# chrished/DEMC.jl

Measured on AMD Instinct MI355X. Metric: chain-updates/sec (N x gens/s) + gens-to-Rhat<1.05, MvNormal d=5 N=1024, higher is better.
Workload: dtype f64

## Files before the change

demc.jl_amd/_lib.py:

```python
from __future__ import annotations

import ctypes as C
import os
import subprocess
from pathlib import Path

import numpy as np

PKG_DIR = Path(__file__).resolve().parent
REPO_ROOT = PKG_DIR.parent
LIB_PATH = Path(os.environ["DEMCZ_LIB"]) if os.environ.get("DEMCZ_LIB") else PKG_DIR / "libdemcz_hip.so"
ABI_VERSION = 1
LAYOUT_SPLIT = 100
LAYOUT_SPLIT_WAVE = 164
LAYOUT_PROGRAM_WAVE = 264

TARGET_MVNORMAL, TARGET_ISO_QUAD, TARGET_LINREG_SSE, TARGET_HOST_CALLBACK, TARGET_PROGRAM = 0, 1, 2, 3, 4
OK, ERR_INVALID_ARGUMENT, ERR_HIP, ERR_CAPACITY, ERR_STATE, ERR_NO_DEVICE, ERR_COMM = range(7)

_dp = C.POINTER(C.c_double)
_ip = C.POINTER(C.c_int32)
_lp = C.POINTER(C.c_int64)
_up = C.POINTER(C.c_uint64)

SYMBOLS = [
    "demcz_abi_version", "demcz_create", "demcz_destroy", "demcz_last_error", "demcz_set_state",
    "demcz_get_state", "demcz_set_history_origin", "demcz_run", "demcz_synchronize",
    "demcz_get_history", "demcz_get_changed", "demcz_rhat", "demcz_accept_ratio", "demcz_mean_cov",
    "demcz_propose", "demcz_accept_commit", "demcz_end_generation", "demcz_comm_unique_id",
    "demcz_comm_init", "demcz_export_current_device", "demcz_append_rows_device",
    "demcz_set_external_append", "demcz_get_info", "demcz_selftest_draws", "demcz_append_rows",
    "demcz_rhat_partial", "demcz_set_rng_offset", "demcz_rhat_array", "demcz_accept_ratio_array",
    "demcz_mean_cov_array", "demcz_set_append_lag", "demcz_run_checked", "demcz_set_kernel_timing",
    "demcz_get_kernel_time", "demcz_set_live_spin_limit", "demcz_get_live_status",
    "demcz_debug_append_slab", "demcz_get_changed_total", "demcz_debug_set_live_fault",
    "demcz_set_comm_timeout", "demcz_debug_stall_exchange", "demcz_get_kernel_time_series",
    "demcz_history_stream", "demcz_get_history_view", "demcz_detach_history", "demcz_release_host_buffer", "demcz_get_archive_pinned",
    "demcz_debug_kernel_counts", "demcz_pool_trim", "demcz_debug_kernel_name", "demcz_peer_group", "demcz_get_peer_status", "demcz_peer_export", "demcz_peer_attach",
    "demcz_peer_detach", "demcz_get_peer_ping", "demcz_set_live_rearms", "demcz_get_live_rearms",
    "demcz_closure_buffers", "demcz_program_check", "demcz_set_program",
    "demcz_program_check_layout",
    "demcz_autocov_sums", "demcz_autocov_sums_array", "demcz_ess_from_sums", "demcz_ess", "demcz_ess_array",
    "demcz_quantile_plan", "demcz_select_counts", "demcz_select_step", "demcz_quantile_finish", "demcz_quantiles",
    "demcz_quantiles_array", "demcz_best", "demcz_best_array",
    "demcz_derive_check", "demcz_derive", "demcz_derive_array",
    "demcz_rank_to_z", "demcz_rank_normalize", "demcz_rank_normalize_array", "demcz_indicator_le", "demcz_rank_diagnostics",
    "demcz_rank_diagnostics_array",
    "demcz_set_snooker", "demcz_get_snooker",
    "demcz_pointwise_check", "demcz_pointwise", "demcz_pointwise_array", "demcz_psis_tail_length", "demcz_gpd_fit",
    "demcz_loo_columns", "demcz_loo_columns_array", "demcz_loo", "demcz_loo_array",
    "demcz_bridge_check", "demcz_bridge_posterior", "demcz_bridge_posterior_array", "demcz_bridge_proposal",
    "demcz_bridge_proposal_program", "demcz_bridge_iterate", "demcz_bridge", "demcz_bridge_array",
    "demcz_histogram_edges", "demcz_histogram", "demcz_histogram_array", "demcz_histogram2d", "demcz_histogram2d_array",
    "demcz_hdi_steps", "demcz_hdi", "demcz_hdi_array",
]


class DemczError(RuntimeError):
    def __init__(self, code: int, msg: str):
        super().__init__(f"libdemcz_hip status {code}: {msg}")
        self.code = code


class Config(C.Structure):
    _fields_ = [
        ("N", C.c_int64), ("chain_id0", C.c_int64), ("d", C.c_int32), ("K", C.c_int32),
        ("Mcap", C.c_int64), ("Gcap", C.c_int64), ("Nblocks", C.c_int32),
        ("block_offsets", _ip), ("block_indices", _ip), ("eps_scale", _dp),
        ("seed", C.c_uint64), ("device_id", C.c_int32), ("target_kind", C.c_int32),
        ("mu", _dp), ("W", _dp), ("c0", C.c_double), ("design", _dp), ("yobs", _dp),
        ("nobs", C.c_int64), ("stream", C.c_void_p), ("lanes_per_chain", C.c_int32),
        ("reserved0", C.c_int32),
    ]


HIPCC_FLAGS = ["-O3", "--offload-arch=gfx950", "-ffp-contract=off", "-fPIC", "-Werror", "-Wno-pass-failed"]


def sources() -> list:
    csrc = PKG_DIR / "csrc"
    return ([csrc / "demcz_capi.hip"] + sorted(csrc.glob("demcz_pw_inst_*.hip")) + sorted(csrc.glob("demcz_mlr_inst_*.hip"))
            + [csrc / "demcz_snooker_inst.hip", csrc / "demcz_bridge_inst.hip", csrc / "demcz_program.hip"])


def build_command(out: Path = LIB_PATH) -> list:
    return ["hipcc"] + HIPCC_FLAGS + ["-shared", "-o", str(out)] + [str(p) for p in sources()] + ["-lrccl", "-lhiprtc"]


def build_lib(out: Path = LIB_PATH, extra: list = (), jobs: int = 0) -> Path:
    from concurrent.futures import ThreadPoolExecutor
    objdir = REPO_ROOT / "build" / "obj" / Path(out).stem
    objdir.mkdir(parents=True, exist_ok=True)
    srcs = sources()
    jobs = jobs or max(1, min(len(srcs), len(os.sched_getaffinity(0))))

    def compile_one(src):
        obj = objdir / (src.stem + ".o")
        r = subprocess.run(["hipcc"] + list(extra) + HIPCC_FLAGS + ["-c", "-o", str(obj), str(src)], capture_output=True, text=True)
        if r.returncode != 0:
            raise RuntimeError(f"hipcc failed on {src.name}:\n{r.stderr[-4000:]}")
        return obj

    with ThreadPoolExecutor(max_workers=jobs) as ex:
        objs = list(ex.map(compile_one, srcs))
    subprocess.run(["hipcc", "--offload-arch=gfx950", "-shared", "-fPIC", "-o", str(out)] + [str(o) for o in objs] + ["-lrccl", "-lhiprtc"], check=True)
    return Path(out)


def build(force: bool = False) -> Path:
    srcs = list((PKG_DIR / "csrc").glob("*")) + [REPO_ROOT / "include" / "demcz.h"]
    if not force and LIB_PATH.exists():
        newest = max(p.stat().st_mtime for p in srcs)
        if LIB_PATH.stat().st_mtime >= newest:
            return LIB_PATH
    return build_lib(LIB_PATH)


_LIB = None


def load():
    global _LIB
    if _LIB is not None:
        return _LIB
    if not LIB_PATH.exists():
        raise FileNotFoundError(
            f"{LIB_PATH} is missing: build it with `python -c 'import __graft_entry__ as g; g.build()'` "
            "(hipcc --offload-arch=gfx950).  There is no CPU fallback.")
    L = C.CDLL(str(LIB_PATH))
    L.demcz_abi_version.restype = C.c_int32
    if L.demcz_abi_version() != ABI_VERSION:
        raise RuntimeError("libdemcz_hip.so ABI version mismatch: rebuild")
    L.demcz_last_error.restype = C.c_char_p
    L.demcz_last_error.argtypes = [C.c_void_p]
    L.demcz_create.argtypes = [C.POINTER(C.c_void_p), C.POINTER(Config)]
    L.demcz_destroy.argtypes = [C.c_void_p]
    L.demcz_set_state.argtypes = [C.c_void_p, _dp, _dp, _dp, C.c_int64, C.c_int64]
    L.demcz_get_state.argtypes = [C.c_void_p, _dp, _dp, _dp, C.c_int64, _lp]
    L.demcz_set_history_origin.argtypes = [C.c_void_p, C.c_int64]
    L.demcz_run.argtypes = [C.c_void_p, C.c_int64, C.c_int64, C.c_double, _dp]
    L.demcz_synchronize.argtypes = [C.c_void_p]
    L.demcz_get_history.argtypes = [C.c_void_p, C.c_int64, C.c_int64, _dp, _dp]
    L.demcz_get_changed.argtypes = [C.c_void_p, C.c_int64, C.c_int64, _lp]
    L.demcz_get_changed_total.argtypes = [C.c_void_p, C.c_int64, C.c_int64, _lp, _ip]
    L.demcz_rhat.argtypes = [C.c_void_p, C.c_int64, C.c_int64, _dp]
    L.demcz_accept_ratio.argtypes = [C.c_void_p, C.c_int64, C.c_int64, _dp]
    L.demcz_mean_cov.argtypes = [C.c_void_p, C.c_int64, C.c_int64, _dp, _dp]
    L.demcz_propose.argtypes = [C.c_void_p, C.c_int64, C.c_int32, C.c_double, _dp]
    L.demcz_accept_commit.argtypes = [C.c_void_p, _dp, _dp]
    L.demcz_end_generation.argtypes = [C.c_void_p, C.c_int64]
    L.demcz_closure_buffers.argtypes = [C.c_void_p, C.POINTER(C.c_void_p), C.POINTER(C.c_void_p)]
    L.demcz_comm_unique_id.argtypes = [C.c_void_p]
    L.demcz_comm_init.argtypes = [C.c_void_p, C.c_void_p, C.c_int32, C.c_int32]
    L.demcz_export_current_device.argtypes = [C.c_void_p, C.c_void_p]
    L.demcz_append_rows_device.argtypes = [C.c_void_p, C.c_void_p, C.c_int64, C.c_int64]
    L.demcz_append_rows.argtypes = [C.c_void_p, _dp, C.c_int64, C.c_int64]
    L.demcz_rhat_partial.argtypes = [C.c_void_p, C.c_int64, C.c_int64, C.c_int32, _dp, _dp]
    L.demcz_set_rng_offset.argtypes = [C.c_void_p, C.c_int64]
    L.demcz_set_snooker.argtypes = [C.c_void_p, C.c_int32, C.c_double, C.c_double]
    L.demcz_get_snooker.argtypes = [C.c_void_p, _ip, _dp, _dp, _lp]
    L.demcz_set_append_lag.argtypes = [C.c_void_p, C.c_int32]
    L.demcz_rhat_array.argtypes = [C.c_int32, _dp, C.c_int64, C.c_int32, C.c_int64, _dp]
    L.demcz_autocov_sums.argtypes = [C.c_void_p, C.c_int64, C.c_int64, C.c_int64, C.c_int64, _dp]
    L.demcz_autocov_sums_array.argtypes = [C.c_int32, _dp, C.c_int64, C.c_int32, C.c_int64, C.c_int64, C.c_int64, _dp]
    L.demcz_ess_from_sums.argtypes = [C.c_int32, C.c_int64, C.c_int64, C.c_int64, _dp, _dp, _dp, _dp, _dp, _lp, _ip]
    L.demcz_ess.argtypes = [C.c_void_p, C.c_int64, C.c_int64, C.c_int64, _dp, _dp, _dp, _lp, _ip]
    L.demcz_ess_array.argtypes = [C.c_int32, _dp, C.c_int64, C.c_int32, C.c_int64, C.c_int64, _dp, _dp, _dp, _lp, _ip]
    L.demcz_quantile_plan.argtypes = [C.c_int64, C.c_int32, _dp, _lp, _lp, _dp]
    L.demcz_select_counts.argtypes = [C.c_void_p, C.c_int64, C.c_int64, C.c_int32, C.c_int32, _up, _lp, _lp]
    L.demcz_select_step.argtypes = [C.c_int32, C.c_int32, _lp, _up, _lp]
    L.demcz_quantile_finish.argtypes = [C.c_int32, C.c_int32, _up, _up, _dp, _lp, _dp, _dp, _dp]
    L.demcz_quantiles.argtypes = [C.c_void_p, C.c_int64, C.c_int64, C.c_int32, _dp, _dp, _dp, _dp]
    L.demcz_quantiles_array.argtypes = [C.c_int32, _dp, C.c_int64, C.c_int32, C.c_int64, C.c_int32, _dp, _dp, _dp, _dp]
    L.demcz_best.argtypes = [C.c_void_p, C.c_int64, C.c_int64, _dp, _lp, _lp, _dp]
    L.demcz_best_array.argtypes = [C.c_int32, _dp, C.c_int64, C.c_int64, _dp, _lp, _lp]
    L.demcz_accept_ratio_array.argtypes = [C.c_int32, _dp, C.c_int64, C.c_int64, _dp]
    L.demcz_mean_cov_array.argtypes = [C.c_int32, _dp, C.c_int64, C.c_int32, C.c_int64, _dp, _dp]
    L.demcz_set_external_append.argtypes = [C.c_void_p, C.c_int32]
    L.demcz_get_info.argtypes = [C.c_void_p, _lp, _lp, _ip]
    L.demcz_selftest_draws.argtypes = [C.c_int32, C.c_uint64, C.c_uint64, C.c_uint64, C.c_int32,
                                       C.POINTER(C.c_uint64), _dp, _dp]
    L.demcz_set_live_spin_limit.argtypes = [C.c_void_p, C.c_int32]
    L.demcz_get_live_status.argtypes = [C.c_void_p, _ip, _ip]
    L.demcz_debug_kernel_counts.argtypes = [C.c_void_p, _lp]
    L.demcz_history_stream.argtypes = [C.c_void_p, C.c_int32]
    L.demcz_get_history_view.argtypes = [C.c_void_p, C.c_int64, C.c_int64, C.POINTER(C.c_void_p), C.POINTER(C.c_void_p)]
    L.demcz_detach_history.argtypes = [C.c_void_p, C.POINTER(C.c_void_p), C.POINTER(C.c_void_p)]
    L.demcz_release_host_buffer.argtypes = [C.c_void_p]
    L.demcz_pool_trim.argtypes = [_lp, _lp]
    L.demcz_peer_group.argtypes = [C.POINTER(C.c_void_p), C.c_int32]
    L.demcz_get_peer_status.argtypes = [C.c_void_p, _ip, _ip]
    L.demcz_peer_export.argtypes = [C.c_void_p, C.c_int32, C.c_int32, C.c_void_p]
    L.demcz_peer_attach.argtypes = [C.c_void_p, C.c_void_p]
    L.demcz_peer_detach.argtypes = [C.c_void_p]
    L.demcz_get_peer_ping.argtypes = [C.c_void_p, _ip, _dp]
    L.demcz_set_live_rearms.argtypes = [C.c_void_p, C.c_int32]
    L.demcz_get_live_rearms.argtypes = [C.c_void_p, _ip, _ip]
    L.demcz_debug_kernel_name.argtypes = [C.c_void_p, C.c_char_p, C.c_int32]
    L.demcz_program_check.argtypes = [C.c_int32, C.c_char_p, C.c_char_p]
    L.demcz_program_check_layout.argtypes = [C.c_int32, C.c_char_p, C.c_char_p, C.c_int32]
    L.demcz_set_program.argtypes = [C.c_void_p, C.c_char_p, C.c_char_p, _dp, C.c_int64]
    L.demcz_derive_check.argtypes = [C.c_int32, C.c_int32, C.c_char_p, C.c_char_p]
    L.demcz_derive.argtypes = [C.c_void_p, C.c_int64, C.c_int64, C.c_int32, C.c_char_p, C.c_char_p, _dp, C.c_int64, C.POINTER(C.c_void_p)]
    L.demcz_derive_array.argtypes = [C.c_int32, _dp, _dp, C.c_int64, C.c_int32, C.c_int64, C.c_int32, C.c_char_p, C.c_char_p, _dp,
                                     C.c_int64, C.POINTER(C.c_void_p)]
    L.demcz_rank_to_z.argtypes = [C.c_int64, _dp, C.c_int64, _dp]
    L.demcz_rank_normalize.argtypes = [C.c_void_p, C.c_int64, C.c_int64, C.c_int32, _dp, C.POINTER(C.c_void_p)]
    L.demcz_rank_normalize_array.argtypes = [C.c_int32, _dp, C.c_int64, C.c_int32, C.c_int64, C.c_int32, _dp, C.POINTER(C.c_void_p)]
    L.demcz_indicator_le.argtypes = [C.c_void_p, C.c_int64, C.c_int64, C.c_int32, _dp, C.POINTER(C.c_void_p)]
    L.demcz_rank_diagnostics.argtypes = [C.c_void_p, C.c_int64, C.c_int64, _dp, _dp, _dp]
    L.demcz_rank_diagnostics_array.argtypes = [C.c_int32, _dp, C.c_int64, C.c_int32, C.c_int64, _dp, _dp, _dp]
    L.demcz_histogram_edges.argtypes = [C.c_int32, C.c_double, C.c_double, _dp]
    L.demcz_histogram.argtypes = [C.c_void_p, C.c_int64, C.c_int64, C.c_int32, _dp, _dp, _dp, _lp, _lp, _lp, _lp]
    L.demcz_histogram_array.argtypes = [C.c_int32, _dp, C.c_int64, C.c_int32, C.c_int64, C.c_int32, _dp, _dp, _dp, _lp, _lp, _lp, _lp]
    L.demcz_histogram2d.argtypes = [C.c_void_p, C.c_int64, C.c_int64, C.c_int32, _ip, C.c_int32, C.c_int32, _dp, _dp, _dp, _dp, _lp, _lp]
    L.demcz_histogram2d_array.argtypes = [C.c_int32, _dp, C.c_int64, C.c_int32, C.c_int64, C.c_int32, _ip, C.c_int32, C.c_int32, _dp, _dp,
                                          _dp, _dp, _lp, _lp]
    L.demcz_hdi_steps.argtypes = [C.c_int64, C.c_int32, _dp, _lp]
    L.demcz_hdi.argtypes = [C.c_void_p, C.c_int64, C.c_int64, C.c_int32, _dp, _dp]
    L.demcz_hdi_array.argtypes = [C.c_int32, _dp, C.c_int64, C.c_int32, C.c_int64, C.c_int32, _dp, _dp]
    _vpp = C.POINTER(C.c_void_p)
    L.demcz_pointwise_check.argtypes = [C.c_int32, C.c_char_p, C.c_char_p]
    L.demcz_pointwise.argtypes = [C.c_void_p, C.c_int64, C.c_int64, C.c_int64, C.c_int32, C.c_char_p, C.c_char_p, _dp, C.c_int64, _vpp]
    L.demcz_pointwise_array.argtypes = [C.c_int32, _dp, C.c_int64, C.c_int32, C.c_int64, C.c_int64, C.c_int32, C.c_char_p, C.c_char_p,
                                        _dp, C.c_int64, _vpp]
    L.demcz_psis_tail_length.argtypes = [C.c_int64, C.c_double, _lp]
    L.demcz_gpd_fit.argtypes = [C.c_int64, _dp, _dp, _dp, _dp]
    L.demcz_loo_columns.argtypes = [C.c_void_p, C.c_int64, C.c_int64, _dp, _dp, _dp, _lp, _dp, _dp]
    L.demcz_loo_columns_array.argtypes = [C.c_int32, _dp, C.c_int64, C.c_int32, C.c_int64, _dp, _dp, _dp, _lp, _dp, _dp]
    L.demcz_loo.argtypes = [C.c_void_p, C.c_int64, C.c_int64, C.c_int64, C.c_char_p, C.c_char_p, _dp, C.c_int64, _dp, _dp, _dp, _lp,
                            _dp, _dp]
    L.demcz_loo_array.argtypes = [C.c_int32, _dp, C.c_int64, C.c_int32, C.c_int64, C.c_int64, C.c_char_p, C.c_char_p, _dp, C.c_int64,
                                  _dp, _dp, _dp, _lp, _dp, _dp]
    _bridge_out = [_dp, _dp, _lp, _ip, _lp, _lp, _dp, _lp, _dp, _dp, _dp]
    L.demcz_bridge_check.argtypes = [C.c_int32, C.c_char_p, C.c_char_p]
    L.demcz_bridge_posterior.argtypes = [C.c_void_p, C.c_int64, C.c_int64, _dp, _dp, _vpp]
    L.demcz_bridge_posterior_array.argtypes = [C.c_int32, _dp, _dp, C.c_int64, C.c_int32, C.c_int64, _dp, _dp, _vpp]
    L.demcz_bridge_proposal.argtypes = [C.c_void_p, C.c_int64, C.c_int64, C.c_uint64, _dp, _dp, _vpp, _vpp]
    L.demcz_bridge_proposal_program.argtypes = [C.c_int32, C.c_int32, C.c_int64, C.c_int64, C.c_uint64, _dp, _dp, C.c_char_p, C.c_char_p,
                                                _dp, C.c_int64, _vpp, _vpp]
    L.demcz_bridge_iterate.argtypes = [C.c_void_p, C.c_int64, C.c_int64, C.c_void_p, C.c_int64, C.c_int64, C.c_double, C.c_double,
                                       C.c_int64, _dp, _lp, _ip, _dp, _lp, _vpp]
    L.demcz_bridge.argtypes = [C.c_void_p, C.c_int64, C.c_int64, C.c_uint64, C.c_double, C.c_double, C.c_int64] + _bridge_out
    L.demcz_bridge_array.argtypes = [C.c_int32, _dp, _dp, C.c_int64, C.c_int32, C.c_int64, C.c_char_p, C.c_char_p, _dp, C.c_int64,
                                     C.c_uint64, C.c_double, C.c_double, C.c_int64] + _bridge_out
    L.demcz_get_archive_pinned.argtypes =[C.c_void_p, C.POINTER(C.c_void_p), _lp]
    L.demcz_get_kernel_time_series.argtypes = [C.c_void_p, C.c_int32, _dp, _dp, _ip]
    L.demcz_set_comm_timeout.argtypes = [C.c_void_p, C.c_int64]
    L.demcz_debug_stall_exchange.argtypes = [C.c_void_p, C.c_int32]
    L.demcz_debug_set_live_fault.argtypes = [C.c_void_p, C.c_int32, C.c_int64]
    L.demcz_debug_append_slab.argtypes = [C.c_void_p, _dp, C.c_int32, C.c_int32, C.c_int32]
    for name in SYMBOLS:
        fn = getattr(L, name)
        if name != "demcz_last_error":
            fn.restype = C.c_int32
    _LIB = L
    return L


def derive_launch_constants() -> tuple:
    import re
    text = (PKG_DIR / "csrc" / "demcz_kernels_derive.h").read_text()
    return tuple(int(re.search(rf"constexpr int {name} = (\d+);", text).group(1)) for name in ("DERIVE_THREADS", "DERIVE_MAX_WG"))


def f64(a, order="C"):
    return np.require(a, dtype=np.float64, requirements=["F" if order == "F" else "C", "A"])


def ptr(a, t=_dp):
    return a.ctypes.data_as(t) if a is not None else None
```

demc.jl_amd/csrc/demcz_capi.hip:

```cpp
#include "../../include/demcz.h"
#include "demcz_kernels.h"
#include "demcz_kernels_acf.h"
#include "demcz_kernels_sel.h"
#include "demcz_select_host.h"
#include "demcz_kernels_rank.h"
#include "demcz_kernels_density.h"
#include "demcz_kernels_loo.h"
#include "demcz_kernels_bridge.h"
#include "demcz_slab_plan.h"
#include "demcz_run_plan.h"
#include "demcz_kernels_ml.h"
#include "demcz_kernels_pc.h"
#include "demcz_kernels_lr.h"
#include "demcz_kernels_ps.h"
#include "demcz_kernels_ps2.h"
#include "demcz_kernels_ps2d.h"
#include "demcz_kernels_snooker.h"
#include "demcz_pw_dispatch.h"
#include "demcz_mlr_dispatch.h"
#include "demcz_program.h"

#include <rccl/rccl.h>

#include <algorithm>
#include <chrono>
#include <thread>
#include <cstdlib>
#include <deque>
#include <map>
#include <mutex>
#include <cfloat>
#include <cmath>
#include <cstdio>
#include <cstring>
#include <string>
#include <unordered_map>
#include <vector>

using namespace demcz;

static thread_local std::string g_create_error;

namespace {
struct BufPool {
    struct Entry { void* p; size_t bytes; int device; };
    std::mutex mu;
    std::vector<Entry> free_list;
    size_t cached = 0;
    const size_t cap;
    const bool host;
    BufPool(size_t cap_, bool host_) : cap(cap_), host(host_) {}
    hipError_t acquire(void** out, size_t bytes, int device)
    {
        {
            std::lock_guard<std::mutex> lk(mu);
            int best = -1;
            for (int i = 0; i < (int)free_list.size(); ++i) {
                const Entry& e = free_list[i];
                if (e.device == device && e.bytes >= bytes && e.bytes <= bytes + bytes / 4 + (1u << 20) && (best < 0 || e.bytes < free_list[best].bytes)) best = i;
            }
            if (best >= 0) {
                *out = free_list[best].p;
                cached -= free_list[best].bytes;
                sizes[*out] = free_list[best].bytes;
                free_list.erase(free_list.begin() + best);
                return hipSuccess;
            }
        }
        hipError_t e = host ? hipHostMalloc(out, bytes, hipHostMallocDefault) : hipMalloc(out, bytes);
        if (e != hipSuccess) {
            (void)hipGetLastError();
            if (trim() > 0) e = host ? hipHostMalloc(out, bytes, hipHostMallocDefault) : hipMalloc(out, bytes);
        }
        if (e == hipSuccess) { std::lock_guard<std::mutex> lk(mu); sizes[*out] = bytes; }
        return e;
    }
    size_t trim()
    {
        std::vector<Entry> drop;
        size_t n = 0;
        {
            std::lock_guard<std::mutex> lk(mu);
            drop.swap(free_list);
            n = cached;
            cached = 0;
        }
        for (const Entry& e : drop) { if (host) (void)hipHostFree(e.p); else (void)hipFree(e.p); }
        return n;
    }
    void discard(void* p)
    {
        if (!p) return;
        { std::lock_guard<std::mutex> lk(mu); sizes.erase(p); }
        if (host) (void)hipHostFree(p); else (void)hipFree(p);
    }
    void release(void* p, int device)
    {
        if (!p) return;
        size_t bytes = 0;
        {
            std::lock_guard<std::mutex> lk(mu);
            auto it = sizes.find(p);
            if (it != sizes.end()) { bytes = it->second; sizes.erase(it); }
            if (bytes && cached + bytes <= cap && !getenv("DEMCZ_NO_POOL")) {
                free_list.push_back({p, bytes, device});
                cached += bytes;
                return;
            }
        }
        if (host) (void)hipHostFree(p); else (void)hipFree(p);
    }
    std::unordered_map<void*, size_t> sizes;
};
BufPool g_dev_pool(6ull << 30, false);
BufPool g_host_pool(3ull << 30, true);
}
static std::mutex g_stream_mu;
static std::vector<std::pair<int, hipStream_t>> g_stream_pool;
static hipError_t stream_acquire(int device, hipStream_t* out)
{
    {
        std::lock_guard<std::mutex> lk(g_stream_mu);
        for (size_t i = 0; i < g_stream_pool.size(); ++i)
            if (g_stream_pool[i].first == device) { *out = g_stream_pool[i].second; g_stream_pool.erase(g_stream_pool.begin() + (long)i); return hipSuccess; }
    }
    return hipStreamCreateWithFlags(out, hipStreamNonBlocking);
}
static void stream_release(int device, hipStream_t s, bool drained)
{
    if (!s) return;
    if (drained && !getenv("DEMCZ_NO_POOL")) {
        std::lock_guard<std::mutex> lk(g_stream_mu);
        if (g_stream_pool.size() < 32) { g_stream_pool.emplace_back(device, s); return; }
    }
    (void)hipStreamDestroy(s);
}
static hipError_t dev_malloc(int device, void** out, size_t bytes) { return g_dev_pool.acquire(out, std::max<size_t>(bytes, 16), device); }
static hipError_t dev_free(int device, void* p) { g_dev_pool.release(p, device); return hipSuccess; }
static hipError_t host_malloc(void** out, size_t bytes) { return g_host_pool.acquire(out, std::max<size_t>(bytes, 16), -1); }
static hipError_t host_free(void* p) { g_host_pool.release(p, -1); return hipSuccess; }

struct demcz_handle;
enum SplitKind {
    SPLIT_NONE = 0,
    SPLIT_PC8,
    SPLIT_ML,
    SPLIT_MLB,
    SPLIT_WAVE,
};

enum KernelArm { ARM_ONE_LANE, ARM_ML, ARM_ML_COOP, ARM_MLB, ARM_LR16, ARM_PC8, ARM_ML_REC, ARM_MLB_REC, ARM_LR16_REC, ARM_LR8S,
                 ARM_PS, ARM_PS2, ARM_PS2D, ARM_PW, ARM_PROGRAM_WAVE, ARM_SNOOKER };
struct WindowKernel {
    const void* fn = nullptr;
    hipFunction_t mod = nullptr;
    int threads = 0;
    size_t dyn_lds = 0;
    bool big_lds = false;
    int waves = 0;
    bool steady = false;
    KernelArm arm = ARM_ONE_LANE;
    bool live = false, temper = false;
    int pw_form = 0;
};

struct LaunchFacts {
    bool live = false;
    bool temper = false;
    bool ps2 = false;
    bool dual = false;
    bool pw_reg = false;
    bool pw_matrix = false;
    bool coop = false;
    bool lr16 = false;
    bool snooker = false;
};

struct PeerGroup {
    std::vector<demcz_handle*> members;
    bool failed = false;
    int32_t rearms_left = 3;
    bool lockstep_only = false;
    bool busy = false;
    bool dead = false;
};

struct demcz_handle {
    demcz_config cfg{};
    int lanes = 1;
    hipStream_t stream = nullptr;
    bool own_stream = false;
    std::string err;
    std::vector<int32_t> block_offsets, block_indices, slot_of;
    std::vector<double> eps;
    int64_t S = 0;
    int64_t ZS = 0;
    bool full_block = false;
    int ngrp = 1;
    uint64_t gstart = 1ull;
    int mlb_qb = 0;
    double* dZ = nullptr;
    double* dX = nullptr;
    double* dlp = nullptr;
    double* dchain = nullptr;
    double* dchain_alloc = nullptr;
    double* dlogobj = nullptr;
    double* dlp_origin = nullptr;
    bool origin_valid = false;
    double* dtemp = nullptr;
    int64_t temp_cap = 0;
    int32_t* d_block_offsets = nullptr;
    int32_t* d_slot_of = nullptr;
    double* d_eps = nullptr;
    double* d_mu = nullptr;
    double* d_Wp = nullptr;
    double* d_design = nullptr;
    double* d_y = nullptr;
    double* d_scratch = nullptr;
    int64_t scratch_cap = 0;
    double* d_stage = nullptr;
    int64_t stage_cap = 0;
    int64_t M = 0;
    int64_t g_done = 0;
    int64_t g0 = 0;
    int64_t rng_offset = 0;
    bool has_state = false;
    int64_t launches = 0;
    mutable int64_t kernel_counts[1] = {0};
    WindowKernel last_kernel;
    bool external_append = false;
    double* dXprop = nullptr;
    double* dlogu = nullptr;
    bool proposal_pending = false;
    bool gen_open = false;
    double* hc_X = nullptr;
    double* hc_lp = nullptr;
    volatile unsigned int* hc_flag = nullptr;
    unsigned int* hc_count = nullptr;
    unsigned int hc_seq = 0;
    hipStream_t diag_stream = nullptr;
    hipEvent_t diag_ev = nullptr;
    hipEvent_t rhat_side_ev = nullptr;
    bool rhat_side_pending = false;
    double* d_spec_X = nullptr;
    double* d_spec_lp = nullptr;
    hipEvent_t spec_ev = nullptr;
    double* pinned_rhat = nullptr;
    unsigned int* pinned_err = nullptr;
    int64_t pinned_err_launches = -1;
    int64_t pinned_cap = 0;
    bool timing = false;
    std::vector<std::pair<hipEvent_t, hipEvent_t>> timed;
    std::vector<int32_t> timed_slabs;
    std::vector<double> series_start_ms, series_dur_ms;
    int64_t timed_launches = 0;
    int64_t live_wg_cap = -1;
    SplitKind split_kind = SPLIT_NONE;
    int split_lanes = 0;
    int split_per_wg = 1;
    int32_t* d_slot_role = nullptr;
    double* d_rec[2] = {nullptr, nullptr};
    unsigned int* d_live_err = nullptr;
#ifdef DEMCZ_STAMPS
    unsigned long long* d_stamps = nullptr;
#endif
    bool arena = false, rec_in_arena = false, hist_joint = false;
    int64_t arena_gens = 0;
    int64_t arena_span = 0;
    double* arena_rec[2] = {nullptr, nullptr};
    double* arena_temp = nullptr;
    int64_t rec_cap = 0;
    int rec_cur = 0;
    bool host_paced = false;
    int wpw = 1;
    bool ps_dual = false;
    bool dual_now = false;
    bool lr_spec = false;
    bool no_live = false;
    bool live_claimed = false;
    unsigned int live_spin_limit = 0;
    int32_t live_fault_polls = 0;
    int64_t live_fault_g = 0;
    bool in_checked = false;
    struct RunCall { int64_t g_from, g_to; double gamma; bool tempered; std::vector<double> temperature; };
    std::vector<RunCall> live_log;
    double* d_safe_X = nullptr;
    double* d_safe_lp = nullptr;
    bool snap_pending = false;
    int64_t safe_M = 0, safe_M_app = 0, safe_g_done = 0;
    bool replaying = false;
    int32_t live_redos = 0;
    int32_t live_rearms_left = 3;
    int32_t live_rearms = 0;
    int64_t rearm_from = -1;
    uint32_t fail_row_hint = 0xffffffffu;
    RecDesc rec_desc[2];
    hipStream_t prod_stream = nullptr;
    hipEvent_t prod_done[2] = {nullptr, nullptr};
    hipEvent_t prod_gate = nullptr;
    bool prod_pending[2] = {false, false};
    hipEvent_t after_launch_ev = nullptr;
    unsigned int* d_acc = nullptr;
    int64_t acc_waves = 0;
    int32_t acc_slots = 0, acc_next = 0;
    struct LaunchRec { int64_t g_first, g_last; int32_t slot; };
    std::deque<LaunchRec> acc_log;
    ncclComm_t comm = nullptr;
    ncclComm_t comm_side = nullptr;
    int nranks = 1, rank = 0;
    double* d_gather = nullptr;
    int lag = 0;
    int64_t M_app = 0;
    struct PendingRows { int64_t visible_from; int64_t M_after; hipEvent_t ev; int64_t xseq = 0; };
    std::deque<PendingRows> pending;
    int64_t batch_J = -1;
    hipStream_t comm_stream = nullptr;
    double* d_send[2] = {nullptr, nullptr};
    double* d_recv[2] = {nullptr, nullptr};
    hipEvent_t buf_done[2] = {nullptr, nullptr};
    int64_t xseq = 0, xseq_waited = 0, buf_xseq[2] = {0, 0};
    int batch_buf = 0, batch_cnt = 0;
    int64_t batch_base = 0;
    bool hs_on = false;
    double* hs_chain = nullptr;
    double* hs_logobj = nullptr;
    hipStream_t hs_stream = nullptr;
    bool pooled_dev = false;
    volatile long long* xdone = nullptr;
    int peer_mode = 0;
    int n_peers = 0;
    double* peer_Z[DEMCZ_MAX_PEERS] = {nullptr};
    void* ipc_mapped[DEMCZ_MAX_PEERS] = {nullptr};
    struct PeerGroup* group = nullptr;
    bool err_clean = false;
    bool peer_fence = false;
    unsigned int* d_err_all = nullptr;
    bool archive_fine = false;
    size_t dZ_bytes = 0;
    size_t mailbox_off = 0;
    bool peers_closed = false;
    int32_t ping_ok = -1;
    double ping_wait_us = 0.0;
    int64_t live_share = 0;
    int64_t comm_timeout_ms = 60000;
    bool comm_dead = false;
    int* stall_flag = nullptr;
    int32_t stall_next_ms = 0;
    bool prog_ready = false;
    demcz_prog::Module prog;
    std::string prog_source, prog_options;
    bool prog_wave = false;
    bool derived = false;
    int64_t snooker_every = 0;
    double snooker_lo = 1.2, snooker_hi = 2.2;
    int64_t snooker_steps = 0;
    bool snooker_now = false;
};

#define HIPCHK(h, expr)                                                                          \
    do {                                                                                         \
        hipError_t e_ = (expr);                                                                  \
        if (e_ != hipSuccess) {                                                                  \
            (h)->err = std::string(#expr) + ": " + hipGetErrorString(e_);                        \
            return DEMCZ_ERR_HIP;                                                                \
        }                                                                                        \
    } while (0)

#define NCCLCHK(h, expr)                                                                         \
    do {                                                                                         \
        ncclResult_t r_ = (expr);                                                                \
        if (r_ != ncclSuccess) {                                                                 \
            (h)->err = std::string(#expr) + ": " + ncclGetErrorString(r_);                       \
            return DEMCZ_ERR_COMM;                                                               \
        }                                                                                        \
    } while (0)


#define DEADCHK(h)                                                                               \
    do {                                                                                         \
        if ((h)->comm_dead) return DEMCZ_ERR_COMM;                                               \
    } while (0)

static int32_t fail(demcz_handle* h, int32_t code, const std::string& msg)
{
    if (h) h->err = msg; else g_create_error = msg;
    return code;
}

static int32_t refuse_derived(const demcz_handle* h, const char* who)
{
    if (!h || !h->derived) return DEMCZ_OK;
    return fail(const_cast<demcz_handle*>(h), DEMCZ_ERR_STATE,
                std::string(who) + ": the handle is a derived history (demcz_derive): it takes the statistics over its values, demcz_get_history "
                                   "without log_obj, demcz_derive, demcz_pointwise, demcz_loo, demcz_bridge_iterate, demcz_synchronize and demcz_destroy, and nothing else");
}
#define NOT_DERIVED(h)                                                                           \
    do {                                                                                         \
        int32_t rd_ = refuse_derived((h), __func__);                                             \
        if (rd_) return rd_;                                                                     \
    } while (0)
// ... 104 lines not shown
}

static int32_t sync_event(demcz_handle* h, hipEvent_t ev, const char* what)
{
    if (h->comm_dead) return DEMCZ_ERR_COMM;
    if (!h->comm) {
        const hipError_t e = hipEventSynchronize(ev);
        if (e != hipSuccess) { h->err = std::string(what) + ": hipEventSynchronize: " + hipGetErrorString(e); return DEMCZ_ERR_HIP; }
        return DEMCZ_OK;
    }
    return wait_deadline(h, [ev]() { return hipEventQuery(ev); }, what);
}

#define SYNCCHK_AS(h, s, who)                                                                    \
    do {                                                                                         \
        int32_t rcs_ = sync_stream((h), (s), (who));                                             \
        if (rcs_) return rcs_;                                                                   \
    } while (0)
#define SYNCCHK(h, s) SYNCCHK_AS(h, s, __func__)

static int32_t quiesce_all(demcz_handle* h)
{
    if (h->comm_dead) return DEMCZ_ERR_COMM;
    if (!h->comm) return DEMCZ_OK;
    for (hipStream_t st : {h->stream, h->comm_stream, h->prod_stream, h->diag_stream, h->hs_stream})
        if (st) { int32_t rc = sync_stream(h, st, "quiesce"); if (rc) return rc; }
    return DEMCZ_OK;
}

static int32_t maybe_stall(demcz_handle* h, hipStream_t s)
{
    if (h->stall_next_ms <= 0) return DEMCZ_OK;
    if (getenv("DEMCZ_DEBUG_COMM")) fprintf(stderr, "[demcz] stall kernel of %d ms enqueued\n", h->stall_next_ms);
    if (!h->stall_flag) HIPCHK(h, dev_malloc(h->cfg.device_id, (void**)&h->stall_flag, sizeof(int)));
    HIPCHK(h, hipMemsetAsync(h->stall_flag, 0, sizeof(int), s));
    hipLaunchKernelGGL(stall_kernel, dim3(1), dim3(1), 0, s, h->stall_flag, (unsigned long long)h->stall_next_ms * 100000ull);
    HIPCHK(h, hipGetLastError());
    h->stall_next_ms = 0;
    return DEMCZ_OK;
}

static int64_t blockstep_nblk(int b)
{
    const int nn = (b == 1) ? 1 : b;
    return 1 + (nn + 1) / 2 + 1;
}

constexpr size_t ML_MAX_DYNAMIC_LDS = 160 * 1024;
constexpr size_t PEER_MAILBOX_BYTES = 4096;
constexpr size_t REC_PAD = 64;
constexpr int PC_CONSUMER_CHAINS = 8;
static int ml_lanes_available(int target_kind, int d, bool full_block, int64_t nobs, int max_blocklen, int nblocks);
static bool pc_available(int target_kind, int d, bool full_block);
static bool mlb32_wanted(int64_t N);
static bool split_ml_available(int target_kind, int d, bool full_block, int64_t nobs);
static bool ps_available(int target_kind, int d);
static int64_t live_wg_capacity(demcz_handle* h);
static WindowKernel window_kernel_of(const demcz_handle* h, const LaunchFacts& f);
static LaunchFacts launch_facts(const demcz_handle* h, const WindowParams* P, bool live);
constexpr int MAX_LIVE_KERNELS = 6;
static int live_kernels(const demcz_handle* h, WindowKernel out[MAX_LIVE_KERNELS]);
static void rec_invalidate(demcz_handle* h)
{
    if (h->prod_stream) (void)hipStreamSynchronize(h->prod_stream);
    h->prod_pending[0] = h->prod_pending[1] = false;
    h->rec_desc[0].valid = h->rec_desc[1].valid = false;
}
static int32_t rec_scrub(demcz_handle* h)
{
    rec_invalidate(h);
    if (h->lanes != DEMCZ_LAYOUT_SPLIT || h->rec_cap <= 0 || getenv("DEMCZ_NO_SCRUB")) return DEMCZ_OK;
    for (int b = 0; b < 2; ++b) {
        if (!h->d_rec[b]) continue;
        const size_t per = h->rec_in_arena ? (size_t)(h->cfg.d + 2) : (size_t)((h->split_kind == SPLIT_MLB) ? 2 * h->S : (int64_t)h->cfg.d + 2);
        const size_t nd = (size_t)h->rec_cap * per * (size_t)h->cfg.N + REC_PAD;
        HIPCHK(h, hipMemsetAsync(h->d_rec[b], 0, nd * sizeof(double), h->stream));
    }
    return DEMCZ_OK;
}
static int32_t flush_exchanges(demcz_handle* h);
static void peer_detach(demcz_handle* h);
static void peer_no_dual(demcz_handle* h);
static int32_t peer_setup_ipc(demcz_handle* h);
static bool peer_capable(const demcz_handle* h);
static int32_t check_live_err(demcz_handle* h);
static int32_t live_verify(demcz_handle* h);
static int32_t group_verify(demcz_handle* h);
static int32_t live_failed(demcz_handle* h, bool& failed);
static void live_release(demcz_handle* h);
static int64_t live_span(demcz_handle* h);
static int64_t rec_target_bytes(bool dual);
static int32_t rec_reserve(demcz_handle* h, int64_t gens);
static int32_t check_hist_range(demcz_handle* h, int64_t g_from, int64_t g_to, const char* who);
static bool ps2_applicable(const demcz_handle* h, const WindowParams& P);

extern "C" int32_t demcz_abi_version(void) { return DEMCZ_ABI_VERSION; }

extern "C" const char* demcz_last_error(const demcz_handle* h)
{
    return h ? h->err.c_str() : g_create_error.c_str();
}

template <class T>
static hipError_t dev_alloc_copy(T** dst, const T* src, size_t n, hipStream_t s, int device)
{
    hipError_t e = dev_malloc(device, (void**)dst, std::max<size_t>(n, 1) * sizeof(T));
    if (e != hipSuccess) return e;
    if (n) e = hipMemcpyAsync(*dst, src, n * sizeof(T), hipMemcpyHostToDevice, s);
    return e;
}

static void free_all(demcz_handle* h)
{
    bool drained = !h->comm_dead;
    for (hipStream_t st : {h->stream, h->prod_stream, h->diag_stream, h->comm_stream, h->hs_stream})
        if (st && hipStreamQuery(st) != hipSuccess) drained = false;
    if (h->d_acc) (void)dev_free(h->cfg.device_id, h->d_acc);
    if (h->d_err_all) (void)dev_free(h->cfg.device_id, h->d_err_all);
    if (h->archive_fine) { if (h->dZ) (void)hipFree(h->dZ); h->dZ = nullptr; }
    if (h->pooled_dev) {
        if (h->archive_fine) {
        } else if (drained) {
            g_dev_pool.release(h->dZ, h->cfg.device_id);
        } else {
            g_dev_pool.discard(h->dZ);
        }
        if (h->hist_joint) { if (drained) g_dev_pool.release(h->dchain_alloc, h->cfg.device_id); else g_dev_pool.discard(h->dchain_alloc); }
        h->dZ = nullptr;
        if (h->hist_joint) { h->dchain = nullptr; h->dchain_alloc = nullptr; }
    }
    if (h->hs_stream) stream_release(h->cfg.device_id, h->hs_stream, drained);
    if (drained) { g_host_pool.release(h->hs_chain, -1); g_host_pool.release(h->hs_logobj, -1); }
    else { g_host_pool.discard(h->hs_chain); g_host_pool.discard(h->hs_logobj); }
    void* bufs[] = {h->dZ, h->dX, h->dlp, h->dchain, h->hist_joint ? nullptr : h->dlogobj, h->dlp_origin, h->dtemp, h->d_block_offsets,
                    h->d_slot_of, h->d_slot_role, h->d_eps, h->d_mu, h->d_Wp, h->d_design, h->d_y, h->d_scratch, h->dXprop,
                    h->dlogu, h->d_gather};
    for (void* b : bufs)
        if (b) (void)dev_free(h->cfg.device_id, b);
    for (auto& pe : h->pending) if (pe.ev) (void)hipEventDestroy(pe.ev);
    h->pending.clear();
    for (int b = 0; b < 2; ++b) {
        if (h->d_rec[b] && !h->rec_in_arena) (void)dev_free(h->cfg.device_id, h->d_rec[b]);
        if (b == 0 && h->d_live_err) (void)dev_free(h->cfg.device_id, h->d_live_err);
        if (h->d_send[b]) (void)dev_free(h->cfg.device_id, h->d_send[b]);
        if (h->d_recv[b]) (void)dev_free(h->cfg.device_id, h->d_recv[b]);
        if (h->buf_done[b]) (void)hipEventDestroy(h->buf_done[b]);
    }
    if (h->comm_stream) stream_release(h->cfg.device_id, h->comm_stream, !h->comm_dead && hipStreamQuery(h->comm_stream) == hipSuccess);
    if (h->prod_stream) { if (!h->comm_dead) (void)hipStreamSynchronize(h->prod_stream); stream_release(h->cfg.device_id, h->prod_stream, !h->comm_dead); }
    for (int b = 0; b < 2; ++b) if (h->prod_done[b]) (void)hipEventDestroy(h->prod_done[b]);
    if (h->prod_gate) (void)hipEventDestroy(h->prod_gate);
    if (h->d_stage) (void)host_free(h->d_stage);
    for (auto& pr : h->timed) { (void)hipEventDestroy(pr.first); (void)hipEventDestroy(pr.second); }
    if (h->pinned_rhat) (void)host_free(h->pinned_rhat);
    if (h->pinned_err) (void)host_free(h->pinned_err);
    if (h->d_safe_X) (void)dev_free(h->cfg.device_id, h->d_safe_X);
    if (h->d_safe_lp) (void)dev_free(h->cfg.device_id, h->d_safe_lp);
    if (h->d_spec_X) (void)dev_free(h->cfg.device_id, h->d_spec_X);
    if (h->d_spec_lp) (void)dev_free(h->cfg.device_id, h->d_spec_lp);
    if (h->spec_ev) (void)hipEventDestroy(h->spec_ev);
    if (h->diag_ev) (void)hipEventDestroy(h->diag_ev);
    if (h->rhat_side_ev) (void)hipEventDestroy(h->rhat_side_ev);
    if (h->diag_stream) stream_release(h->cfg.device_id, h->diag_stream, !h->comm_dead && hipStreamQuery(h->diag_stream) == hipSuccess);
    if (h->stall_flag) (void)dev_free(h->cfg.device_id, h->stall_flag);
    if (h->hc_X) (void)hipHostFree(h->hc_X);
    if (h->hc_lp) (void)hipHostFree(h->hc_lp);
    if (h->hc_flag) (void)hipHostFree(const_cast<unsigned int*>(h->hc_flag));
    if (h->hc_count) (void)dev_free(h->cfg.device_id, h->hc_count);
    if (h->xdone) (void)host_free(const_cast<long long*>(h->xdone));
    if (!h->comm_dead) {
        if (h->comm_side) (void)ncclCommDestroy(h->comm_side);
        if (h->comm) (void)ncclCommDestroy(h->comm);
    }
    if (h->own_stream && h->stream) stream_release(h->cfg.device_id, h->stream, !h->comm_dead && hipStreamQuery(h->stream) == hipSuccess);
}

extern "C" int32_t demcz_create(demcz_handle** out, const demcz_config* cfg)
{
    if (!out || !cfg) return fail(nullptr, DEMCZ_ERR_INVALID_ARGUMENT, "demcz_create: null argument");
    *out = nullptr;
    if (cfg->N < 1 || cfg->d < 1 || cfg->d > MAX_D || cfg->K < 1 || cfg->Mcap < 2 || cfg->Gcap < 0 ||
        cfg->Nblocks < 1 || !cfg->block_offsets || !cfg->block_indices || !cfg->eps_scale || cfg->chain_id0 < 0)
        return fail(nullptr, DEMCZ_ERR_INVALID_ARGUMENT,
                    "demcz_create: need N>=1, 1<=d<=64, K>=1, Mcap>=2, Gcap>=0, Nblocks>=1 and block/eps tables");
    if (cfg->lanes_per_chain != 0 && cfg->lanes_per_chain != 1 && cfg->lanes_per_chain != 8 && cfg->lanes_per_chain != 16 &&
        cfg->lanes_per_chain != DEMCZ_LAYOUT_SPLIT && cfg->lanes_per_chain != DEMCZ_LAYOUT_SPLIT_WAVE &&
        cfg->lanes_per_chain != DEMCZ_LAYOUT_PROGRAM_WAVE)
        return fail(nullptr, DEMCZ_ERR_INVALID_ARGUMENT,
                    "demcz_create: lanes_per_chain must be 0 (auto), 1, 8, 16, DEMCZ_LAYOUT_SPLIT, DEMCZ_LAYOUT_SPLIT_WAVE or (program targets) "
                    "DEMCZ_LAYOUT_PROGRAM_WAVE");
    if (cfg->lanes_per_chain == DEMCZ_LAYOUT_PROGRAM_WAVE && cfg->target_kind != DEMCZ_TARGET_PROGRAM)
        return fail(nullptr, DEMCZ_ERR_INVALID_ARGUMENT, "demcz_create: DEMCZ_LAYOUT_PROGRAM_WAVE is the wave-per-chain layout of program targets: "
                                                         "target_kind must be DEMCZ_TARGET_PROGRAM (built-in targets: DEMCZ_LAYOUT_SPLIT_WAVE)");
    const int d = cfg->d;
    if (cfg->block_offsets[0] != 0) return fail(nullptr, DEMCZ_ERR_INVALID_ARGUMENT, "block_offsets[0] must be 0");
    for (int ib = 0; ib < cfg->Nblocks; ++ib) {
        const int a = cfg->block_offsets[ib], b = cfg->block_offsets[ib + 1];
        if (b <= a || b - a > d) return fail(nullptr, DEMCZ_ERR_INVALID_ARGUMENT, "empty or oversized block");
        for (int t = a; t < b; ++t) {
            if (cfg->block_indices[t] < 0 || cfg->block_indices[t] >= d)
                return fail(nullptr, DEMCZ_ERR_INVALID_ARGUMENT, "block index out of range");
            for (int u = a; u < t; ++u)
                if (cfg->block_indices[u] == cfg->block_indices[t])
                    return fail(nullptr, DEMCZ_ERR_INVALID_ARGUMENT, "duplicate index inside a block");
        }
    }
    switch (cfg->target_kind) {
    case DEMCZ_TARGET_MVNORMAL:
        if (!cfg->mu || !cfg->W) return fail(nullptr, DEMCZ_ERR_INVALID_ARGUMENT, "MVNORMAL needs mu and W");
        break;
    case DEMCZ_TARGET_ISO_QUAD:
        if (!cfg->mu) return fail(nullptr, DEMCZ_ERR_INVALID_ARGUMENT, "ISO_QUAD needs mu");
        break;
    case DEMCZ_TARGET_LINREG_SSE:
        if (!cfg->design || !cfg->yobs || cfg->nobs < 1)
            return fail(nullptr, DEMCZ_ERR_INVALID_ARGUMENT, "LINREG_SSE needs design, yobs, nobs>=1");
        break;
    case DEMCZ_TARGET_HOST_CALLBACK: break;
    case DEMCZ_TARGET_PROGRAM:
        if (cfg->lanes_per_chain != 0 && cfg->lanes_per_chain != 1 && cfg->lanes_per_chain != DEMCZ_LAYOUT_PROGRAM_WAVE)
            return fail(nullptr, DEMCZ_ERR_INVALID_ARGUMENT, "demcz_create: a program target runs one lane per chain: lanes_per_chain must be 0 or 1 "
                                                             "(or DEMCZ_LAYOUT_PROGRAM_WAVE: one wavefront per chain)");
        if (cfg->d > demcz_prog::MAX_PROGRAM_D)
            return fail(nullptr, DEMCZ_ERR_INVALID_ARGUMENT, "demcz_create: a program target needs 1 <= d <= 32");
        if (cfg->lanes_per_chain == DEMCZ_LAYOUT_PROGRAM_WAVE) {
            bool one_block = cfg->Nblocks == 1 && cfg->block_offsets[1] == d;
            for (int p = 0; one_block && p < d; ++p) one_block = cfg->block_indices[p] == p;
            if (!one_block)
                return fail(nullptr, DEMCZ_ERR_INVALID_ARGUMENT, "demcz_create: DEMCZ_LAYOUT_PROGRAM_WAVE needs one block 0..d-1 in order (block updates run one lane per chain)");
            if (d < demcz_prog::WAVE_MIN_D)
                return fail(nullptr, DEMCZ_ERR_INVALID_ARGUMENT, "demcz_create: DEMCZ_LAYOUT_PROGRAM_WAVE needs 2 <= d <= 32");
            if (cfg->N > PS_MAX_N)
                return fail(nullptr, DEMCZ_ERR_INVALID_ARGUMENT, "demcz_create: DEMCZ_LAYOUT_PROGRAM_WAVE needs N <= " + std::to_string(PS_MAX_N) +
                                                                 " (one wavefront per chain: PS_MAX_N)");
            if (!(cfg->Mcap <= 0xffffffffll && (double)cfg->Mcap * 8.0 * (((d + 7) / 8) * 8) < 4294967296.0))
                return fail(nullptr, DEMCZ_ERR_INVALID_ARGUMENT, "demcz_create: DEMCZ_LAYOUT_PROGRAM_WAVE needs an archive reachable by 32-bit offsets: "
                                                                 "Mcap * 8 * (d rounded up to a multiple of 8) < 2^32");
        }
        break;
    default: return fail(nullptr, DEMCZ_ERR_INVALID_ARGUMENT, "unknown target_kind");
    }
    int ndev = 0;
    if (hipGetDeviceCount(&ndev) != hipSuccess || ndev < 1)
        return fail(nullptr, DEMCZ_ERR_NO_DEVICE, "demcz_create: no HIP device visible (there is no CPU fallback)");
    if (cfg->device_id < 0 || cfg->device_id >= ndev)
        return fail(nullptr, DEMCZ_ERR_INVALID_ARGUMENT, "demcz_create: device_id out of range");

    demcz_handle* h = new demcz_handle();
    h->cfg = *cfg;
    h->lanes = 1;
    if (const char* re = getenv("DEMCZ_LIVE_REARMS")) h->live_rearms_left = std::max(0, atoi(re));
    auto bail = [&](int32_t code) {
        g_create_error = h->err;
        free_all(h);
        delete h;
        return code;
    };
#define CRCHK(expr)                                                                              \
    do {                                                                                         \
        hipError_t e_ = (expr);                                                                  \
        if (e_ != hipSuccess) {                                                                  \
            h->err = std::string(#expr) + ": " + hipGetErrorString(e_);                          \
            return bail(DEMCZ_ERR_HIP);                                                          \
        }                                                                                        \
    } while (0)
    CRCHK(hipSetDevice(cfg->device_id));
    if (cfg->stream) {
        h->stream = (hipStream_t)cfg->stream;
    } else {
        CRCHK(stream_acquire(cfg->device_id, &h->stream));
        h->own_stream = true;
    }
    h->block_offsets.assign(cfg->block_offsets, cfg->block_offsets + cfg->Nblocks + 1);
    h->block_indices.assign(cfg->block_indices, cfg->block_indices + h->block_offsets.back());
    h->eps.assign(cfg->eps_scale, cfg->eps_scale + d);
    h->slot_of.assign((size_t)cfg->Nblocks * d, -1);
    h->S = 0;
    for (int ib = 0; ib < cfg->Nblocks; ++ib) {
        const int a = h->block_offsets[ib], b = h->block_offsets[ib + 1];
        for (int t = a; t < b; ++t) h->slot_of[(size_t)ib * d + h->block_indices[t]] = t - a;
        h->S += blockstep_nblk(b - a);
    }
    h->full_block = (cfg->Nblocks == 1 && h->block_offsets[1] == d);
    if (h->full_block)
        for (int p = 0; p < d; ++p) h->full_block = h->full_block && (h->block_indices[p] == p);
    if (cfg->target_kind == DEMCZ_TARGET_MVNORMAL && cfg->Nblocks >= 2 && h->block_offsets.back() == d) {
        bool ok = true;
        uint64_t starts = 0;
        for (int ib = 0; ib < cfg->Nblocks && ok; ++ib) {
            const int lo = h->block_offsets[ib], hi = h->block_offsets[ib + 1];
            uint64_t seen = 0;
            for (int t = lo; t < hi; ++t) {
                const int j = h->block_indices[t];
                if (j < lo || j >= hi || ((seen >> (j - lo)) & 1ull)) { ok = false; break; }
                seen |= 1ull << (j - lo);
            }
            starts |= 1ull << lo;
        }
        if (ok) {
            h->ngrp = cfg->Nblocks;
            h->gstart = starts;
            bool equal = true;
            for (int ib = 0; ib < cfg->Nblocks; ++ib) equal = equal && (h->block_offsets[ib + 1] - h->block_offsets[ib] == h->block_offsets[1]);
            if (equal && d == 20 && h->block_offsets[1] == 5 && !getenv("DEMCZ_NO_MLB_INCREMENTAL")) h->mlb_qb = 5;
        }
    }
    {
// ... 1782 lines not shown
extern "C" int32_t demcz_run(demcz_handle* h, int64_t g_from, int64_t g_to, double gamma, const double* temperature)
{
    NOT_DERIVED(h);
    return run_call(h, g_from, g_to, gamma, temperature, RunHints{});
}

extern "C" int32_t demcz_synchronize(demcz_handle* h)
{
    if (!h) return DEMCZ_ERR_INVALID_ARGUMENT;
    DEADCHK(h);
    HIPCHK(h, hipSetDevice(h->cfg.device_id));
    SYNCCHK(h, h->stream);
    if (h->comm_stream) SYNCCHK(h, h->comm_stream);
    if (h->prod_stream) SYNCCHK(h, h->prod_stream);
    return live_verify(h);
}

static int32_t check_hist_range(demcz_handle* h, int64_t g_from, int64_t g_to, const char* who)
{
    if (h->cfg.Gcap <= 0) return fail(h, DEMCZ_ERR_STATE, std::string(who) + ": handle keeps no history (Gcap = 0)");
    if (g_from < 1 || g_to < g_from || g_from - h->g0 - 1 < 0 || g_to - h->g0 > h->cfg.Gcap)
        return fail(h, DEMCZ_ERR_INVALID_ARGUMENT, std::string(who) + ": generations outside the history window");
    return DEMCZ_OK;
}

extern "C" int32_t demcz_get_history(demcz_handle* h, int64_t g_from, int64_t g_to, double* chain, double* log_obj)
{
    if (!h) return DEMCZ_ERR_INVALID_ARGUMENT;
    DEADCHK(h);
    if (log_obj) NOT_DERIVED(h);
    int32_t rc = check_hist_range(h, g_from, g_to, "demcz_get_history");
    if (rc) return rc;
    HIPCHK(h, hipSetDevice(h->cfg.device_id));
    rc = live_verify(h);
    if (rc) return rc;
    const int64_t N = h->cfg.N, G = g_to - g_from + 1, s0 = g_from - h->g0 - 1;
    const int d = h->cfg.d;
    if (chain)
        HIPCHK(h, hipMemcpyAsync(chain, h->dchain + (size_t)N * d * s0, (size_t)N * d * G * sizeof(double),
                                 hipMemcpyDeviceToHost, h->stream));
    if (log_obj)
        HIPCHK(h, hipMemcpyAsync(log_obj, h->dlogobj + (size_t)N * s0, (size_t)N * G * sizeof(double),
                                 hipMemcpyDeviceToHost, h->stream));
    SYNCCHK(h, h->stream);
    return DEMCZ_OK;
}

extern "C" int32_t demcz_get_changed(demcz_handle* h, int64_t g_from, int64_t g_to, int64_t* changed)
{
    NOT_DERIVED(h);
    if (!h || !changed) return DEMCZ_ERR_INVALID_ARGUMENT;
    int32_t rc = check_hist_range(h, g_from, g_to, "demcz_get_changed");
    if (rc) return rc;
    const int64_t G = g_to - g_from + 1, s0 = g_from - h->g0 - 1;
    if (s0 == 0 && !h->origin_valid)
        return fail(h, DEMCZ_ERR_STATE, "demcz_get_changed: the log_obj before the first history slot is not known "
                                        "(set the history origin when exactly g0 generations have been run)");
    HIPCHK(h, hipSetDevice(h->cfg.device_id));
    rc = live_verify(h);
    if (rc) return rc;
    rc = ensure_scratch(h, G);
    if (rc) return rc;
    static_assert(sizeof(long long) == sizeof(double), "scratch reuse");
    hipLaunchKernelGGL(changed_from_history_kernel, dim3((unsigned)G), dim3(256), 0, h->stream, (const double*)h->dlogobj,
                       (const double*)h->dlp_origin, h->cfg.N, s0, (long long*)h->d_scratch);
    HIPCHK(h, hipGetLastError());
    static_assert(sizeof(int64_t) == sizeof(long long), "int64 layout");
    HIPCHK(h, hipMemcpyAsync(changed, h->d_scratch, (size_t)G * sizeof(int64_t), hipMemcpyDeviceToHost, h->stream));
    SYNCCHK(h, h->stream);
    return DEMCZ_OK;
}

namespace demcz {
__global__ void __launch_bounds__(256) sum_counts_kernel(const unsigned int* acc, int64_t waves, int slot0, int nslots, int ring,
                                                         int skip_first, long long* out)
{
    __shared__ long long red[256];
    long long a = 0;
    for (int64_t i = threadIdx.x; i < (int64_t)nslots * waves; i += 256) {
        const int sl = (int)(i / waves);
        const int64_t w = i % waves;
        const unsigned int* e = acc + ((size_t)((slot0 + sl) % ring) * (size_t)waves + (size_t)w) * 2;
        a += (long long)e[0];
        if (skip_first && sl == 0) a -= (long long)e[1];
    }
    red[threadIdx.x] = a;
    __syncthreads();
    for (int st = 128; st > 0; st >>= 1) {
        if ((int)threadIdx.x < st) red[threadIdx.x] += red[threadIdx.x + st];
        __syncthreads();
    }
    if (threadIdx.x == 0) *out = red[0];
}
}

extern "C" int32_t demcz_get_changed_total(demcz_handle* h, int64_t g_from, int64_t g_to, int64_t* total, int32_t* from_ballots)
{
    NOT_DERIVED(h);
    if (!h || !total || g_from < 1 || g_to < g_from) return DEMCZ_ERR_INVALID_ARGUMENT;
    HIPCHK(h, hipSetDevice(h->cfg.device_id));
    int32_t rc = live_verify(h);
    if (rc) return rc;
    int first = -1, last = -1, skip = 0;
    for (int i = 0; i < (int)h->acc_log.size(); ++i) {
        const auto& r = h->acc_log[i];
        if (first < 0 && (r.g_first == g_from || r.g_first == g_from - 1) && r.g_last >= g_from) { first = i; skip = (r.g_first == g_from - 1); }
        if (first >= 0 && r.g_last == g_to) { last = i; break; }
    }
    bool ok = first >= 0 && last >= first;
    for (int i = first; ok && i < last; ++i)
        ok = h->acc_log[i].g_last + 1 == h->acc_log[i + 1].g_first && (h->acc_log[i].slot + 1) % h->acc_slots == h->acc_log[i + 1].slot;
    if (ok && h->d_acc) {
        rc = ensure_scratch(h, 1);
        if (rc) return rc;
        static_assert(sizeof(long long) == sizeof(double), "scratch reuse");
        hipLaunchKernelGGL(sum_counts_kernel, dim3(1), dim3(256), 0, h->stream, (const unsigned int*)h->d_acc, h->acc_waves,
                           (int)h->acc_log[first].slot, last - first + 1, (int)h->acc_slots, skip, (long long*)h->d_scratch);
        HIPCHK(h, hipGetLastError());
        long long v = 0;
        HIPCHK(h, hipMemcpyAsync(&v, h->d_scratch, sizeof(v), hipMemcpyDeviceToHost, h->stream));
        SYNCCHK(h, h->stream);
        *total = (int64_t)v;
        if (from_ballots) *from_ballots = 1;
        return DEMCZ_OK;
    }
    std::vector<int64_t> ch((size_t)(g_to - g_from + 1));
    rc = demcz_get_changed(h, g_from, g_to, ch.data());
    if (rc) return rc;
    int64_t t = 0;
    for (int64_t v : ch) t += v;
    *total = t;
    if (from_ballots) *from_ballots = 0;
    return DEMCZ_OK;
}

struct RhatPlan { int64_t N, w, s0, n, nd, need; int d, nchunk; double *S1, *S2, *mean_j, *s2_j, *sums; int slabs = 1; double* out = nullptr; };

static int rhat_chunks(int64_t n) { return (int)std::min<int64_t>(std::max<int64_t>(1, n / 32), 32); }
static int64_t rhat_need(int64_t nd, int d, int nchunk) { return 2 * (2 * nchunk * nd) + 2 * (2 * nd) + 4 * d; }

static int32_t rhat_plan(demcz_handle* h, int64_t g_from, int64_t g_to, RhatPlan& r, const char* who = "demcz_rhat")
{
    int32_t rc = check_hist_range(h, g_from, g_to, who);
    if (rc) return rc;
    r.N = h->cfg.N; r.w = g_to - g_from + 1; r.s0 = g_from - h->g0 - 1; r.d = h->cfg.d;
    r.n = r.w / 2;
    if (r.n < 2) return fail(h, DEMCZ_ERR_INVALID_ARGUMENT, std::string(who) + ": window needs at least 4 generations");
    r.nchunk = rhat_chunks(r.n);
    r.nd = r.N * r.d;
    r.need = rhat_need(r.nd, r.d, r.nchunk);
    return DEMCZ_OK;
}

static int32_t rhat_scratch(demcz_handle* h, RhatPlan& r, int64_t extra, bool compute, hipStream_t qs = nullptr)
{
    HIPCHK(h, hipSetDevice(h->cfg.device_id));
    int32_t rc = ensure_scratch(h, r.need * r.slabs + (r.slabs > 1 ? (int64_t)r.slabs * r.d : 0) + extra);
    if (rc) return rc;
    r.S1 = h->d_scratch;
    r.S2 = r.S1 + 2 * r.nchunk * r.nd;
    r.mean_j = r.S2 + 2 * r.nchunk * r.nd;
    r.s2_j = r.mean_j + 2 * r.nd;
    r.sums = r.s2_j + 2 * r.nd;
    r.out = r.slabs > 1 ? h->d_scratch + r.need * r.slabs : r.sums + 3 * r.d;
    if (compute) {
        const int bs = 256;
        const unsigned gx = (unsigned)((r.nd + bs - 1) / bs);
        if (!qs) qs = h->stream;
        hipLaunchKernelGGL(rhat_moments_kernel, dim3(gx, 2 * r.nchunk, r.slabs), dim3(bs), 0, qs, h->dchain, r.N, r.d, r.s0, r.n, r.nchunk, r.S1, r.S2,
                           r.w, r.need);
        hipLaunchKernelGGL(rhat_chainstats_kernel, dim3(gx, 2, r.slabs), dim3(bs), 0, qs, h->dchain, r.N, r.d, r.s0, r.n, r.nchunk, r.S1, r.S2, r.mean_j,
                           r.s2_j, r.w, r.need);
        HIPCHK(h, hipGetLastError());
    }
    return DEMCZ_OK;
}

static int32_t rhat_prepare(demcz_handle* h, int64_t g_from, int64_t g_to, RhatPlan& r, bool compute, hipStream_t qs = nullptr, int slabs = 1)
{
    int32_t rc = rhat_plan(h, g_from, g_to, r);
    if (rc) return rc;
    if (slabs > 1) {
        rc = check_hist_range(h, g_from, g_from + r.w * slabs - 1, "demcz_run_checked");
        if (rc) return rc;
        r.slabs = slabs;
    }
    return rhat_scratch(h, r, 0, compute, qs);
}

extern "C" int32_t demcz_rhat_partial(demcz_handle* h, int64_t g_from, int64_t g_to, int32_t stage, const double* grand, double* out)
{
    if (!h || !out || (stage != 0 && stage != 1) || (stage == 1 && !grand)) return DEMCZ_ERR_INVALID_ARGUMENT;
    RhatPlan r;
    int32_t rc = live_verify(h);
    if (rc) return rc;
    rc = rhat_prepare(h, g_from, g_to, r, true);
    if (rc) return rc;
    const int d = r.d;
    if (stage == 0) {
        hipLaunchKernelGGL(rhat_reduce_kernel, dim3(d), dim3(256), 0, h->stream, r.mean_j, r.s2_j, r.N, d, 0, (const double*)nullptr, 1.0, r.sums);
        HIPCHK(h, hipGetLastError());
        HIPCHK(h, hipMemcpyAsync(out, r.sums, (size_t)d * sizeof(double), hipMemcpyDeviceToHost, h->stream));
    } else {
        HIPCHK(h, hipMemcpyAsync(r.sums, grand, (size_t)d * sizeof(double), hipMemcpyHostToDevice, h->stream));
        hipLaunchKernelGGL(rhat_reduce_kernel, dim3(d), dim3(256), 0, h->stream, r.mean_j, r.s2_j, r.N, d, 1, (const double*)r.sums, 1.0, r.sums + d);
        HIPCHK(h, hipGetLastError());
        HIPCHK(h, hipMemcpyAsync(out, r.sums + d, (size_t)2 * d * sizeof(double), hipMemcpyDeviceToHost, h->stream));
    }
    SYNCCHK(h, h->stream);
    return DEMCZ_OK;
}

static int32_t rhat_enqueue(demcz_handle* h, int64_t g_from, int64_t g_to, double* out, bool side = false, int slabs = 1)
{
    RhatPlan r;
    hipStream_t qs = h->stream;
    static const bool own_env = getenv("DEMCZ_RHAT_OWN_STREAM") != nullptr;
    if (side && !h->comm && !own_env && h->prod_stream) {
        if (!h->diag_ev) HIPCHK(h, hipEventCreateWithFlags(&h->diag_ev, hipEventDisableTiming));
        if (h->after_launch_ev) {
            HIPCHK(h, hipStreamWaitEvent(h->prod_stream, h->after_launch_ev, 0));
        } else {
            HIPCHK(h, hipEventRecord(h->diag_ev, h->stream));
            HIPCHK(h, hipStreamWaitEvent(h->prod_stream, h->diag_ev, 0));
            h->after_launch_ev = h->diag_ev;
        }
        qs = h->prod_stream;
    } else if (side && h->comm && h->peer_mode == 2 && !h->no_live && h->comm_side && h->comm_stream && h->lag == 0) {
        if (!h->diag_ev) HIPCHK(h, hipEventCreateWithFlags(&h->diag_ev, hipEventDisableTiming));
        if (h->after_launch_ev) {
            HIPCHK(h, hipStreamWaitEvent(h->comm_stream, h->after_launch_ev, 0));
        } else {
            HIPCHK(h, hipEventRecord(h->diag_ev, h->stream));
            HIPCHK(h, hipStreamWaitEvent(h->comm_stream, h->diag_ev, 0));
            h->after_launch_ev = h->diag_ev;
        }
        qs = h->comm_stream;
    } else if (side && !h->comm) {
        if (!h->diag_stream) HIPCHK(h, stream_acquire(h->cfg.device_id, &h->diag_stream));
        if (!h->diag_ev) HIPCHK(h, hipEventCreateWithFlags(&h->diag_ev, hipEventDisableTiming));
        if (h->after_launch_ev) {
            HIPCHK(h, hipStreamWaitEvent(h->diag_stream, h->after_launch_ev, 0));
        } else {
            HIPCHK(h, hipEventRecord(h->diag_ev, h->stream));
            HIPCHK(h, hipStreamWaitEvent(h->diag_stream, h->diag_ev, 0));
            h->after_launch_ev = h->diag_ev;
        }
        qs = h->diag_stream;
    }
    if (qs == h->stream && h->rhat_side_pending) {
        HIPCHK(h, hipStreamWaitEvent(h->stream, h->rhat_side_ev, 0));
        h->rhat_side_pending = false;
    }
    struct SideMark {
        demcz_handle* h; hipStream_t qs;
        ~SideMark() {
            if (qs == h->stream) return;
            if (!h->rhat_side_ev && hipEventCreateWithFlags(&h->rhat_side_ev, hipEventDisableTiming) != hipSuccess) { h->rhat_side_ev = nullptr; return; }
            if (hipEventRecord(h->rhat_side_ev, qs) == hipSuccess) h->rhat_side_pending = true;
        }
    } side_mark{h, qs};
    if (slabs > 1 && h->comm) return fail(h, DEMCZ_ERR_STATE, "demcz_run_checked: batched checks are for unsharded runs");
    int32_t rc = rhat_prepare(h, g_from, g_to, r, true, qs, slabs);
    if (rc) return rc;
    const int d = r.d;
    const int64_t n = r.n;
    const int64_t m = 2 * r.N * h->nranks;
    const bool sharded = (h->comm != nullptr);
    double* sums = r.sums;
    if (!sharded) {
        hipLaunchKernelGGL(rhat_tail_kernel, dim3(d, r.slabs), dim3(256), 0, qs, r.mean_j, r.s2_j, r.N, d, (double)n, (double)m, r.out, r.need);
        HIPCHK(h, hipGetLastError());
        HIPCHK(h, hipMemcpyAsync(out, r.out, (size_t)r.slabs * d * sizeof(double), hipMemcpyDeviceToHost, qs));
        return DEMCZ_OK;
    }
    const ncclComm_t cq = (qs == h->comm_stream && qs != h->stream) ? h->comm_side : h->comm;
    hipLaunchKernelGGL(rhat_reduce_kernel, dim3(d), dim3(256), 0, qs, r.mean_j, r.s2_j, r.N, d, 0, (const double*)nullptr, 1.0, sums);
    HIPCHK(h, hipGetLastError());
    NCCLCHK(h, ncclAllReduce(sums, sums, (size_t)d, ncclDouble, ncclSum, cq, qs));
    hipLaunchKernelGGL(rhat_reduce_kernel, dim3(d), dim3(256), 0, qs, r.mean_j, r.s2_j, r.N, d, 1, (const double*)sums, (double)m, sums + d);
    HIPCHK(h, hipGetLastError());
    NCCLCHK(h, ncclAllReduce(sums + d, sums + d, (size_t)2 * d, ncclDouble, ncclSum, cq, qs));
    hipLaunchKernelGGL(rhat_final_kernel, dim3((unsigned)((d + 63) / 64)), dim3(64), 0, qs, (const double*)(sums + d), d, (double)n, (double)m, sums + 3 * d);
    HIPCHK(h, hipGetLastError());
    HIPCHK(h, hipMemcpyAsync(out, sums + 3 * d, (size_t)d * sizeof(double), hipMemcpyDeviceToHost, qs));
    return DEMCZ_OK;
}

extern "C" int32_t demcz_rhat(demcz_handle* h, int64_t g_from, int64_t g_to, double* rhat)
{
    if (!h || !rhat) return DEMCZ_ERR_INVALID_ARGUMENT;
    int32_t rc = live_verify(h);
    if (rc) return rc;
    rc = rhat_enqueue(h, g_from, g_to, rhat);
    if (rc) return rc;
    SYNCCHK(h, h->stream);
    return DEMCZ_OK;
}

struct AcfPlan { RhatPlan r; int nchunk, tiles; int64_t per; double *part, *out; };

static void acf_chunks(int64_t N, int d, int64_t n, int& nchunk, int64_t& per)
{
    const int64_t waves = (N * d + ACF_BS - 1) / ACF_BS;
    const int64_t want = (4096 + 8 * waves - 1) / (8 * waves);
    const int64_t k = std::max<int64_t>(1, std::min<int64_t>(std::min<int64_t>(n / (2 * ACF_TL), want), 64));
    per = ((n + k - 1) / k + ACF_TL - 1) / ACF_TL * ACF_TL;
    nchunk = (int)((n + per - 1) / per);
}

static int32_t acf_prepare(demcz_handle* h, int64_t g_from, int64_t g_to, AcfPlan& a, const char* who)
{
    int32_t rc = live_verify(h);
    if (rc) return rc;
    rc = rhat_plan(h, g_from, g_to, a.r, who);
    if (rc) return rc;
    RhatPlan& r = a.r;
    acf_chunks(r.N, r.d, r.n, a.nchunk, a.per);
    const int64_t tile = (int64_t)2 * a.nchunk * ACF_TL * r.nd;
    a.tiles = (int)std::max<int64_t>(1, std::min<int64_t>(4, ((int64_t)1 << 24) / tile));
    rc = rhat_scratch(h, r, a.tiles * tile + (int64_t)a.tiles * ACF_TL * r.d, false);
    if (rc) return rc;
    if (h->rhat_side_pending) {
        HIPCHK(h, hipStreamWaitEvent(h->stream, h->rhat_side_ev, 0));
        h->rhat_side_pending = false;
    }
    a.part = h->d_scratch + r.need;
    a.out = a.part + a.tiles * tile;
    return DEMCZ_OK;
}

static int32_t acf_enqueue(demcz_handle* h, const AcfPlan& a, int64_t lag_from, int64_t lag_to, double* sums)
{
    const RhatPlan& r = a.r;
    const unsigned gx = (unsigned)((r.nd + ACF_BS - 1) / ACF_BS);
    for (int64_t t = lag_from; t <= lag_to; t += (int64_t)a.tiles * ACF_TL) {
        const int64_t nl = std::min<int64_t>((int64_t)a.tiles * ACF_TL, lag_to - t + 1);
        const unsigned nz = (unsigned)((nl + ACF_TL - 1) / ACF_TL);
        hipLaunchKernelGGL(acf_products_kernel, dim3(gx, 2 * a.nchunk, nz), dim3(ACF_BS), 0, h->stream, (const double*)h->dchain,
                           (const double*)r.mean_j, r.N, r.d, r.s0, r.n, a.nchunk, a.per, t, a.part);
        hipLaunchKernelGGL(acf_reduce_kernel, dim3(r.d, (unsigned)nl), dim3(256), 0, h->stream, (const double*)a.part, r.N, r.d, a.nchunk,
                           a.out, (int64_t)0);
        HIPCHK(h, hipGetLastError());
        HIPCHK(h, hipMemcpyAsync(sums + (size_t)r.d * (t - lag_from), a.out, (size_t)r.d * nl * sizeof(double), hipMemcpyDeviceToHost, h->stream));
    }
    return DEMCZ_OK;
}

extern "C" int32_t demcz_autocov_sums(demcz_handle* h, int64_t g_from, int64_t g_to, int64_t lag_from, int64_t lag_to, double* sums)
{
    if (!h || !sums) return DEMCZ_ERR_INVALID_ARGUMENT;
    AcfPlan a;
    int32_t rc = acf_prepare(h, g_from, g_to, a, "demcz_autocov_sums");
    if (rc) return rc;
    if (lag_from < 0 || lag_to < lag_from || lag_to > a.r.n - 1)
        return fail(h, DEMCZ_ERR_INVALID_ARGUMENT, "demcz_autocov_sums: 0 <= lag_from <= lag_to <= n - 1, n = half the window");
    rc = rhat_scratch(h, a.r, 0, true);
    if (rc) return rc;
    rc = acf_enqueue(h, a, lag_from, lag_to, sums);
    if (rc) return rc;
    SYNCCHK(h, h->stream);
    return DEMCZ_OK;
}

extern "C" int32_t demcz_ess_from_sums(int32_t d, int64_t m, int64_t n, int64_t nlags, const double* sums, const double* between,
                                       double* ess, double* tau, double* varplus, int64_t* pairs, int32_t* converged)
{
    if (d <= 0 || m < 1 || n < 2 || nlags < 1 || !sums || !between || !ess) return DEMCZ_ERR_INVALID_ARGUMENT;
    const double dn = (double)n, dm = (double)m, S = dm * dn;
    const double cap = S * std::log10(S), floor_tau = 1.0 / std::log10(S);
    const int64_t L = nlags - 1;
    for (int p = 0; p < d; ++p) {
        const double A0 = sums[p] / S;
        const double W = A0 * dn / (dn - 1.0);
        const double vp = A0 + between[p] / (dm - 1.0);
        double sum = 0.0, prev = 0.0;
        int64_t k = 0;
        int32_t conv = 0;
        for (; 2 * k + 1 <= L; ++k) {
            const double r0 = k ? 1.0 - (W - sums[p + (size_t)d * (2 * k)] / S) / vp : 1.0;
            const double r1 = 1.0 - (W - sums[p + (size_t)d * (2 * k + 1)] / S) / vp;
            double P = r0 + r1;
            if (!(P > 0.0)) {
                conv = 1;
                if (P != P) sum = P;
                break;
            }
            if (k && prev < P) P = prev;
            sum += P;
            prev = P;
        }
        const double t = -1.0 + 2.0 * sum;
        ess[p] = (t < floor_tau) ? cap : S / t;
        if (tau) tau[p] = t;
        if (varplus) varplus[p] = vp;
        if (pairs) pairs[p] = k;
        if (converged) converged[p] = conv;
    }
    return DEMCZ_OK;
}

extern "C" int32_t demcz_ess(demcz_handle* h, int64_t g_from, int64_t g_to, int64_t max_lag,
                             double* ess, double* tau, double* varplus, int64_t* pairs, int32_t* converged)
{
    if (!h || !ess) return DEMCZ_ERR_INVALID_ARGUMENT;
    if (h->comm && h->nranks > 1)
        return fail(h, DEMCZ_ERR_INVALID_ARGUMENT, "demcz_ess: on a sharded handle add demcz_autocov_sums and demcz_rhat_partial over the ranks "
                                                   "on the host and finish with demcz_ess_from_sums");
    AcfPlan a;
    int32_t rc = acf_prepare(h, g_from, g_to, a, "demcz_ess");
    if (rc) return rc;
    rc = rhat_scratch(h, a.r, 0, true);
    if (rc) return rc;
    const RhatPlan& r = a.r;
    const int d = r.d;
    const int64_t n = r.n, m = 2 * r.N;
    const int64_t L = (max_lag <= 0) ? n - 1 : std::min<int64_t>(n - 1, max_lag);
    hipLaunchKernelGGL(rhat_reduce_kernel, dim3(d), dim3(256), 0, h->stream, r.mean_j, r.s2_j, r.N, d, 0, (const double*)nullptr, 1.0, r.sums);
    hipLaunchKernelGGL(rhat_reduce_kernel, dim3(d), dim3(256), 0, h->stream, r.mean_j, r.s2_j, r.N, d, 1, (const double*)r.sums, (double)m, r.sums + d);
    HIPCHK(h, hipGetLastError());
    std::vector<double> between((size_t)d), sums;
    std::vector<int32_t> conv((size_t)d);
    HIPCHK(h, hipMemcpyAsync(between.data(), r.sums + d, (size_t)d * sizeof(double), hipMemcpyDeviceToHost, h->stream));
    const int64_t batch = (int64_t)a.tiles * ACF_TL;
    int64_t have = 0;
    for (;;) {
        const int64_t to = std::min<int64_t>(L, have + batch - 1);
        sums.resize((size_t)d * (to + 1));
        rc = acf_enqueue(h, a, have, to, sums.data() + (size_t)d * have);
        if (rc) { (void)hipStreamSynchronize(h->stream); return rc; }
        SYNCCHK(h, h->stream);
        have = to + 1;
        rc = demcz_ess_from_sums(d, m, n, have, sums.data(), between.data(), ess, tau, varplus, pairs, conv.data());
        if (rc) return fail(h, rc, "demcz_ess: finisher");
        if (have > L || std::all_of(conv.begin(), conv.end(), [](int32_t c) { return c == 1; })) break;
    }
    if (converged) std::copy(conv.begin(), conv.end(), converged);
    return DEMCZ_OK;
}
// ... 2298 lines not shown
}

extern "C" int32_t demcz_bridge_posterior_array(int32_t device_id, const double* chain, const double* log_obj, int64_t N, int32_t d,
                                                int64_t G, const double* mean, const double* L, demcz_handle** derived)
{
    if (derived) *derived = nullptr;
    if (!chain || !log_obj || !derived || !mean || !L) return DEMCZ_ERR_INVALID_ARGUMENT;
    return with_arrays(device_id, N, d, G, chain, log_obj, [&](demcz_handle* h) { return bridge_posterior_from(h, 1, G, mean, L, derived); });
}

extern "C" int32_t demcz_bridge_proposal(demcz_handle* h, int64_t Np, int64_t wp, uint64_t seed, const double* mean, const double* L,
                                         demcz_handle** logratio, demcz_handle** draws)
{
    if (logratio) *logratio = nullptr;
    if (draws) *draws = nullptr;
    NOT_DERIVED(h);
    if (!h || !logratio || !mean || !L) return DEMCZ_ERR_INVALID_ARGUMENT;
    DEADCHK(h);
    BridgeTarget t;
    int32_t rc = bridge_target_of(h, "demcz_bridge_proposal", t);
    if (rc) return rc;
    return bridge_proposal_from(h, h->cfg.d, t, Np, wp, seed, mean, L, logratio, draws);
}

extern "C" int32_t demcz_bridge_proposal_program(int32_t device_id, int32_t d, int64_t Np, int64_t wp, uint64_t seed, const double* mean,
                                                 const double* L, const char* source, const char* options, const double* data,
                                                 int64_t ndata, demcz_handle** logratio, demcz_handle** draws)
{
    if (logratio) *logratio = nullptr;
    if (draws) *draws = nullptr;
    if (!logratio || !mean || !L) return DEMCZ_ERR_INVALID_ARGUMENT;
    int32_t rc = demcz_bridge_check(d, source, options);
    if (rc) return rc;
    return with_arrays(device_id, 1, d, 1, nullptr, nullptr, [&](demcz_handle* h) {
        BridgeTarget t;
        int32_t r2 = bridge_target_program(h, d, source, options, data, ndata, "demcz_bridge_proposal_program", t);
        return r2 ? r2 : bridge_proposal_from(h, d, t, Np, wp, seed, mean, L, logratio, draws);
    });
}

extern "C" int32_t demcz_bridge_iterate(demcz_handle* post, int64_t g_from, int64_t g_to, demcz_handle* prop, int64_t gp_from,
                                        int64_t gp_to, double neff, double tol, int64_t max_iter, double* logml, int64_t* iterations,
                                        int32_t* converged, double* moments, int64_t* n_nan, demcz_handle** f2)
{
    if (f2) *f2 = nullptr;
    if (!post || !prop) return DEMCZ_ERR_INVALID_ARGUMENT;
    DEADCHK(post);
    DEADCHK(prop);
    BridgeResult res;
    int32_t rc = bridge_iterate_from(post, g_from, g_to, prop, gp_from, gp_to, neff, tol, max_iter, res, f2);
    if (rc) return rc;
    if (logml) *logml = res.logml;
    if (iterations) *iterations = res.iterations;
    if (converged) *converged = res.converged;
    if (moments) std::copy(res.moments, res.moments + 4, moments);
    if (n_nan) *n_nan = res.n_nan;
    return DEMCZ_OK;
}

extern "C" int32_t demcz_bridge(demcz_handle* h, int64_t g_from, int64_t g_to, uint64_t seed, double neff, double tol, int64_t max_iter,
                                double* logml, double* se_logml, int64_t* iterations, int32_t* converged, int64_t* n_post,
                                int64_t* n_prop, double* neff_used, int64_t* n_nan, double* ess_f2, double* mean_out, double* L_out)
{
    NOT_DERIVED(h);
    if (!h) return DEMCZ_ERR_INVALID_ARGUMENT;
    DEADCHK(h);
    int32_t rc = rank_refuse_sharded(h, "demcz_bridge");
    if (rc) return rc;
    BridgeTarget t;
    rc = bridge_target_of(h, "demcz_bridge", t);
    if (rc) return rc;
    const BridgeOut o{logml, se_logml, iterations, converged, n_post, n_prop, neff_used, n_nan, ess_f2, mean_out, L_out};
    return bridge_from(h, t, g_from, g_to, seed, neff, tol, max_iter, o);
}

extern "C" int32_t demcz_bridge_array(int32_t device_id, const double* chain, const double* log_obj, int64_t N, int32_t d, int64_t G,
                                      const char* source, const char* options, const double* data, int64_t ndata, uint64_t seed,
                                      double neff, double tol, int64_t max_iter, double* logml, double* se_logml, int64_t* iterations,
                                      int32_t* converged, int64_t* n_post, int64_t* n_prop, double* neff_used, int64_t* n_nan,
                                      double* ess_f2, double* mean_out, double* L_out)
{
    if (!chain || !log_obj) return DEMCZ_ERR_INVALID_ARGUMENT;
    int32_t rc = demcz_bridge_check(d, source, options);
    if (rc) return rc;
    const BridgeOut o{logml, se_logml, iterations, converged, n_post, n_prop, neff_used, n_nan, ess_f2, mean_out, L_out};
    return with_arrays(device_id, N, d, G, chain, log_obj, [&](demcz_handle* h) {
        BridgeTarget t;
        int32_t r2 = bridge_target_program(h, d, source, options, data, ndata, "demcz_bridge_array", t);
        return r2 ? r2 : bridge_from(h, t, 1, G, seed, neff, tol, max_iter, o);
    });
}

extern "C" int32_t demcz_get_info(const demcz_handle* h, int64_t* M, int64_t* launches_window, int32_t* lanes_per_chain)
{
    NOT_DERIVED(h);
    if (!h) return DEMCZ_ERR_INVALID_ARGUMENT;
    if (M) *M = h->M_app;
    if (launches_window) *launches_window = h->launches;
    if (lanes_per_chain) *lanes_per_chain = h->prog_wave ? DEMCZ_LAYOUT_PROGRAM_WAVE : (h->split_kind == SPLIT_WAVE) ? DEMCZ_LAYOUT_SPLIT_WAVE : h->lanes;
    return DEMCZ_OK;
}

extern "C" int32_t demcz_selftest_draws(int32_t device_id, uint64_t seed, uint64_t chain, uint64_t blk0, int32_t n,
                                        uint64_t* words, double* normals, double* logu)
{
    if (n < 1 || !words || !normals || !logu) return DEMCZ_ERR_INVALID_ARGUMENT;
    int ndev = 0;
    if (hipGetDeviceCount(&ndev) != hipSuccess || ndev < 1)
        return fail(nullptr, DEMCZ_ERR_NO_DEVICE, "demcz_selftest_draws: no HIP device visible");
    if (hipSetDevice(device_id) != hipSuccess) return fail(nullptr, DEMCZ_ERR_HIP, "hipSetDevice failed");
    uint64_t* dw = nullptr; double* dn = nullptr; double* dl = nullptr;
    int32_t rc = DEMCZ_OK;
    if (hipMalloc((void**)&dw, (size_t)n * 16) != hipSuccess || hipMalloc((void**)&dn, (size_t)n * 16) != hipSuccess ||
        hipMalloc((void**)&dl, (size_t)n * 8) != hipSuccess) {
        rc = fail(nullptr, DEMCZ_ERR_HIP, "demcz_selftest_draws: hipMalloc failed");
    } else {
        hipLaunchKernelGGL(selftest_draws_kernel, dim3((unsigned)((n + 63) / 64)), dim3(64), 0, 0, seed, chain, blk0, (int)n, dw, dn, dl);
        if (hipMemcpy(words, dw, (size_t)n * 16, hipMemcpyDeviceToHost) != hipSuccess ||
            hipMemcpy(normals, dn, (size_t)n * 16, hipMemcpyDeviceToHost) != hipSuccess ||
            hipMemcpy(logu, dl, (size_t)n * 8, hipMemcpyDeviceToHost) != hipSuccess)
            rc = fail(nullptr, DEMCZ_ERR_HIP, "demcz_selftest_draws: kernel or copy failed");
    }
    if (dw) (void)hipFree(dw);
    if (dn) (void)hipFree(dn);
    if (dl) (void)hipFree(dl);
    return rc;
}

#ifdef DEMCZ_STAMPS
extern "C" int32_t demcz_debug_read_stamps(demcz_handle* h, unsigned long long* out, int64_t n_wg)
{
    NOT_DERIVED(h);
    if (!h || !out || n_wg < 0 || n_wg > DEMCZ_STAMP_WGS || !h->d_stamps) return DEMCZ_ERR_INVALID_ARGUMENT;
    SYNCCHK(h, h->stream);
    HIPCHK(h, hipMemcpy(out, h->d_stamps, (size_t)n_wg * 16 * sizeof(unsigned long long), hipMemcpyDeviceToHost));
    return DEMCZ_OK;
}
#endif

static int32_t run_checked_body(demcz_handle* h, int64_t g_from, int64_t g_to, double gamma, const double* temperature,
                                int64_t every, double threshold, int64_t* g_stop, int32_t* n_checks,
                                double* rhat_max, int32_t n_max, double* rhat_last)
{
    const int d = h->cfg.d;
    int32_t checks = 0;
    int64_t g = g_from;
    if (g_stop) *g_stop = g_to;
    const bool monitor = !(threshold > 0.0);
    const int64_t max_checks = (g_to - g_from + 1) / every + 2;
    HIPCHK(h, hipSetDevice(h->cfg.device_id));
    if (max_checks * d > h->pinned_cap) {
        { int32_t rcq = quiesce_all(h); if (rcq) return rcq; }
        SYNCCHK(h, h->stream);
        if (h->pinned_rhat) (void)host_free(h->pinned_rhat);
        h->pinned_rhat = nullptr; h->pinned_cap = 0;
        const int64_t cap = std::max<int64_t>(max_checks, 1024) * d;
        HIPCHK(h, host_malloc((void**)&h->pinned_rhat, (size_t)cap * sizeof(double)));
        h->pinned_cap = cap;
    }
    double* pinned = h->pinned_rhat;
    auto max_of = [d](const double* r) {
        double mx = r[0];
        for (int p = 1; p < d; ++p) mx = (r[p] > mx || r[p] != r[p]) ? r[p] : mx;
        return mx;
    };
    int32_t rc = DEMCZ_OK;
    const bool speculate = !monitor && !h->comm && h->lag == 0 && !h->external_append && !temperature;
    const int64_t N = h->cfg.N;
    if (speculate) {
        if (!h->d_spec_X) HIPCHK(h, dev_malloc(h->cfg.device_id, (void**)&h->d_spec_X, (size_t)N * d * sizeof(double)));
        if (!h->d_spec_lp) HIPCHK(h, dev_malloc(h->cfg.device_id, (void**)&h->d_spec_lp, (size_t)N * sizeof(double)));
        if (!h->spec_ev) HIPCHK(h, hipEventCreateWithFlags(&h->spec_ev, hipEventDisableTiming));
    }
    bool ahead = false;
    const bool grouped = monitor && !h->comm && h->lag == 0 && !h->external_append;
    int64_t max_slabs = 1;
    if (grouped && h->cfg.Gcap > 0) {
        const int64_t need1 = rhat_need(N * d, d, rhat_chunks(every / 2));
        const int64_t ls0 = live_span(h);
        max_slabs = std::max<int64_t>(1, std::min<int64_t>(std::min<int64_t>(SLAB_GROUP_MAX, ((int64_t)1 << 25) / need1), (ls0 > 0 ? ls0 : h->cfg.Gcap) / every + 1));
        rc = ensure_scratch(h, max_slabs * (need1 + d));
    }
    auto cut_now = [h]() {
        int64_t cut = 0;
        if (h->live_fault_polls != 0) cut = h->live_fault_g;
        if (h->no_live && h->rearm_from >= 0 && (cut == 0 || h->rearm_from + 1 < cut)) cut = h->rearm_from + 1;
        return cut;
    };
    while (g <= g_to && rc == DEMCZ_OK) {
        int64_t nxt = std::min(g_to, slab_end_at_or_after(g, every));
        RunHints hints;
        if (grouped) {
            const int64_t ls = live_span(h);
            const int64_t span = ls > 0 ? ls : INT64_MAX;
            nxt = slab_group_end(g, g_to, every, span, cut_now(), max_slabs);
            hints.bracket_slabs = (int32_t)(slab_ends_in(g, nxt, every) + (nxt % every != 0 ? 1 : 0));
            hints.next_ngen = nxt < g_to ? std::min<int64_t>(span, slab_group_end(nxt + 1, g_to, every, span, cut_now(), max_slabs) - nxt) : 0;
        }
        if (!ahead) rc = run_call(h, g, nxt, gamma, temperature ? temperature + (g - g_from) : nullptr, hints);
        ahead = false;
        if (rc) break;
        int64_t c0 = slab_end_at_or_after(g, every);
        while (c0 <= nxt && c0 - every < h->g0) c0 += every;
        const int64_t nck = c0 <= nxt ? (nxt - c0) / every + 1 : 0;
        if (nck > 0) {
            double* slot = pinned + (size_t)checks * d;
            rc = rhat_enqueue(h, c0 - every + 1, c0, slot, monitor && nxt < g_to, (int)nck);
            if (rc) break;
            checks += (int32_t)nck;
            if (!monitor) {
                int64_t M_before = 0;
                if (speculate && nxt < g_to) {
                    if (hipEventRecord(h->spec_ev, h->stream) != hipSuccess) { rc = fail(h, DEMCZ_ERR_HIP, "demcz_run_checked: event failed"); break; }
                    if (hipMemcpyAsync(h->d_spec_X, h->dX, (size_t)N * d * sizeof(double), hipMemcpyDeviceToDevice, h->stream) != hipSuccess ||
                        hipMemcpyAsync(h->d_spec_lp, h->dlp, (size_t)N * sizeof(double), hipMemcpyDeviceToDevice, h->stream) != hipSuccess) {
                        rc = fail(h, DEMCZ_ERR_HIP, "demcz_run_checked: snapshot failed");
                        break;
                    }
                    M_before = h->M_app;
                    const int64_t nn = std::min(g_to, slab_end_at_or_after(nxt + 1, every));
                    rc = demcz_run(h, nxt + 1, nn, gamma, nullptr);
                    if (rc) break;
                    ahead = true;
                    if ((rc = sync_event(h, h->spec_ev, "demcz_run_checked")) != DEMCZ_OK) break;
                } else if ((rc = sync_stream(h, h->stream, "demcz_run_checked")) != DEMCZ_OK) {
                    break;
                }
                if (max_of(slot) < threshold) {
                    if (g_stop) *g_stop = nxt;
                    if (ahead) {
                        if ((rc = sync_stream(h, h->stream, "demcz_run_checked")) != DEMCZ_OK) break;
                        rc = check_live_err(h);
                        if (rc) break;
                        if (hipMemcpyAsync(h->dX, h->d_spec_X, (size_t)N * d * sizeof(double), hipMemcpyDeviceToDevice, h->stream) != hipSuccess ||
                            hipMemcpyAsync(h->dlp, h->d_spec_lp, (size_t)N * sizeof(double), hipMemcpyDeviceToDevice, h->stream) != hipSuccess) {
                            rc = fail(h, DEMCZ_ERR_HIP, "demcz_run_checked: restore failed");
                            break;
                        }
                        const size_t rest = (size_t)(h->M_app - M_before) * (size_t)h->ZS;
                        if (rest > 0) {
                            hipLaunchKernelGGL(fill_u64_kernel, dim3((unsigned)((rest + 255) / 256)), dim3(256), 0, h->stream,
                                               reinterpret_cast<unsigned long long*>(h->dZ + (size_t)M_before * h->ZS), rest, LIVE_SENTINEL);
                            if (hipGetLastError() != hipSuccess) { rc = fail(h, DEMCZ_ERR_HIP, "demcz_run_checked: restore failed"); break; }
                        }
                        const int64_t s_lo = nxt - h->g0, s_hi = std::min<int64_t>(h->g_done - h->g0, h->cfg.Gcap);
                        if (s_hi > s_lo &&
                            (hipMemsetAsync(h->dchain + (size_t)N * d * s_lo, 0, (size_t)N * d * (s_hi - s_lo) * sizeof(double), h->stream) != hipSuccess ||
                             hipMemsetAsync(h->dlogobj + (size_t)N * s_lo, 0, (size_t)N * (s_hi - s_lo) * sizeof(double), h->stream) != hipSuccess)) {
                            rc = fail(h, DEMCZ_ERR_HIP, "demcz_run_checked: restore failed");
                            break;
                        }
                        if (h->hs_on) { h->after_launch_ev = nullptr; rc = stream_history(h, nxt + 1, h->g_done); if (rc) break; }
                        h->M_app = M_before;
                        h->M = M_before;
                        h->g_done = nxt;
                        if ((rc = rec_scrub(h)) != DEMCZ_OK) break;
                        if (!h->live_log.empty() && h->live_log.back().g_from == nxt + 1) h->live_log.pop_back();
                        while (!h->acc_log.empty() && h->acc_log.back().g_last > nxt) h->acc_log.pop_back();
                    }
                    break;
                }
            }
        }
        g = nxt + 1;
    }
    h->pinned_err_launches = -1;
    if (rc == DEMCZ_OK && !h->live_log.empty() && h->peer_mode != 2) {
        if (!h->pinned_err && host_malloc((void**)&h->pinned_err, 4 * sizeof(unsigned int)) != hipSuccess) { h->pinned_err = nullptr; (void)hipGetLastError(); }
        if (h->pinned_err && hipMemcpyAsync(h->pinned_err, h->d_live_err, 4 * sizeof(unsigned int), hipMemcpyDeviceToHost, h->stream) == hipSuccess)
            h->pinned_err_launches = h->launches;
    }
    if (rc == DEMCZ_OK) rc = sync_stream(h, h->stream, "demcz_run_checked");
    if (rc == DEMCZ_OK && h->diag_stream) rc = sync_stream(h, h->diag_stream, "demcz_run_checked");
    if (rc == DEMCZ_OK && h->prod_stream) rc = sync_stream(h, h->prod_stream, "demcz_run_checked");
    if (rc == DEMCZ_OK && h->comm_stream) rc = sync_stream(h, h->comm_stream, "demcz_run_checked");
    if (rc == DEMCZ_OK) {
        for (int32_t i = 0; i < checks; ++i)
            if (rhat_max && i < n_max) rhat_max[i] = max_of(pinned + (size_t)i * d);
        if (rhat_last && checks > 0) std::copy(pinned + (size_t)(checks - 1) * d, pinned + (size_t)checks * d, rhat_last);
        if (n_checks) *n_checks = checks;
    }
    return rc;
}

extern "C" int32_t demcz_run_checked(demcz_handle* h, int64_t g_from, int64_t g_to, double gamma, const double* temperature,
                                     int64_t every, double threshold, int64_t* g_stop, int32_t* n_checks,
                                     double* rhat_max, int32_t n_max, double* rhat_last)
{
    NOT_DERIVED(h);
    if (!h) return DEMCZ_ERR_INVALID_ARGUMENT;
    DEADCHK(h);
    if (every < 4 || g_from < 1 || g_to < g_from) return fail(h, DEMCZ_ERR_INVALID_ARGUMENT, "demcz_run_checked: need every >= 4 and 1 <= g_from <= g_to");
    if (!h->has_state) return fail(h, DEMCZ_ERR_STATE, "demcz_run_checked: call demcz_set_state first");
    if (h->peer_mode == 1 || h->peer_mode == 3) return fail(h, DEMCZ_ERR_STATE, "demcz_run_checked: replica groups and host-mediated peers are driven call by call (demcz_run, demcz_rhat_partial)");
    HIPCHK(h, hipSetDevice(h->cfg.device_id));
    int32_t rc = live_verify(h);
    if (rc) return rc;
    if (h->no_live && h->rearm_from >= g_from) h->rearm_from = g_from - 1;
    const bool pacing = (getenv("DEMCZ_NO_HOST_PACING") == nullptr);
    for (;;) {
        h->host_paced = pacing;
        h->in_checked = true;
        rc = run_checked_body(h, g_from, g_to, gamma, temperature, every, threshold, g_stop, n_checks, rhat_max, n_max, rhat_last);
        h->host_paced = false;
        h->in_checked = false;
        if (h->live_log.empty()) break;
        if (rc != DEMCZ_OK && h->peer_mode == 2) break;
        bool failed = false;
        { int32_t rcf = live_failed(h, failed); if (rcf) { rc = rcf; break; } }
        if (!failed) { h->live_log.clear(); break; }
        std::vector<demcz_handle::RunCall> dropped;
        rc = live_rollback(h, dropped);
        if (rc) break;
        h->replaying = true;
    }
    h->replaying = false;
    return rc;
}

extern "C" int32_t demcz_set_live_spin_limit(demcz_handle* h, int32_t polls)
{
    NOT_DERIVED(h);
    if (!h || polls < 0) return DEMCZ_ERR_INVALID_ARGUMENT;
    h->live_spin_limit = (unsigned int)polls;
    return DEMCZ_OK;
}

extern "C" int32_t demcz_set_live_rearms(demcz_handle* h, int32_t n)
{
    NOT_DERIVED(h);
    if (!h || n < 0) return DEMCZ_ERR_INVALID_ARGUMENT;
    h->live_rearms_left = n;
    if (h->peer_mode == 1 && h->group) {
        h->group->rearms_left = n;
        for (demcz_handle* m : h->group->members) m->live_rearms_left = n;
    }
    if (n == 0) h->rearm_from = -1;
    return DEMCZ_OK;
}

extern "C" int32_t demcz_get_live_rearms(const demcz_handle* h, int32_t* rearms, int32_t* left)
{
    NOT_DERIVED(h);
    if (!h) return DEMCZ_ERR_INVALID_ARGUMENT;
    if (rearms) *rearms = h->live_rearms;
    if (left) *left = h->live_rearms_left;
    return DEMCZ_OK;
}

extern "C" int32_t demcz_debug_set_live_fault(demcz_handle* h, int32_t polls, int64_t g_from)
{
    NOT_DERIVED(h);
    if (!h || polls < -1 || g_from < 0) return DEMCZ_ERR_INVALID_ARGUMENT;
    h->live_fault_polls = polls;
    h->live_fault_g = g_from;
    return DEMCZ_OK;
}

extern "C" int32_t demcz_debug_kernel_counts(const demcz_handle* h, int64_t* counts)
{
    NOT_DERIVED(h);
    if (!h || !counts) return DEMCZ_ERR_INVALID_ARGUMENT;
    const bool wave = h->lanes == DEMCZ_LAYOUT_SPLIT && h->split_kind == SPLIT_WAVE;
    counts[0] = h->kernel_counts[0];
    counts[1] = wave ? h->launches - h->kernel_counts[0] : 0;
    counts[2] = wave ? 0 : h->launches;
    return DEMCZ_OK;
}

extern "C" int32_t demcz_debug_kernel_name(const demcz_handle* h, char* buf, int32_t cap)
{
    NOT_DERIVED(h);
    if (!h || !buf || cap < 1) return DEMCZ_ERR_INVALID_ARGUMENT;
    const int d = h->cfg.d;
    const char* tg = h->cfg.target_kind == DEMCZ_TARGET_MVNORMAL ? "MVNORMAL" : h->cfg.target_kind == DEMCZ_TARGET_ISO_QUAD ? "ISO_QUAD"
                     : h->cfg.target_kind == DEMCZ_TARGET_LINREG_SSE ? "LINREG_SSE" : h->cfg.target_kind == DEMCZ_TARGET_PROGRAM ? "PROGRAM" : "HOST";
    const WindowKernel k = h->last_kernel.threads ? h->last_kernel : window_kernel_of(h, launch_facts(h, nullptr, false));
    const char* lv = k.live ? "true" : "false";
    const char* tm = k.temper ? "true" : "false";
    char tmp[160];
    switch (k.arm) {
    case ARM_LR8S: snprintf(tmp, sizeof tmp, "window_kernel_lr8s<%d, %s>", d, lv); break;
    case ARM_PROGRAM_WAVE: snprintf(tmp, sizeof tmp, "%s<%d, %d, %s, %s> (program)", d <= 5 ? "window_kernel_ps" : "window_kernel_pw", (int)TARGET_PROGRAM, d, lv, tm); break;
    case ARM_PS: snprintf(tmp, sizeof tmp, "window_kernel_ps<%s, %d, %s, %s>", tg, d, lv, tm); break;
    case ARM_PS2: snprintf(tmp, sizeof tmp, "window_kernel_ps2<%s, %d, %s, %s>", tg, d, lv, tm); break;
    case ARM_PS2D: snprintf(tmp, sizeof tmp, "window_kernel_ps2d<%s, %d, %s, %s>", tg, d, lv, tm); break;
    case ARM_PW:
        snprintf(tmp, sizeof tmp, "window_kernel_pw<%s, %d, %s, %s%s>", tg, d, lv, tm,
                 k.pw_form == PW_FORM_MATRIX ? ", true" : k.pw_form == PW_FORM_REGULAR ? ", false, true" : "");
        break;
    case ARM_MLB_REC:
        if (h->mlb_qb > 0 && h->split_lanes == 16) snprintf(tmp, sizeof tmp, "window_kernel_mlb<%s, %d, %d, true, %s, %d>", tg, d, h->split_lanes, lv, h->mlb_qb);
        else snprintf(tmp, sizeof tmp, "window_kernel_mlb<%s, %d, %d, true, %s>", tg, d, h->split_lanes, lv);
        break;
    case ARM_LR16_REC: snprintf(tmp, sizeof tmp, "window_kernel_lr16<%d, true, %s>", d, lv); break;
    case ARM_ML_REC: snprintf(tmp, sizeof tmp, "window_kernel_ml<%s, %d, 16, true, %s>", tg, d, lv); break;
    case ARM_PC8: snprintf(tmp, sizeof tmp, "window_kernel_pc8<%s, %d, %s, %s>", tg, d, lv, tm); break;
    case ARM_MLB: snprintf(tmp, sizeof tmp, "window_kernel_mlb<%s, %d, %d>", tg, d, h->lanes); break;
    case ARM_LR16: snprintf(tmp, sizeof tmp, "window_kernel_lr16<%d, false, false>", d); break;
    case ARM_ML_COOP: snprintf(tmp, sizeof tmp, "window_kernel_ml<%s, %d, %d, false, false, true>", tg, d, h->lanes); break;
    case ARM_ML: snprintf(tmp, sizeof tmp, "window_kernel_ml<%s, %d, %d>", tg, d, h->lanes); break;
    case ARM_SNOOKER:
        if (h->cfg.target_kind == DEMCZ_TARGET_PROGRAM) snprintf(tmp, sizeof tmp, "snooker_kernel<%d, %d> (program)", (int)TARGET_PROGRAM, d);
        else if (k.dyn_lds) snprintf(tmp, sizeof tmp, "snooker_kernel_generic<%s>", tg);
        else snprintf(tmp, sizeof tmp, "snooker_kernel<%s, %d>", tg, d);
        break;
    case ARM_ONE_LANE:
        if (h->cfg.target_kind == DEMCZ_TARGET_PROGRAM) snprintf(tmp, sizeof tmp, "window_kernel<%d, %d, %s> (program)", (int)TARGET_PROGRAM, d, h->full_block ? "true" : "false");
        else snprintf(tmp, sizeof tmp, "window_kernel<%s, %d, %s>", tg, d, h->full_block ? "true" : "false");
        break;
    }
    snprintf(buf, (size_t)cap, "demcz::%s", tmp);
    return DEMCZ_OK;
}

extern "C" int32_t demcz_get_live_status(const demcz_handle* h, int32_t* live_enabled, int32_t* redos)
{
    NOT_DERIVED(h);
    if (!h) return DEMCZ_ERR_INVALID_ARGUMENT;
    if (live_enabled) *live_enabled = (h->lanes == DEMCZ_LAYOUT_SPLIT && !h->no_live && h->live_claimed) ? 1 : 0;
    if (redos) *redos = h->live_redos;
    return DEMCZ_OK;
}

extern "C" int32_t demcz_debug_append_slab(demcz_handle* h, const double* slab, int32_t R, int32_t cnt, int32_t batched)
{
    NOT_DERIVED(h);
    if (!h || !slab || R < 1 || cnt < 1 || (!batched && cnt != 1)) return DEMCZ_ERR_INVALID_ARGUMENT;
    if (!h->has_state) return fail(h, DEMCZ_ERR_STATE, "demcz_debug_append_slab: no state");
    if (h->lag != 0 || !h->pending.empty()) return fail(h, DEMCZ_ERR_STATE, "demcz_debug_append_slab: rows are pending");
    const int64_t N = h->cfg.N, rows = N * R * cnt;
    const int d = h->cfg.d;
    if (h->M_app + rows > h->cfg.Mcap) return fail(h, DEMCZ_ERR_CAPACITY, "demcz_debug_append_slab: Z capacity exceeded");
    HIPCHK(h, hipSetDevice(h->cfg.device_id));
    int32_t rc = ensure_scratch(h, rows * d);
    if (rc) return rc;
    HIPCHK(h, hipMemcpyAsync(h->d_scratch, slab, (size_t)rows * d * sizeof(double), hipMemcpyHostToDevice, h->stream));
    const int64_t tot = rows * d;
    if (batched)
        hipLaunchKernelGGL(append_batch_kernel, dim3((unsigned)((tot + 255) / 256)), dim3(256), 0, h->stream, h->dZ, h->ZS,
                           h->M_app, (const double*)h->d_scratch, N, (int)R, (int)cnt, d);
    else
        hipLaunchKernelGGL(append_gathered_kernel, dim3((unsigned)((tot + 255) / 256)), dim3(256), 0, h->stream, h->dZ, h->ZS,
                           h->M_app, (const double*)h->d_scratch, N, (int)R, d);
    HIPCHK(h, hipGetLastError());
    SYNCCHK(h, h->stream);
    h->M_app += rows;
    h->M = h->M_app;
    rec_invalidate(h);
    return DEMCZ_OK;
}

extern "C" int32_t demcz_set_kernel_timing(demcz_handle* h, int32_t enabled)
{
    NOT_DERIVED(h);
    if (!h) return DEMCZ_ERR_INVALID_ARGUMENT;
    h->timing = enabled != 0;
    return DEMCZ_OK;
}

extern "C" int32_t demcz_get_kernel_time(demcz_handle* h, int64_t* launches, double* milliseconds)
{
    NOT_DERIVED(h);
    if (!h) return DEMCZ_ERR_INVALID_ARGUMENT;
    HIPCHK(h, hipSetDevice(h->cfg.device_id));
    SYNCCHK(h, h->stream);
    double total = 0.0;
    h->after_launch_ev = nullptr;
    h->series_start_ms.clear(); h->series_dur_ms.clear();
    for (auto& pr : h->timed) {
        float ms = 0.0f, st = 0.0f;
        HIPCHK(h, hipEventElapsedTime(&ms, pr.first, pr.second));
        if (&pr != &h->timed.front()) HIPCHK(h, hipEventElapsedTime(&st, h->timed.front().first, pr.first));
        const int32_t k = h->timed_slabs[(size_t)(&pr - &h->timed.front())];
        for (int32_t i = 0; i < k; ++i) { h->series_start_ms.push_back((double)st + i * ((double)ms / k)); h->series_dur_ms.push_back((double)ms / k); }
        total += ms;
    }
    for (auto& pr : h->timed) {
        (void)hipEventDestroy(pr.first);
        (void)hipEventDestroy(pr.second);
    }
    if (launches) *launches = h->timed_launches;
    if (milliseconds) *milliseconds = total;
    h->timed.clear();
    h->timed_slabs.clear();
    h->timed_launches = 0;
    return DEMCZ_OK;
}

extern "C" int32_t demcz_get_kernel_time_series(demcz_handle* h, int32_t cap, double* start_ms, double* duration_ms, int32_t* n)
{
    NOT_DERIVED(h);
    if (!h || cap < 0 || !n) return DEMCZ_ERR_INVALID_ARGUMENT;
    const int32_t m = (int32_t)std::min<size_t>(h->series_start_ms.size(), (size_t)cap);
    for (int32_t i = 0; i < m; ++i) {
        if (start_ms) start_ms[i] = h->series_start_ms[i];
        if (duration_ms) duration_ms[i] = h->series_dur_ms[i];
    }
    *n = (int32_t)h->series_start_ms.size();
    return DEMCZ_OK;
}
```

demc.jl_amd/csrc/demcz_kernels.h:

```cpp
#pragma once

#include "demcz_device.h"

#pragma clang fp contract(off)

#ifdef DEMCZ_STAMPS
#define DEMCZ_STAMP(P, i) do { if ((P).stamps && threadIdx.x == 0 && blockIdx.x < 65536u) (P).stamps[(size_t)blockIdx.x * 16 + (i)] = __builtin_readcyclecounter(); } while (0)
#else
#define DEMCZ_STAMP(P, i) do { } while (0)
#endif

namespace demcz {

enum { TARGET_MVNORMAL = 0, TARGET_ISO_QUAD = 1, TARGET_LINREG_SSE = 2, TARGET_HOST_CALLBACK = 3, TARGET_PROGRAM = 4 };

constexpr int MAX_D = 64;
constexpr int LINREG_PARTIALS = 16;
constexpr int WINDOW_BS = 64;

struct TargetParams {
    const double* mu;
    const double* Wp;
    double c0;
    const double* design;
// ... 376 lines not shown
            if (P.snap) {
#pragma unroll
                for (int p = 0; p < D; ++p) P.snap[nb * P.N * D + c + P.N * p] = x[p];
            }
            ++nb;
        }
    }
#pragma unroll
    for (int p = 0; p < D; ++p) P.Xcur[c + P.N * p] = x[p];
    P.lpcur[c] = lp;
    wave_store_counts(P, blockIdx.x, cnt_total, cnt_first);
}

template <int TARGET>
__global__ void __launch_bounds__(WINDOW_BS) window_kernel_generic(const WindowParams P)
{
    extern __shared__ double lds[];
    const int d = P.d;
    double* xs = lds;
    double* xps = lds + d * WINDOW_BS;
    double* zs = lds + 2 * d * WINDOW_BS;
    const int64_t c = (int64_t)blockIdx.x * WINDOW_BS + threadIdx.x;
    if (c >= P.N) return;
    const int tid = threadIdx.x;

    for (int p = 0; p < d; ++p) xs[p * WINDOW_BS + tid] = P.Xcur[c + P.N * p];
    double lp = P.lpcur[c];
    rng_state st;
    rng_seek(st, P.seed, (uint64_t)(P.chain_id0 + c), (uint64_t)(P.g_first - 1) * (uint64_t)P.S);
    int to_b = P.to_boundary;
    int64_t nb = 0;
    unsigned int cnt_total = 0, cnt_first = 0;
    const unsigned long long speak64 = __builtin_amdgcn_ballot_w64(true);

    for (int gi = 0; gi < P.ngen; ++gi) {
        const double lp_gen0 = lp;
        for (int ib = 0; ib < P.Nblocks; ++ib) {
            uint64_t r1, r2, i1, i2;
            rng_next(st, r1, r2);
            draw_rows(r1, r2, (uint64_t)P.M, i1, i2);
            const int b = P.block_offsets[ib + 1] - P.block_offsets[ib];
            const int nn = (b == 1) ? 1 : b;
            const int npairs = (nn + 1) / 2;
            for (int pr = 0; pr < npairs; ++pr) {
                rng_next(st, r1, r2);
                double z0, z1;
                normal_pair(r1, r2, z0, z1);
                zs[(2 * pr) * WINDOW_BS + tid] = z0;
                zs[(2 * pr + 1) * WINDOW_BS + tid] = z1;
            }
            const double scale = (b == 1) ? P.gamma : P.gamma / sqrt((double)(2 * b));
            const int32_t* so = P.slot_of + ib * d;
            const double* za = P.Z + (int64_t)i1 * P.ZS;
            const double* zb = P.Z + (int64_t)i2 * P.ZS;
            for (int p = 0; p < d; ++p) {
                const int t = so[p];
                double xv = xs[p * WINDOW_BS + tid];
                if (t >= 0) {
                    double diff = za[p] - zb[p];
                    double zt = zs[((b == 1) ? 0 : t) * WINDOW_BS + tid];
                    double t1 = scale * diff;
                    double t2 = P.eps[p] * zt;
                    double delta = t1 + t2;
                    xv = xv + delta;
                }
                xps[p * WINDOW_BS + tid] = xv;
            }
            rng_next(st, r1, r2);
            const double logu = dm_log(u_open(r1));
            const double lpp = target_logp<TARGET, 0>(P.tp, d, [&](int j) { return xps[j * WINDOW_BS + tid]; });
            double dlt = lpp - lp;
            if (P.temperature) dlt = dlt / P.temperature[gi];
            if (logu < dlt) {
                for (int p = 0; p < d; ++p) xs[p * WINDOW_BS + tid] = xps[p * WINDOW_BS + tid];
                lp = lpp;
            }
        }
        {
            const unsigned int k = wave_count_changed(lp, lp_gen0, speak64);
            cnt_total += k;
            cnt_first = (gi == 0) ? k : cnt_first;
        }
        const int64_t slot = P.slot_first + gi;
        if (P.chain) {
            for (int p = 0; p < d; ++p) P.chain[c + P.N * (p + (int64_t)d * slot)] = xs[p * WINDOW_BS + tid];
            P.logobj[c + P.N * slot] = lp;
        }
        if (--to_b == 0) {
            to_b = P.K;
            for (int p = 0; p < d; ++p) {
                const double xv = xs[p * WINDOW_BS + tid];
                if (P.do_append) P.Zw[(P.M_append + nb * P.N + c) * P.ZS + p] = xv;
                if (P.snap) P.snap[nb * P.N * d + c + P.N * p] = xv;
            }
            ++nb;
        }
    }
    for (int p = 0; p < d; ++p) P.Xcur[c + P.N * p] = xs[p * WINDOW_BS + tid];
    P.lpcur[c] = lp;
    wave_store_counts(P, blockIdx.x, cnt_total, cnt_first);
}

template <int TARGET>
__global__ void logp_kernel(TargetParams tp, int d, const double* X, int64_t ldX, int64_t n, double* out)
{
    const int64_t c = (int64_t)blockIdx.x * blockDim.x + threadIdx.x;
    if (c >= n) return;
    out[c] = target_logp<TARGET, 0>(tp, d, [&](int j) { return X[c + ldX * j]; });
}

#ifndef DEMCZ_NO_AUX_KERNELS
__global__ void fill_u64_kernel(unsigned long long* p, size_t n, unsigned long long v)
{
    const size_t i = (size_t)blockIdx.x * blockDim.x + threadIdx.x;
    if (i < n) p[i] = v;
}

__global__ void append_rows_kernel(double* Z, int64_t ZS, int64_t M, const double* rows, int64_t nrows,
                                   int64_t ldrows, int d)
{
    const int64_t i = (int64_t)blockIdx.x * blockDim.x + threadIdx.x;
    if (i >= nrows * d) return;
    const int64_t r = i % nrows, p = i / nrows;
    Z[(M + r) * ZS + p] = rows[r + ldrows * p];
}

__global__ void export_rows_kernel(const double* Z, int64_t ZS, int64_t r0, double* out, int64_t nrows, int64_t ldout, int d)
{
    const int64_t i = (int64_t)blockIdx.x * blockDim.x + threadIdx.x;
    if (i >= nrows * d) return;
    const int64_t r = i % nrows, p = i / nrows;
    out[r + ldout * p] = Z[(r0 + r) * ZS + p];
}

__global__ void append_gathered_kernel(double* Z, int64_t ZS, int64_t M, const double* slab, int64_t n_loc,
                                       int R, int d)
{
    const int64_t i = (int64_t)blockIdx.x * blockDim.x + threadIdx.x;
    const int64_t per = n_loc * d;
    if (i >= per * R) return;
    const int64_t r = i / per, rem = i % per, p = rem / n_loc, j = rem % n_loc;
    Z[(M + r * n_loc + j) * ZS + p] = slab[i];
}

__global__ void append_batch_kernel(double* Z, int64_t ZS, int64_t base, const double* slab, int64_t n_loc, int R, int cnt, int d)
{
    const int64_t i = (int64_t)blockIdx.x * blockDim.x + threadIdx.x;
    const int64_t per = n_loc * d;
    if (i >= per * cnt * R) return;
    const int64_t r = i / (per * cnt), rem = i % (per * cnt), sidx = rem / per, rem2 = rem % per, p = rem2 / n_loc, j = rem2 % n_loc;
    Z[(base + (sidx * R + r) * n_loc + j) * ZS + p] = slab[i];
}

__global__ void rhat_moments_kernel(const double* chain, int64_t N, int d, int64_t s0, int64_t n, int nchunk,
                                    double* S1, double* S2, int64_t w, int64_t slice)
{
    const int64_t i = (int64_t)blockIdx.x * blockDim.x + threadIdx.x;
    if (i >= N * d) return;
    s0 += (int64_t)blockIdx.z * w;
    S1 += (int64_t)blockIdx.z * slice;
    S2 += (int64_t)blockIdx.z * slice;
    const int h = blockIdx.y / nchunk, ck = blockIdx.y % nchunk;
    const int64_t per = (n + nchunk - 1) / nchunk;
    const int64_t t0 = ck * per, t1 = (t0 + per < n) ? t0 + per : n;
    const int64_t stride = N * d;
    const double* base = chain + i + stride * (s0 + h * n);
    const double x0 = base[0];
    double a = 0.0, b = 0.0;
    int64_t t = t0;
    for (; t + 8 <= t1; t += 8) {
        double v[8];
#pragma unroll
        for (int u = 0; u < 8; ++u) v[u] = base[stride * (t + u)];
#pragma unroll
        for (int u = 0; u < 8; ++u) {
            const double w = v[u] - x0;
            a += w;
            b = fma(w, w, b);
        }
    }
    for (; t < t1; ++t) {
        double v = base[stride * t] - x0;
        a += v;
        b = fma(v, v, b);
    }
    const int64_t o = i + stride * blockIdx.y;
    S1[o] = a;
    S2[o] = b;
}

__global__ void rhat_chainstats_kernel(const double* chain, int64_t N, int d, int64_t s0, int64_t n, int nchunk,
                                       const double* S1, const double* S2, double* mean_j, double* s2_j, int64_t w, int64_t slice)
{
    const int64_t i = (int64_t)blockIdx.x * blockDim.x + threadIdx.x;
    if (i >= N * d) return;
    s0 += (int64_t)blockIdx.z * w;
    S1 += (int64_t)blockIdx.z * slice;
    S2 += (int64_t)blockIdx.z * slice;
    mean_j += (int64_t)blockIdx.z * slice;
    s2_j += (int64_t)blockIdx.z * slice;
    const int h = blockIdx.y;
    const int64_t stride = N * d;
    const double x0 = chain[i + stride * (s0 + h * n)];
    double a = 0.0, b = 0.0;
    for (int ck = 0; ck < nchunk; ++ck) {
        a += S1[i + stride * (h * nchunk + ck)];
        b += S2[i + stride * (h * nchunk + ck)];
    }
    const double nn = (double)n;
    mean_j[i + stride * h] = x0 + a / nn;
    s2_j[i + stride * h] = (b - a * a / nn) / (nn - 1.0);
}

__global__ void __launch_bounds__(256) rhat_reduce_kernel(const double* mean_j, const double* s2_j, int64_t N, int d,
                                                          int stage, const double* grand, double grand_div, double* out)
{
    __shared__ double ra[256], rb[256];
    const int p = blockIdx.x;
    const int64_t stride = N * d;
    double a = 0.0, b = 0.0;
    const double gm = stage ? grand[p] / grand_div : 0.0;
    int64_t h = 0, c = threadIdx.x;
    while (c >= N) { c -= N; ++h; }
    for (int64_t k = threadIdx.x; k < 2 * N; k += 256) {
        const int64_t at = c + N * p + stride * h;
        const double mj = mean_j[at];
        if (stage == 0) {
            a += mj;
        } else {
            const double dv = mj - gm;
            a = fma(dv, dv, a);
            b += s2_j[at];
        }
        c += 256;
        while (c >= N) { c -= N; ++h; }
    }
    ra[threadIdx.x] = a;
    rb[threadIdx.x] = b;
    __syncthreads();
    for (int s = 128; s > 0; s >>= 1) {
        if ((int)threadIdx.x < s) {
            ra[threadIdx.x] += ra[threadIdx.x + s];
            rb[threadIdx.x] += rb[threadIdx.x + s];
        }
        __syncthreads();
    }
    if (threadIdx.x == 0) {
        out[p] = ra[0];
        if (stage) out[d + p] = rb[0];
    }
}

__global__ void __launch_bounds__(256) rhat_tail_kernel(const double* mean_j, const double* s2_j, int64_t N, int d,
                                                        double n, double m, double* rhat, int64_t slice)
{
    __shared__ double ra[256], rb[256];
    const int p = blockIdx.x;
    mean_j += (int64_t)blockIdx.y * slice;
    s2_j += (int64_t)blockIdx.y * slice;
    rhat += (int64_t)blockIdx.y * d;
    const int64_t stride = N * d;
    double a = 0.0, b = 0.0;
    int64_t h0 = 0, c0 = threadIdx.x;
    while (c0 >= N) { c0 -= N; ++h0; }
    {
        int64_t h = h0, c = c0;
        for (int64_t k = threadIdx.x; k < 2 * N; k += 256) {
            a += mean_j[c + N * p + stride * h];
            c += 256;
            while (c >= N) { c -= N; ++h; }
        }
    }
    ra[threadIdx.x] = a;
    __syncthreads();
    for (int s = 128; s > 0; s >>= 1) {
        if ((int)threadIdx.x < s) ra[threadIdx.x] += ra[threadIdx.x + s];
        __syncthreads();
    }
    const double gm = ra[0] / m;
    __syncthreads();
    a = 0.0;
    {
        int64_t h = h0, c = c0;
        for (int64_t k = threadIdx.x; k < 2 * N; k += 256) {
            const int64_t at = c + N * p + stride * h;
            const double dv = mean_j[at] - gm;
            a = fma(dv, dv, a);
            b += s2_j[at];
            c += 256;
            while (c >= N) { c -= N; ++h; }
        }
    }
    ra[threadIdx.x] = a;
    rb[threadIdx.x] = b;
    __syncthreads();
    for (int s = 128; s > 0; s >>= 1) {
        if ((int)threadIdx.x < s) {
            ra[threadIdx.x] += ra[threadIdx.x + s];
            rb[threadIdx.x] += rb[threadIdx.x + s];
        }
        __syncthreads();
    }
    if (threadIdx.x == 0) {
        const double B = n / (m - 1.0) * ra[0];
        const double W = rb[0] / m;
        const double varhat = (n - 1.0) / n * W + B / n;
        rhat[p] = sqrt(varhat / W);
    }
}

__global__ void rhat_final_kernel(const double* in, int d, double n, double m, double* rhat)
{
    const int p = blockIdx.x * blockDim.x + threadIdx.x;
    if (p >= d) return;
    const double B = n / (m - 1.0) * in[p];
    const double W = in[d + p] / m;
    const double varhat = (n - 1.0) / n * W + B / n;
    rhat[p] = sqrt(varhat / W);
}

__global__ void __launch_bounds__(256) changed_from_history_kernel(const double* logobj, const double* lp_origin, int64_t N,
                                                                   int64_t s_from, long long* out)
{
    __shared__ int cnt[256];
    const int64_t s = s_from + blockIdx.x;
    const double* cur = logobj + N * s;
    const double* prev = (s == 0) ? lp_origin : logobj + N * (s - 1);
    int k = 0;
    for (int64_t c = threadIdx.x; c < N; c += 256) k += ((cur[c] - prev[c]) != 0.0) ? 1 : 0;
    cnt[threadIdx.x] = k;
    __syncthreads();
    for (int st = 128; st > 0; st >>= 1) {
        if ((int)threadIdx.x < st) cnt[threadIdx.x] += cnt[threadIdx.x + st];
        __syncthreads();
    }
    if (threadIdx.x == 0) out[blockIdx.x] = cnt[0];
}

__global__ void __launch_bounds__(64) changed_per_chain_kernel(const double* logobj, int64_t N, int64_t s0, int64_t w, int nchunk,
                                                               unsigned int* cnt)
{
    const int64_t c = (int64_t)blockIdx.x * 64 + threadIdx.x;
    if (c >= N) return;
    const int64_t per = (w - 1 + nchunk - 1) / nchunk;
    const int64_t t0 = 1 + (int64_t)blockIdx.y * per, t1 = (t0 + per < w) ? t0 + per : w;
    if (t0 >= t1) return;
    unsigned int k = 0;
    double prev = logobj[c + N * (s0 + t0 - 1)];
    for (int64_t t = t0; t < t1; ++t) {
        const double cur = logobj[c + N * (s0 + t)];
        k += ((cur - prev) != 0.0) ? 1u : 0u;
        prev = cur;
    }
    atomicAdd(&cnt[c], k);
}

__global__ void changed_ratio_kernel(const unsigned int* cnt, int64_t N, int64_t w, double* ratio)
{
    const int64_t c = (int64_t)blockIdx.x * blockDim.x + threadIdx.x;
    if (c < N) ratio[c] = (double)cnt[c] / (double)(w - 1);
}

constexpr int MC_TS = 8;
constexpr int MC_VALS = MC_TS * MC_TS + MC_TS;

__global__ void __launch_bounds__(256) meancov_partial_kernel(const double* chain, int64_t N, int d, int64_t s0, int64_t w, int nchunk,
                                                              double* partial)
{
    __shared__ double red[4][MC_VALS];
    const int T = (d + MC_TS - 1) / MC_TS;
    int I = 0, J = (int)blockIdx.z;
    while (J >= T - I) { J -= T - I; ++I; }
    J += I;
    const int64_t c = (int64_t)blockIdx.x * 256 + threadIdx.x;
    const int64_t per = (w + nchunk - 1) / nchunk;
    const int64_t t0 = (int64_t)blockIdx.y * per, t1 = (t0 + per < w) ? t0 + per : w;
    const int64_t stride = N * d;
    double acc[MC_TS][MC_TS], sm[MC_TS];
#pragma unroll
    for (int a = 0; a < MC_TS; ++a) {
        sm[a] = 0.0;
#pragma unroll
        for (int b = 0; b < MC_TS; ++b) acc[a][b] = 0.0;
    }
    if (c < N) {
        double ri[MC_TS], rj[MC_TS];
#pragma unroll
        for (int a = 0; a < MC_TS; ++a) {
            ri[a] = (I * MC_TS + a < d) ? chain[N * (I * MC_TS + a) + stride * s0] : 0.0;
            rj[a] = (J * MC_TS + a < d) ? chain[N * (J * MC_TS + a) + stride * s0] : 0.0;
        }
        for (int64_t t = t0; t < t1; ++t) {
            const double* base = chain + c + stride * (s0 + t);
            double xi[MC_TS], xj[MC_TS];
#pragma unroll
            for (int a = 0; a < MC_TS; ++a) {
                xi[a] = (I * MC_TS + a < d) ? base[N * (I * MC_TS + a)] - ri[a] : 0.0;
                xj[a] = (J * MC_TS + a < d) ? base[N * (J * MC_TS + a)] - rj[a] : 0.0;
            }
#pragma unroll
            for (int a = 0; a < MC_TS; ++a) {
                sm[a] += xi[a];
#pragma unroll
                for (int b = 0; b < MC_TS; ++b) acc[a][b] = fma(xi[a], xj[b], acc[a][b]);
            }
        }
    }
    const int lane = threadIdx.x & 63, wv = threadIdx.x >> 6;
#pragma unroll
    for (int a = 0; a < MC_TS; ++a) {
#pragma unroll
        for (int b = 0; b <= MC_TS; ++b) {
            double v = (b < MC_TS) ? acc[a][b] : sm[a];
#pragma unroll
            for (int off = 32; off > 0; off >>= 1) v += __shfl_down(v, off, 64);
            if (lane == 0) red[wv][(b < MC_TS) ? a * MC_TS + b : MC_TS * MC_TS + a] = v;
        }
    }
    __syncthreads();
    if (threadIdx.x < MC_VALS) {
        const double v = ((red[0][threadIdx.x] + red[1][threadIdx.x]) + red[2][threadIdx.x]) + red[3][threadIdx.x];
        const size_t blk = ((size_t)blockIdx.z * gridDim.y + blockIdx.y) * gridDim.x + blockIdx.x;
        partial[blk * MC_VALS + threadIdx.x] = v;
    }
}

__global__ void meancov_final_kernel(const double* partial, int d, int nblk_xy, double* out)
{
    const int e = blockIdx.x * blockDim.x + threadIdx.x;
    if (e >= d * (d + 1)) return;
    const int p = e % d, q = e / d;
    const int T = (d + MC_TS - 1) / MC_TS;
    int lo = p, hi = (q < d) ? q : p;
    bool swap = false;
    if (q < d && q / MC_TS < p / MC_TS) { lo = q; hi = p; swap = true; }
    const int I = lo / MC_TS, J = (q < d) ? hi / MC_TS : I;
    int z = 0;
    for (int i = 0; i < I; ++i) z += T - i;
    z += J - I;
    int idx;
    if (q == d) idx = MC_TS * MC_TS + p % MC_TS;
    else idx = swap ? (q % MC_TS) * MC_TS + p % MC_TS : (p % MC_TS) * MC_TS + q % MC_TS;
    double a = 0.0;
    for (int b = 0; b < nblk_xy; ++b) a += partial[((size_t)z * nblk_xy + b) * MC_VALS + idx];
    out[e] = a;
}

__global__ void selftest_draws_kernel(uint64_t seed, uint64_t chain, uint64_t blk0, int n, uint64_t* words,
                                      double* normals, double* logu)
{
    const int i = blockIdx.x * blockDim.x + threadIdx.x;
    if (i >= n) return;
    rng_state st;
    rng_seek(st, seed, chain, blk0 + (uint64_t)i);
    uint64_t r1, r2;
    rng_next(st, r1, r2);
    words[2 * i] = r1;
    words[2 * i + 1] = r2;
    double z0, z1;
    normal_pair(r1, r2, z0, z1);
    normals[2 * i] = z0;
    normals[2 * i + 1] = z1;
    logu[i] = dm_log(u_open(r1));
}
#endif

}
```

demc.jl_amd/engine.py:

```python
from __future__ import annotations

import ctypes as C
from collections import namedtuple

import numpy as np

from . import _lib
from ._lib import DemczError
from .targets import is_device_target

ESS = namedtuple("ESS", "ess tau varplus pairs converged")


def ess_from_sums(m, n, sums, between):
    sums = _lib.f64(sums, "F")
    d, nlags = sums.shape
    between = _lib.f64(between)
    if between.shape != (d,):
        raise ValueError("between must have d entries")
    out = ESS(np.empty(d), np.empty(d), np.empty(d), np.zeros(d, dtype=np.int64), np.zeros(d, dtype=np.int32))
    rc = _lib.load().demcz_ess_from_sums(d, int(m), int(n), nlags, _lib.ptr(sums), _lib.ptr(between), _lib.ptr(out.ess), _lib.ptr(out.tau),
                                         _lib.ptr(out.varplus), _lib.ptr(out.pairs, _lib._lp), _lib.ptr(out.converged, _lib._ip))
    if rc != 0:
        raise DemczError(rc, "demcz_ess_from_sums: d >= 1, n >= 2, nlags >= 1")
# ... 562 lines not shown

    def __del__(self):
        try:
            self.close()
        except Exception:
            pass

    def bridge_posterior(self, g_from, g_to, mean, L):
        mean, L = _bridge_ml(mean, L, self.d)
        out = C.c_void_p()
        self._chk(self._L.demcz_bridge_posterior(self._h, int(g_from), int(g_to), _lib.ptr(mean), _lib.ptr(L), C.byref(out)))
        return DerivedHistory(self._L, out, self.N, 1, int(g_from), int(g_to), ["a1"], self.chain_id0)

    def bridge_proposal(self, Np, wp, mean, L, seed=None, want_draws=False):
        mean, L = _bridge_ml(mean, L, self.d)
        seed = bridge_seed(self.seed) if seed is None else int(seed) & (2**64 - 1)
        a2, xs = C.c_void_p(), C.c_void_p()
        self._chk(self._L.demcz_bridge_proposal(self._h, int(Np), int(wp), seed, _lib.ptr(mean), _lib.ptr(L), C.byref(a2),
                                                C.byref(xs) if want_draws else None))
        ha = DerivedHistory(self._L, a2, int(Np), 1, 1, int(wp), ["a2"])
        return (ha, DerivedHistory(self._L, xs, int(Np), self.d, 1, int(wp), getattr(self, "names", None))) if want_draws else ha

    def bridge(self, g_from, g_to, seed=None, neff="auto", tol=1e-10, max_iter=1000):
        g_from, g_to = int(g_from), int(g_to)
        if isinstance(neff, str):
            if neff != "auto":
                raise ValueError('neff must be a number, None or "auto"')
            w = g_to - g_from + 1
            ne = float(np.median(self.ess(g_from + w // 2, g_to).ess)) if w >= 8 else 0.0
            ne = ne if np.isfinite(ne) and ne > 0 else 0.0
        else:
            ne = 0.0 if neff is None else float(neff)
        seed = bridge_seed(self.seed) if seed is None else int(seed) & (2**64 - 1)
        o = _bridge_outputs(self.d)
        self._chk(self._L.demcz_bridge(self._h, g_from, g_to, seed, ne, float(tol), int(max_iter), *_bridge_out_args(o)))
        return _bridge_record(o)

    def set_state(self, X, logp, Z):
        X = _lib.f64(X, "F")
        Z = _lib.f64(Z, "F")
        if X.shape != (self.N, self.d) or Z.ndim != 2 or Z.shape[1] != self.d:
            raise ValueError("X must be N x d and Z must be M0 x d")
        lp = _lib.f64(logp) if logp is not None else None
        if lp is not None and lp.shape != (self.N,):
            raise ValueError("logp must have N entries")
        self._chk(self._L.demcz_set_state(self._h, _lib.ptr(X), _lib.ptr(lp), _lib.ptr(Z), Z.shape[0], Z.shape[0]))

    def get_state(self, with_Z=True):
        X = np.empty((self.N, self.d), order="F")
        lp = np.empty(self.N)
        M = C.c_int64()
        self._chk(self._L.demcz_get_state(self._h, _lib.ptr(X), _lib.ptr(lp), None, 0, C.byref(M)))
        Z = None
        if with_Z:
            pz, Mz = C.c_void_p(), C.c_int64()
            self._chk(self._L.demcz_get_archive_pinned(self._h, C.byref(pz), C.byref(Mz)))
            buf = (C.c_double * (Mz.value * self.d)).from_address(pz.value)
            buf._owner = _PinnedOwner(self._L, [pz.value])
            Z = np.ctypeslib.as_array(buf).reshape((Mz.value, self.d), order="F")
        return X, lp, Z, int(M.value)

    @property
    def M(self):
        M = C.c_int64()
        self._chk(self._L.demcz_get_info(self._h, C.byref(M), None, None))
        return int(M.value)

    def info(self):
        M, nl, lanes = C.c_int64(), C.c_int64(), C.c_int32()
        self._chk(self._L.demcz_get_info(self._h, C.byref(M), C.byref(nl), C.byref(lanes)))
        return dict(M=int(M.value), window_launches=int(nl.value), lanes_per_chain=int(lanes.value))

    def set_append_lag(self, batches):
        self._chk(self._L.demcz_set_append_lag(self._h, int(batches)))

    def set_rng_offset(self, generations):
        self._chk(self._L.demcz_set_rng_offset(self._h, int(generations)))

    def set_snooker(self, every, gamma=(1.2, 2.2)):
        lo, hi = gamma
        self._chk(self._L.demcz_set_snooker(self._h, C.c_int32(int(every)), C.c_double(float(lo)), C.c_double(float(hi))))

    @property
    def snooker(self):
        ev, lo, hi, n = C.c_int32(0), C.c_double(0.0), C.c_double(0.0), C.c_int64(0)
        self._chk(self._L.demcz_get_snooker(self._h, C.byref(ev), C.byref(lo), C.byref(hi), C.byref(n)))
        return int(ev.value), float(lo.value), float(hi.value), int(n.value)

    def set_history_origin(self, g0):
        self._chk(self._L.demcz_set_history_origin(self._h, int(g0)))

    def run(self, g_from, g_to, gamma, temperature=None):
        t = None
        if temperature is not None:
            t = _lib.f64(temperature)
            if t.shape != (g_to - g_from + 1,):
                raise ValueError("one temperature per generation")
        self._chk(self._L.demcz_run(self._h, int(g_from), int(g_to), float(gamma), _lib.ptr(t)))

    def run_checked(self, g_from, g_to, gamma, every, threshold=0.0, temperature=None):
        t = None
        if temperature is not None:
            t = _lib.f64(temperature)
            if t.shape != (g_to - g_from + 1,):
                raise ValueError("one temperature per generation")
        n_max = int((g_to - g_from + 1) // every + 2)
        mx = np.zeros(n_max)
        last = np.full(self.d, np.nan)
        g_stop, n = C.c_int64(0), C.c_int32(0)
        self._chk(self._L.demcz_run_checked(self._h, C.c_int64(int(g_from)), C.c_int64(int(g_to)), C.c_double(float(gamma)),
                                            _lib.ptr(t), C.c_int64(int(every)), C.c_double(float(threshold)), C.byref(g_stop),
                                            C.byref(n), _lib.ptr(mx), C.c_int32(n_max), _lib.ptr(last)))
        return int(g_stop.value), mx[:n.value].copy(), last

    def set_kernel_timing(self, enabled: bool):
        self._chk(self._L.demcz_set_kernel_timing(self._h, C.c_int32(1 if enabled else 0)))

    def get_kernel_time(self):
        n, ms = C.c_int64(0), C.c_double(0.0)
        self._chk(self._L.demcz_get_kernel_time(self._h, C.byref(n), C.byref(ms)))
        return int(n.value), float(ms.value)

    def get_kernel_time_series(self):
        n = C.c_int32(0)
        self._chk(self._L.demcz_get_kernel_time_series(self._h, 0, None, None, C.byref(n)))
        st, du = np.zeros(n.value), np.zeros(n.value)
        self._chk(self._L.demcz_get_kernel_time_series(self._h, n.value, _lib.ptr(st), _lib.ptr(du), C.byref(n)))
        return st, du

    def set_live_spin_limit(self, polls: int):
        self._chk(self._L.demcz_set_live_spin_limit(self._h, C.c_int32(int(polls))))

    def debug_set_live_fault(self, polls: int, g_from: int = 0):
        self._chk(self._L.demcz_debug_set_live_fault(self._h, C.c_int32(int(polls)), C.c_int64(int(g_from))))

    def live_status(self):
        on, redos = C.c_int32(0), C.c_int32(0)
        self._chk(self._L.demcz_get_live_status(self._h, C.byref(on), C.byref(redos)))
        return bool(on.value), int(redos.value)

    def set_live_rearms(self, n: int):
        self._chk(self._L.demcz_set_live_rearms(self._h, C.c_int32(int(n))))

    def live_rearms(self):
        a, b = C.c_int32(0), C.c_int32(0)
        self._chk(self._L.demcz_get_live_rearms(self._h, C.byref(a), C.byref(b)))
        return int(a.value), int(b.value)

    def kernel_counts(self):
        c = (C.c_int64 * 3)()
        self._chk(self._L.demcz_debug_kernel_counts(self._h, c))
        return dict(zip(("ps2", "ps_general", "other"), (int(v) for v in c)))

    def kernel_name(self):
        buf = C.create_string_buffer(192)
        self._chk(self._L.demcz_debug_kernel_name(self._h, buf, 192))
        return buf.value.decode()

    def synchronize(self):
        self._chk(self._L.demcz_synchronize(self._h))

    def get_history(self, g_from, g_to, chain=True, log_obj=True, out=None):
        G = g_to - g_from + 1
        if out is not None and chain and log_obj:
            ch_full, lo_full = out
            ok = (ch_full.flags.f_contiguous and lo_full.flags.f_contiguous and ch_full.shape[:2] == (self.N, self.d)
                  and lo_full.shape[0] == self.N and ch_full.shape[2] >= G and lo_full.shape[1] >= G
                  and ch_full.dtype == np.float64 and lo_full.dtype == np.float64)
            if ok:
                self._chk(self._L.demcz_get_history(self._h, int(g_from), int(g_to), _lib.ptr(ch_full), _lib.ptr(lo_full)))
                return ch_full[:, :, :G], lo_full[:, :G]
        ch = np.empty((self.N, self.d, G), order="F") if chain else None
        lo = np.empty((self.N, G), order="F") if log_obj else None
        self._chk(self._L.demcz_get_history(self._h, int(g_from), int(g_to), _lib.ptr(ch), _lib.ptr(lo)))
        return ch, lo

    def history_stream(self, enabled=True):
        self._chk(self._L.demcz_history_stream(self._h, 1 if enabled else 0))
        self._streaming = bool(enabled)

    def take_history(self, g_from, g_to):
        G = g_to - g_from + 1
        pc, pl = C.c_void_p(), C.c_void_p()
        self._chk(self._L.demcz_get_history_view(self._h, int(g_from), int(g_to), C.byref(pc), C.byref(pl)))
        bc, bl = C.c_void_p(), C.c_void_p()
        self._chk(self._L.demcz_detach_history(self._h, C.byref(bc), C.byref(bl)))
        self._streaming = False
        owner = _PinnedOwner(self._L, [bc.value, bl.value])
        cbuf = (C.c_double * (self.N * self.d * G)).from_address(pc.value)
        lbuf = (C.c_double * (self.N * G)).from_address(pl.value)
        cbuf._owner = owner
        lbuf._owner = owner
        chain = np.ctypeslib.as_array(cbuf).reshape((self.N, self.d, G), order="F")
        lobj = np.ctypeslib.as_array(lbuf).reshape((self.N, G), order="F")
        return chain, lobj

    def get_changed(self, g_from, g_to):
        out = np.zeros(g_to - g_from + 1, dtype=np.int64)
        self._chk(self._L.demcz_get_changed(self._h, int(g_from), int(g_to), _lib.ptr(out, _lib._lp)))
        return out

    def changed_total(self, g_from, g_to, with_source=False):
        tot, src = C.c_int64(0), C.c_int32(0)
        self._chk(self._L.demcz_get_changed_total(self._h, int(g_from), int(g_to), C.byref(tot), C.byref(src)))
        return (int(tot.value), bool(src.value)) if with_source else int(tot.value)

    def best(self, g_from, g_to):
        v, c, g = C.c_double(), C.c_int64(), C.c_int64()
        par = np.empty(self.d)
        self._chk(self._L.demcz_best(self._h, int(g_from), int(g_to), C.byref(v), C.byref(c), C.byref(g), _lib.ptr(par)))
        return Best(v.value, c.value, g.value, par)

    def accept_ratio(self, g_from, g_to):
        out = np.empty(self.N)
        self._chk(self._L.demcz_accept_ratio(self._h, int(g_from), int(g_to), _lib.ptr(out)))
        return out

    def closure_buffers(self):
        if getattr(self, "_hc", None) is None:
            px, pl = C.c_void_p(), C.c_void_p()
            self._chk(self._L.demcz_closure_buffers(self._h, C.byref(px), C.byref(pl)))
            bx = (C.c_double * (self.N * self.d)).from_address(px.value)
            bl = (C.c_double * self.N).from_address(pl.value)
            self._hc = (np.ctypeslib.as_array(bx).reshape((self.N, self.d), order="F"), np.ctypeslib.as_array(bl))
        return self._hc

    def propose(self, g, ib, gamma):
        if getattr(self, "_hc", None) is not None:
            self._chk(self._L.demcz_propose(self._h, int(g), int(ib), float(gamma), None))
            return self._hc[0]
        Xp = np.empty((self.N, self.d), order="F")
        self._chk(self._L.demcz_propose(self._h, int(g), int(ib), float(gamma), _lib.ptr(Xp)))
        return Xp

    def accept_commit(self, logp_prop=None, temperature=None):
        t = C.byref(C.c_double(float(temperature))) if temperature is not None else None
        tp = C.cast(t, _lib._dp) if t is not None else None
        hc = getattr(self, "_hc", None)
        if logp_prop is None or (hc is not None and logp_prop is hc[1]):
            if hc is None:
                raise ValueError("accept_commit() without values needs closure_buffers() first")
            self._chk(self._L.demcz_accept_commit(self._h, None, tp))
            return
        lp = _lib.f64(logp_prop)
        self._chk(self._L.demcz_accept_commit(self._h, _lib.ptr(lp), tp))

    def end_generation(self, g):
        self._chk(self._L.demcz_end_generation(self._h, int(g)))

    def comm_unique_id(self) -> bytes:
        buf = C.create_string_buffer(128)
        rc = self._L.demcz_comm_unique_id(buf)
        if rc != 0:
            raise DemczError(rc, (self._L.demcz_last_error(None) or b"").decode())
        return buf.raw

    def comm_init(self, unique_id: bytes, nranks: int, rank: int):
        buf = C.create_string_buffer(unique_id, 128)
        self._chk(self._L.demcz_comm_init(self._h, buf, int(nranks), int(rank)))

    @staticmethod
    def peer_group(engines):
        L = engines[0]._L
        arr = (C.c_void_p * len(engines))(*[e._h for e in engines])
        rc = L.demcz_peer_group(arr, len(engines))
        if rc != 0:
            msgs = [(L.demcz_last_error(e._h) or b"").decode() for e in engines]
            raise DemczError(rc, next((m for m in msgs if m), ""))

    def peer_export(self, nranks: int, rank: int) -> bytes:
        buf = C.create_string_buffer(64)
        self._chk(self._L.demcz_peer_export(self._h, int(nranks), int(rank), buf))
        return buf.raw

    def peer_attach(self, handles):
        blob = b"".join(handles)
        buf = C.create_string_buffer(blob, len(blob))
        self._chk(self._L.demcz_peer_attach(self._h, buf))

    def peer_detach(self):
        self._chk(self._L.demcz_peer_detach(self._h))

    def peer_ping(self):
        ok, us = C.c_int32(-1), C.c_double(0.0)
        self._chk(self._L.demcz_get_peer_ping(self._h, C.byref(ok), C.byref(us)))
        return int(ok.value), float(us.value)

    def peer_status(self):
        m, n = C.c_int32(0), C.c_int32(0)
        self._chk(self._L.demcz_get_peer_status(self._h, C.byref(m), C.byref(n)))
        return int(m.value), int(n.value)

    def set_comm_timeout(self, milliseconds: int):
        self._chk(self._L.demcz_set_comm_timeout(self._h, C.c_int64(int(milliseconds))))

    def debug_stall_exchange(self, milliseconds: int):
        self._chk(self._L.demcz_debug_stall_exchange(self._h, C.c_int32(int(milliseconds))))

    def set_external_append(self, enabled: bool):
        self._chk(self._L.demcz_set_external_append(self._h, 1 if enabled else 0))

    def append_rows(self, rows):
        rows = _lib.f64(rows, "F")
        if rows.ndim != 2 or rows.shape[1] != self.d:
            raise ValueError("rows must be nrows x d")
        self._chk(self._L.demcz_append_rows(self._h, _lib.ptr(rows), rows.shape[0], rows.shape[0]))
# ... 32 lines not shown
```

include/demcz.h:

```cpp
#ifndef DEMCZ_H
#define DEMCZ_H

#include <stdint.h>

#ifdef __cplusplus
extern "C" {
#endif

typedef struct demcz_handle demcz_handle;

enum demcz_status {
    DEMCZ_OK = 0,
    DEMCZ_ERR_INVALID_ARGUMENT = 1,
    DEMCZ_ERR_HIP = 2,
    DEMCZ_ERR_CAPACITY = 3,
    DEMCZ_ERR_STATE = 4,
    DEMCZ_ERR_NO_DEVICE = 5,
    DEMCZ_ERR_COMM = 6
};

enum demcz_target_kind {
    DEMCZ_TARGET_MVNORMAL = 0,
    DEMCZ_TARGET_ISO_QUAD = 1,
    DEMCZ_TARGET_LINREG_SSE = 2,
// ... 85 lines not shown
int32_t demcz_quantile_finish(int32_t d, int32_t nq, const uint64_t* key_lo, const uint64_t* key_hi, const double* frac,
                              const int64_t* nan_count, double* q, double* lower, double* upper);
int32_t demcz_quantiles(demcz_handle* h, int64_t g_from, int64_t g_to, int32_t nq, const double* probs,
                        double* q, double* lower, double* upper);

int32_t demcz_best(demcz_handle* h, int64_t g_from, int64_t g_to, double* bestval, int64_t* chain, int64_t* generation,
                   double* bestpar);

int32_t demcz_accept_ratio(demcz_handle* h, int64_t g_from, int64_t g_to, double* ratio);

int32_t demcz_mean_cov(demcz_handle* h, int64_t g_from, int64_t g_to, double* mean, double* cov);

int32_t demcz_propose(demcz_handle* h, int64_t g, int32_t ib, double gamma, double* Xprop);
int32_t demcz_closure_buffers(demcz_handle* h, double** Xprop, double** logp);
int32_t demcz_accept_commit(demcz_handle* h, const double* logp_prop, const double* temperature);
int32_t demcz_end_generation(demcz_handle* h, int64_t g);

int32_t demcz_comm_unique_id(void* unique_id_128B);
int32_t demcz_comm_init(demcz_handle* h, const void* unique_id_128B, int32_t nranks, int32_t rank);

int32_t demcz_peer_group(demcz_handle** handles, int32_t R);
int32_t demcz_get_peer_status(const demcz_handle* h, int32_t* mode, int32_t* peers);
int32_t demcz_peer_export(demcz_handle* h, int32_t nranks, int32_t rank, void* handle_64B);
int32_t demcz_peer_attach(demcz_handle* h, const void* handles_64B_each);
int32_t demcz_peer_detach(demcz_handle* h);
int32_t demcz_get_peer_ping(const demcz_handle* h, int32_t* ok, double* wait_us);

int32_t demcz_set_comm_timeout(demcz_handle* h, int64_t milliseconds);

int32_t demcz_export_current_device(demcz_handle* h, double* X_device);
int32_t demcz_append_rows_device(demcz_handle* h, const double* rows_device, int64_t nrows, int64_t ldrows);
int32_t demcz_append_rows(demcz_handle* h, const double* rows, int64_t nrows, int64_t ldrows);
int32_t demcz_set_external_append(demcz_handle* h, int32_t enabled);

int32_t demcz_set_append_lag(demcz_handle* h, int32_t batches);

int32_t demcz_set_rng_offset(demcz_handle* h, int64_t generations);

int32_t demcz_set_snooker(demcz_handle* h, int32_t every, double gamma_lo, double gamma_hi);
int32_t demcz_get_snooker(const demcz_handle* h, int32_t* every, double* gamma_lo, double* gamma_hi, int64_t* steps_launched);

int32_t demcz_rhat_array(int32_t device_id, const double* chain, int64_t N, int32_t d, int64_t G, double* rhat);
int32_t demcz_accept_ratio_array(int32_t device_id, const double* log_obj, int64_t N, int64_t G, double* ratio);
int32_t demcz_mean_cov_array(int32_t device_id, const double* chain, int64_t N, int32_t d, int64_t G, double* mean, double* cov);
int32_t demcz_autocov_sums_array(int32_t device_id, const double* chain, int64_t N, int32_t d, int64_t G,
                                 int64_t lag_from, int64_t lag_to, double* sums);
int32_t demcz_ess_array(int32_t device_id, const double* chain, int64_t N, int32_t d, int64_t G, int64_t max_lag,
                        double* ess, double* tau, double* varplus, int64_t* pairs, int32_t* converged);
int32_t demcz_quantiles_array(int32_t device_id, const double* chain, int64_t N, int32_t d, int64_t G, int32_t nq,
                              const double* probs, double* q, double* lower, double* upper);
int32_t demcz_best_array(int32_t device_id, const double* log_obj, int64_t N, int64_t G, double* bestval, int64_t* chain,
                         int64_t* column);

int32_t demcz_derive_check(int32_t d, int32_t m, const char* source, const char* options);
int32_t demcz_derive(demcz_handle* h, int64_t g_from, int64_t g_to, int32_t m, const char* source, const char* options,
                     const double* data, int64_t ndata, demcz_handle** derived);
int32_t demcz_derive_array(int32_t device_id, const double* chain, const double* log_obj ,
                           int64_t N, int32_t d, int64_t G, int32_t m, const char* source, const char* options,
                           const double* data, int64_t ndata, demcz_handle** derived);

#define DEMCZ_RANK_Z 0
#define DEMCZ_RANK_AVERAGE 1
int32_t demcz_rank_to_z(int64_t n, const double* r, int64_t S, double* z);
int32_t demcz_rank_normalize(demcz_handle* h, int64_t g_from, int64_t g_to, int32_t mode,
                             const double* center , demcz_handle** ranked);
int32_t demcz_rank_normalize_array(int32_t device_id, const double* chain, int64_t N, int32_t d, int64_t G,
                                   int32_t mode, const double* center, demcz_handle** ranked);
int32_t demcz_indicator_le(demcz_handle* h, int64_t g_from, int64_t g_to, int32_t nthr,
                           const double* thr , demcz_handle** derived);
int32_t demcz_rank_diagnostics(demcz_handle* h, int64_t g_from, int64_t g_to,
                               double* rhat_rank, double* ess_bulk, double* ess_tail);
int32_t demcz_rank_diagnostics_array(int32_t device_id, const double* chain, int64_t N, int32_t d, int64_t G,
                                     double* rhat_rank, double* ess_bulk, double* ess_tail);

int32_t demcz_histogram_edges(int32_t nbins, double lo, double hi, double* edges);
int32_t demcz_histogram(demcz_handle* h, int64_t g_from, int64_t g_to, int32_t nbins, const double* lo, const double* hi,
                        double* edges, int64_t* counts, int64_t* below, int64_t* above, int64_t* nan_count);
int32_t demcz_histogram_array(int32_t device_id, const double* chain, int64_t N, int32_t d, int64_t G, int32_t nbins,
                              const double* lo, const double* hi, double* edges, int64_t* counts, int64_t* below,
                              int64_t* above, int64_t* nan_count);
int32_t demcz_histogram2d(demcz_handle* h, int64_t g_from, int64_t g_to, int32_t npairs, const int32_t* pairs, int32_t nbx,
                          int32_t nby, const double* lo, const double* hi, double* edges_x, double* edges_y,
                          int64_t* counts, int64_t* outside);
int32_t demcz_histogram2d_array(int32_t device_id, const double* chain, int64_t N, int32_t d, int64_t G, int32_t npairs,
                                const int32_t* pairs, int32_t nbx, int32_t nby, const double* lo, const double* hi,
                                double* edges_x, double* edges_y, int64_t* counts, int64_t* outside);
int32_t demcz_hdi_steps(int64_t S, int32_t nprob, const double* probs, int64_t* steps);
int32_t demcz_hdi(demcz_handle* h, int64_t g_from, int64_t g_to, int32_t nprob, const double* probs, double* hdi);
int32_t demcz_hdi_array(int32_t device_id, const double* chain, int64_t N, int32_t d, int64_t G, int32_t nprob,
                        const double* probs, double* hdi);

int32_t demcz_pointwise_check(int32_t d, const char* source, const char* options);
int32_t demcz_pointwise(demcz_handle* h, int64_t g_from, int64_t g_to, int64_t obs_from, int32_t mc, const char* source,
                        const char* options, const double* data, int64_t ndata, demcz_handle** derived);
int32_t demcz_pointwise_array(int32_t device_id, const double* chain, int64_t N, int32_t d, int64_t G, int64_t obs_from,
                              int32_t mc, const char* source, const char* options, const double* data, int64_t ndata,
                              demcz_handle** derived);
int32_t demcz_psis_tail_length(int64_t S, double r_eff, int64_t* M);
int32_t demcz_gpd_fit(int64_t n, const double* x_ascending, double* k, double* sigma, double* khat);
int32_t demcz_loo_columns(demcz_handle* h, int64_t g_from, int64_t g_to, const double* r_eff ,
                          double* elpd_loo, double* pareto_k, int64_t* n_tail, double* lppd, double* p_waic);
int32_t demcz_loo_columns_array(int32_t device_id, const double* chain, int64_t N, int32_t d, int64_t G, const double* r_eff,
                                double* elpd_loo, double* pareto_k, int64_t* n_tail, double* lppd, double* p_waic);
int32_t demcz_loo(demcz_handle* h, int64_t g_from, int64_t g_to, int64_t nobs, const char* source, const char* options,
                  const double* data, int64_t ndata, const double* r_eff ,
                  double* elpd_loo, double* pareto_k, int64_t* n_tail, double* lppd, double* p_waic);
int32_t demcz_loo_array(int32_t device_id, const double* chain, int64_t N, int32_t d, int64_t G, int64_t nobs,
                        const char* source, const char* options, const double* data, int64_t ndata, const double* r_eff,
                        double* elpd_loo, double* pareto_k, int64_t* n_tail, double* lppd, double* p_waic);

int32_t demcz_bridge_check(int32_t d, const char* source, const char* options);
int32_t demcz_bridge_posterior(demcz_handle* h, int64_t g_from, int64_t g_to, const double* mean, const double* L,
                               demcz_handle** derived);
int32_t demcz_bridge_posterior_array(int32_t device_id, const double* chain, const double* log_obj, int64_t N, int32_t d,
                                     int64_t G, const double* mean, const double* L, demcz_handle** derived);
int32_t demcz_bridge_proposal(demcz_handle* h, int64_t Np, int64_t wp, uint64_t seed, const double* mean, const double* L,
                              demcz_handle** logratio, demcz_handle** draws );
int32_t demcz_bridge_proposal_program(int32_t device_id, int32_t d, int64_t Np, int64_t wp, uint64_t seed, const double* mean,
                                      const double* L, const char* source, const char* options, const double* data,
                                      int64_t ndata, demcz_handle** logratio, demcz_handle** draws );
int32_t demcz_bridge_iterate(demcz_handle* post, int64_t g_from, int64_t g_to, demcz_handle* prop, int64_t gp_from,
                             int64_t gp_to, double neff, double tol, int64_t max_iter, double* logml, int64_t* iterations,
                             int32_t* converged, double* moments , int64_t* n_nan,
                             demcz_handle** f2 );
int32_t demcz_bridge(demcz_handle* h, int64_t g_from, int64_t g_to, uint64_t seed, double neff, double tol, int64_t max_iter,
                     double* logml, double* se_logml, int64_t* iterations, int32_t* converged, int64_t* n_post,
                     int64_t* n_prop, double* neff_used, int64_t* n_nan, double* ess_f2, double* mean_out, double* L_out);
int32_t demcz_bridge_array(int32_t device_id, const double* chain, const double* log_obj, int64_t N, int32_t d, int64_t G,
                           const char* source, const char* options, const double* data, int64_t ndata, uint64_t seed,
                           double neff, double tol, int64_t max_iter, double* logml, double* se_logml, int64_t* iterations,
                           int32_t* converged, int64_t* n_post, int64_t* n_prop, double* neff_used, int64_t* n_nan,
                           double* ess_f2, double* mean_out, double* L_out);

int32_t demcz_get_info(const demcz_handle* h, int64_t* M, int64_t* launches_window, int32_t* lanes_per_chain);

int32_t demcz_run_checked(demcz_handle* h, int64_t g_from, int64_t g_to, double gamma, const double* temperature,
                          int64_t every, double threshold, int64_t* g_stop, int32_t* n_checks,
                          double* rhat_max, int32_t n_max, double* rhat_last);


int32_t demcz_set_kernel_timing(demcz_handle* h, int32_t enabled);
int32_t demcz_get_kernel_time(demcz_handle* h, int64_t* launches, double* milliseconds);

int32_t demcz_get_kernel_time_series(demcz_handle* h, int32_t cap, double* start_ms, double* duration_ms, int32_t* n);

int32_t demcz_selftest_draws(int32_t device_id, uint64_t seed, uint64_t chain, uint64_t blk0, int32_t n,
                             uint64_t* words, double* normals, double* logu);

int32_t demcz_set_live_spin_limit(demcz_handle* h, int32_t polls);
int32_t demcz_get_live_status(const demcz_handle* h, int32_t* live_enabled, int32_t* redos);
int32_t demcz_set_live_rearms(demcz_handle* h, int32_t n);
int32_t demcz_get_live_rearms(const demcz_handle* h, int32_t* rearms, int32_t* left);
int32_t demcz_debug_kernel_counts(const demcz_handle* h, int64_t* counts);
int32_t demcz_debug_kernel_name(const demcz_handle* h, char* buf, int32_t cap);

int32_t demcz_debug_set_live_fault(demcz_handle* h, int32_t polls, int64_t g_from);

int32_t demcz_debug_stall_exchange(demcz_handle* h, int32_t milliseconds);

int32_t demcz_debug_append_slab(demcz_handle* h, const double* slab, int32_t R, int32_t cnt, int32_t batched);

#ifdef __cplusplus
}
#endif
#endif
```

Measured before the change: 725.0 million.

## Fuse R-hat chainstats and tail into one LDS finish kernel with mapped output

```diff
diff --git a/demc.jl_amd/_lib.py b/demc.jl_amd/_lib.py
--- a/demc.jl_amd/_lib.py
+++ b/demc.jl_amd/_lib.py
@@ -36,7 +36,7 @@
     "demcz_debug_append_slab", "demcz_get_changed_total", "demcz_debug_set_live_fault",
     "demcz_set_comm_timeout", "demcz_debug_stall_exchange", "demcz_get_kernel_time_series",
     "demcz_history_stream", "demcz_get_history_view", "demcz_detach_history", "demcz_release_host_buffer", "demcz_get_archive_pinned",
-    "demcz_debug_kernel_counts", "demcz_pool_trim", "demcz_debug_kernel_name", "demcz_peer_group", "demcz_get_peer_status", "demcz_peer_export", "demcz_peer_attach",
+    "demcz_debug_kernel_counts", "demcz_debug_rhat_counts", "demcz_pool_trim", "demcz_debug_kernel_name", "demcz_peer_group", "demcz_get_peer_status", "demcz_peer_export", "demcz_peer_attach",
     "demcz_peer_detach", "demcz_get_peer_ping", "demcz_set_live_rearms", "demcz_get_live_rearms",
     "demcz_closure_buffers", "demcz_program_check", "demcz_set_program",
     "demcz_program_check_layout",
@@ -183,6 +183,7 @@
     L.demcz_set_live_spin_limit.argtypes = [C.c_void_p, C.c_int32]
     L.demcz_get_live_status.argtypes = [C.c_void_p, _ip, _ip]
     L.demcz_debug_kernel_counts.argtypes = [C.c_void_p, _lp]
+    L.demcz_debug_rhat_counts.argtypes = [C.c_void_p, _lp]
     L.demcz_history_stream.argtypes = [C.c_void_p, C.c_int32]
     L.demcz_get_history_view.argtypes = [C.c_void_p, C.c_int64, C.c_int64, C.POINTER(C.c_void_p), C.POINTER(C.c_void_p)]
     L.demcz_detach_history.argtypes = [C.c_void_p, C.POINTER(C.c_void_p), C.POINTER(C.c_void_p)]
diff --git a/demc.jl_amd/csrc/demcz_capi.hip b/demc.jl_amd/csrc/demcz_capi.hip
--- a/demc.jl_amd/csrc/demcz_capi.hip
+++ b/demc.jl_amd/csrc/demcz_capi.hip
@@ -1,5 +1,6 @@
 #include "../../include/demcz.h"
 #include "demcz_kernels.h"
+#include "demcz_kernels_rhat.h"
 #include "demcz_kernels_acf.h"
 #include "demcz_kernels_sel.h"
 #include "demcz_select_host.h"
@@ -246,6 +247,8 @@
     double* d_spec_lp = nullptr;
     hipEvent_t spec_ev = nullptr;
     double* pinned_rhat = nullptr;
+    double* pinned_rhat_dev = nullptr;
+    mutable int64_t rhat_counts[2] = {0, 0};
     unsigned int* pinned_err = nullptr;
     int64_t pinned_err_launches = -1;
     int64_t pinned_cap = 0;
@@ -656,7 +659,7 @@
     if (h->prod_gate) (void)hipEventDestroy(h->prod_gate);
     if (h->d_stage) (void)host_free(h->d_stage);
     for (auto& pr : h->timed) { (void)hipEventDestroy(pr.first); (void)hipEventDestroy(pr.second); }
-    if (h->pinned_rhat) (void)host_free(h->pinned_rhat);
+    if (h->pinned_rhat) (void)hipHostFree(h->pinned_rhat);
     if (h->pinned_err) (void)host_free(h->pinned_err);
     if (h->d_safe_X) (void)dev_free(h->cfg.device_id, h->d_safe_X);
     if (h->d_safe_lp) (void)dev_free(h->cfg.device_id, h->d_safe_lp);
@@ -2745,7 +2748,9 @@
     return DEMCZ_OK;
 }
 
-static int32_t rhat_scratch(demcz_handle* h, RhatPlan& r, int64_t extra, bool compute, hipStream_t qs = nullptr)
+static bool rhat_finish_fits(const RhatPlan& r) { return r.N <= RHAT_FINISH_MAX_N; }
+
+static int32_t rhat_scratch(demcz_handle* h, RhatPlan& r, int64_t extra, bool compute, hipStream_t qs = nullptr, bool finish = false)
 {
     HIPCHK(h, hipSetDevice(h->cfg.device_id));
     int32_t rc = ensure_scratch(h, r.need * r.slabs + (r.slabs > 1 ? (int64_t)r.slabs * r.d : 0) + extra);
@@ -2762,14 +2767,16 @@
         if (!qs) qs = h->stream;
         hipLaunchKernelGGL(rhat_moments_kernel, dim3(gx, 2 * r.nchunk, r.slabs), dim3(bs), 0, qs, h->dchain, r.N, r.d, r.s0, r.n, r.nchunk, r.S1, r.S2,
                            r.w, r.need);
-        hipLaunchKernelGGL(rhat_chainstats_kernel, dim3(gx, 2, r.slabs), dim3(bs), 0, qs, h->dchain, r.N, r.d, r.s0, r.n, r.nchunk, r.S1, r.S2, r.mean_j,
-                           r.s2_j, r.w, r.need);
+        if (!finish)
+            hipLaunchKernelGGL(rhat_chainstats_kernel, dim3(gx, 2, r.slabs), dim3(bs), 0, qs, h->dchain, r.N, r.d, r.s0, r.n, r.nchunk, r.S1, r.S2, r.mean_j,
+                               r.s2_j, r.w, r.need);
         HIPCHK(h, hipGetLastError());
     }
     return DEMCZ_OK;
 }
 
-static int32_t rhat_prepare(demcz_handle* h, int64_t g_from, int64_t g_to, RhatPlan& r, bool compute, hipStream_t qs = nullptr, int slabs = 1)
+static int32_t rhat_prepare(demcz_handle* h, int64_t g_from, int64_t g_to, RhatPlan& r, bool compute, hipStream_t qs = nullptr, int slabs = 1,
+                            bool may_finish = false)
 {
     int32_t rc = rhat_plan(h, g_from, g_to, r);
     if (rc) return rc;
@@ -2778,7 +2785,7 @@
         if (rc) return rc;
         r.slabs = slabs;
     }
-    return rhat_scratch(h, r, 0, compute, qs);
+    return rhat_scratch(h, r, 0, compute, qs, may_finish && rhat_finish_fits(r));
 }
 
 extern "C" int32_t demcz_rhat_partial(demcz_handle* h, int64_t g_from, int64_t g_to, int32_t stage, const double* grand, double* out)
@@ -2804,10 +2811,9 @@
     return DEMCZ_OK;
 }
 
-static int32_t rhat_enqueue(demcz_handle* h, int64_t g_from, int64_t g_to, double* out, bool side = false, int slabs = 1)
-{
-    RhatPlan r;
-    hipStream_t qs = h->stream;
+static int32_t rhat_side_gate(demcz_handle* h, bool side, hipStream_t& qs)
+{
+    qs = h->stream;
     static const bool own_env = getenv("DEMCZ_RHAT_OWN_STREAM") != nullptr;
     if (side && !h->comm && !own_env && h->prod_stream) {
         if (!h->diag_ev) HIPCHK(h, hipEventCreateWithFlags(&h->diag_ev, hipEventDisableTiming));
@@ -2841,6 +2847,12 @@
         }
         qs = h->diag_stream;
     }
+    return DEMCZ_OK;
+}
+
+static int32_t rhat_enqueue_on(demcz_handle* h, hipStream_t qs, int64_t g_from, int64_t g_to, double* out, int slabs = 1, double* out_dev = nullptr)
+{
+    RhatPlan r;
     if (qs == h->stream && h->rhat_side_pending) {
         HIPCHK(h, hipStreamWaitEvent(h->stream, h->rhat_side_ev, 0));
         h->rhat_side_pending = false;
@@ -2854,16 +2866,29 @@
         }
     } side_mark{h, qs};
     if (slabs > 1 && h->comm) return fail(h, DEMCZ_ERR_STATE, "demcz_run_checked: batched checks are for unsharded runs");
-    int32_t rc = rhat_prepare(h, g_from, g_to, r, true, qs, slabs);
+    const bool sharded = (h->comm != nullptr);
+    int32_t rc = rhat_prepare(h, g_from, g_to, r, true, qs, slabs, !sharded);
     if (rc) return rc;
     const int d = r.d;
     const int64_t n = r.n;
     const int64_t m = 2 * r.N * h->nranks;
-    const bool sharded = (h->comm != nullptr);
     double* sums = r.sums;
+    if (!sharded && rhat_finish_fits(r)) {
+        const size_t lds = (size_t)4 * r.N * sizeof(double);
+        if (lds + 2 * RHAT_TREE * sizeof(double) > 65536)
+            HIPCHK(h, hipFuncSetAttribute(reinterpret_cast<const void*>(&rhat_finish_kernel), hipFuncAttributeMaxDynamicSharedMemorySize,
+                                          (int)(4 * RHAT_FINISH_MAX_N * sizeof(double))));
+        hipLaunchKernelGGL(rhat_finish_kernel, dim3(d, r.slabs), dim3(RHAT_FINISH_BS), lds, qs, h->dchain, r.N, d, r.s0, r.n, r.nchunk, r.S1, r.S2,
+                           (double)m, out_dev ? out_dev : r.out, r.w, r.need);
+        HIPCHK(h, hipGetLastError());
+        h->rhat_counts[0] += r.slabs;
+        if (!out_dev) HIPCHK(h, hipMemcpyAsync(out, r.out, (size_t)r.slabs * d * sizeof(double), hipMemcpyDeviceToHost, qs));
+        return DEMCZ_OK;
+    }
     if (!sharded) {
         hipLaunchKernelGGL(rhat_tail_kernel, dim3(d, r.slabs), dim3(256), 0, qs, r.mean_j, r.s2_j, r.N, d, (double)n, (double)m, r.out, r.need);
         HIPCHK(h, hipGetLastError());
+        h->rhat_counts[1] += r.slabs;
         HIPCHK(h, hipMemcpyAsync(out, r.out, (size_t)r.slabs * d * sizeof(double), hipMemcpyDeviceToHost, qs));
         return DEMCZ_OK;
     }
@@ -2878,6 +2903,14 @@
     HIPCHK(h, hipGetLastError());
     HIPCHK(h, hipMemcpyAsync(out, sums + 3 * d, (size_t)d * sizeof(double), hipMemcpyDeviceToHost, qs));
     return DEMCZ_OK;
+}
+
+static int32_t rhat_enqueue(demcz_handle* h, int64_t g_from, int64_t g_to, double* out, bool side = false, int slabs = 1, double* out_dev = nullptr)
+{
+    hipStream_t qs = nullptr;
+    int32_t rc = rhat_side_gate(h, side, qs);
+    if (rc) return rc;
+    return rhat_enqueue_on(h, qs, g_from, g_to, out, slabs, out_dev);
 }
 
 extern "C" int32_t demcz_rhat(demcz_handle* h, int64_t g_from, int64_t g_to, double* rhat)
@@ -5482,13 +5515,20 @@
     if (max_checks * d > h->pinned_cap) {
         { int32_t rcq = quiesce_all(h); if (rcq) return rcq; }
         SYNCCHK(h, h->stream);
-        if (h->pinned_rhat) (void)host_free(h->pinned_rhat);
-        h->pinned_rhat = nullptr; h->pinned_cap = 0;
+        if (h->pinned_rhat) (void)hipHostFree(h->pinned_rhat);
+        h->pinned_rhat = h->pinned_rhat_dev = nullptr; h->pinned_cap = 0;
         const int64_t cap = std::max<int64_t>(max_checks, 1024) * d;
-        HIPCHK(h, host_malloc((void**)&h->pinned_rhat, (size_t)cap * sizeof(double)));
+        HIPCHK(h, hipHostMalloc((void**)&h->pinned_rhat, (size_t)cap * sizeof(double), hipHostMallocMapped));
+        if (hipHostGetDevicePointer((void**)&h->pinned_rhat_dev, h->pinned_rhat, 0) != hipSuccess) {
+            (void)hipGetLastError();
+            (void)hipHostFree(h->pinned_rhat);
+            h->pinned_rhat = h->pinned_rhat_dev = nullptr;
+            return fail(h, DEMCZ_ERR_HIP, "demcz_run_checked: no device address for the pinned statistics");
+        }
         h->pinned_cap = cap;
     }
     double* pinned = h->pinned_rhat;
+    double* const pinned_dev = h->pinned_rhat_dev;
     auto max_of = [d](const double* r) {
         double mx = r[0];
         for (int p = 1; p < d; ++p) mx = (r[p] > mx || r[p] != r[p]) ? r[p] : mx;
@@ -5517,6 +5557,13 @@
         if (h->no_live && h->rearm_from >= 0 && (cut == 0 || h->rearm_from + 1 < cut)) cut = h->rearm_from + 1;
         return cut;
     };
+    struct HeldCheck { bool on = false; hipStream_t qs = nullptr; int64_t g_from = 0, g_to = 0; double* slot = nullptr; double* slot_dev = nullptr; int nck = 0; } held;
+    static const bool rhat_first_env = getenv("DEMCZ_RHAT_FIRST") != nullptr;
+    auto flush_held = [&]() -> int32_t {
+        if (!held.on) return DEMCZ_OK;
+        held.on = false;
+        return rhat_enqueue_on(h, held.qs, held.g_from, held.g_to, held.slot, held.nck, held.slot_dev);
+    };
     while (g <= g_to && rc == DEMCZ_OK) {
         int64_t nxt = std::min(g_to, slab_end_at_or_after(g, every));
         RunHints hints;
@@ -5530,13 +5577,22 @@
         if (!ahead) rc = run_call(h, g, nxt, gamma, temperature ? temperature + (g - g_from) : nullptr, hints);
         ahead = false;
         if (rc) break;
+        if ((rc = flush_held()) != DEMCZ_OK) break;
         int64_t c0 = slab_end_at_or_after(g, every);
         while (c0 <= nxt && c0 - every < h->g0) c0 += every;
         const int64_t nck = c0 <= nxt ? (nxt - c0) / every + 1 : 0;
         if (nck > 0) {
             double* slot = pinned + (size_t)checks * d;
-            rc = rhat_enqueue(h, c0 - every + 1, c0, slot, monitor && nxt < g_to, (int)nck);
+            double* const slot_dev = pinned_dev + (size_t)checks * d;
+            hipStream_t qs = nullptr;
+            rc = rhat_side_gate(h, monitor && nxt < g_to, qs);
             if (rc) break;
+            if (qs != h->stream && qs == h->prod_stream && !rhat_first_env) {
+                held.on = true; held.qs = qs; held.g_from = c0 - every + 1; held.g_to = c0; held.slot = slot; held.slot_dev = slot_dev; held.nck = (int)nck;
+            } else {
+                rc = rhat_enqueue_on(h, qs, c0 - every + 1, c0, slot, (int)nck, slot_dev);
+                if (rc) break;
+            }
             checks += (int32_t)nck;
             if (!monitor) {
                 int64_t M_before = 0;
@@ -5594,6 +5650,7 @@
         }
         g = nxt + 1;
     }
+    { const int32_t rcf = flush_held(); if (rc == DEMCZ_OK) rc = rcf; }
     h->pinned_err_launches = -1;
     if (rc == DEMCZ_OK && !h->live_log.empty() && h->peer_mode != 2) {
         if (!h->pinned_err && host_malloc((void**)&h->pinned_err, 4 * sizeof(unsigned int)) != hipSuccess) { h->pinned_err = nullptr; (void)hipGetLastError(); }
@@ -5695,6 +5752,15 @@
     counts[0] = h->kernel_counts[0];
     counts[1] = wave ? h->launches - h->kernel_counts[0] : 0;
     counts[2] = wave ? 0 : h->launches;
+    return DEMCZ_OK;
+}
+
+extern "C" int32_t demcz_debug_rhat_counts(const demcz_handle* h, int64_t* counts)
+{
+    NOT_DERIVED(h);
+    if (!h || !counts) return DEMCZ_ERR_INVALID_ARGUMENT;
+    counts[0] = h->rhat_counts[0];
+    counts[1] = h->rhat_counts[1];
     return DEMCZ_OK;
 }
 
diff --git a/demc.jl_amd/csrc/demcz_kernels.h b/demc.jl_amd/csrc/demcz_kernels.h
--- a/demc.jl_amd/csrc/demcz_kernels.h
+++ b/demc.jl_amd/csrc/demcz_kernels.h
@@ -552,172 +552,6 @@
     Z[(base + (sidx * R + r) * n_loc + j) * ZS + p] = slab[i];
 }
 
-__global__ void rhat_moments_kernel(const double* chain, int64_t N, int d, int64_t s0, int64_t n, int nchunk,
-                                    double* S1, double* S2, int64_t w, int64_t slice)
-{
-    const int64_t i = (int64_t)blockIdx.x * blockDim.x + threadIdx.x;
-    if (i >= N * d) return;
-    s0 += (int64_t)blockIdx.z * w;
-    S1 += (int64_t)blockIdx.z * slice;
-    S2 += (int64_t)blockIdx.z * slice;
-    const int h = blockIdx.y / nchunk, ck = blockIdx.y % nchunk;
-    const int64_t per = (n + nchunk - 1) / nchunk;
-    const int64_t t0 = ck * per, t1 = (t0 + per < n) ? t0 + per : n;
-    const int64_t stride = N * d;
-    const double* base = chain + i + stride * (s0 + h * n);
-    const double x0 = base[0];
-    double a = 0.0, b = 0.0;
-    int64_t t = t0;
-    for (; t + 8 <= t1; t += 8) {
-        double v[8];
-#pragma unroll
-        for (int u = 0; u < 8; ++u) v[u] = base[stride * (t + u)];
-#pragma unroll
-        for (int u = 0; u < 8; ++u) {
-            const double w = v[u] - x0;
-            a += w;
-            b = fma(w, w, b);
-        }
-    }
-    for (; t < t1; ++t) {
-        double v = base[stride * t] - x0;
-        a += v;
-        b = fma(v, v, b);
-    }
-    const int64_t o = i + stride * blockIdx.y;
-    S1[o] = a;
-    S2[o] = b;
-}
-
-__global__ void rhat_chainstats_kernel(const double* chain, int64_t N, int d, int64_t s0, int64_t n, int nchunk,
-                                       const double* S1, const double* S2, double* mean_j, double* s2_j, int64_t w, int64_t slice)
-{
-    const int64_t i = (int64_t)blockIdx.x * blockDim.x + threadIdx.x;
-    if (i >= N * d) return;
-    s0 += (int64_t)blockIdx.z * w;
-    S1 += (int64_t)blockIdx.z * slice;
-    S2 += (int64_t)blockIdx.z * slice;
-    mean_j += (int64_t)blockIdx.z * slice;
-    s2_j += (int64_t)blockIdx.z * slice;
-    const int h = blockIdx.y;
-    const int64_t stride = N * d;
-    const double x0 = chain[i + stride * (s0 + h * n)];
-    double a = 0.0, b = 0.0;
-    for (int ck = 0; ck < nchunk; ++ck) {
-        a += S1[i + stride * (h * nchunk + ck)];
-        b += S2[i + stride * (h * nchunk + ck)];
-    }
-    const double nn = (double)n;
-    mean_j[i + stride * h] = x0 + a / nn;
-    s2_j[i + stride * h] = (b - a * a / nn) / (nn - 1.0);
-}
-
-__global__ void __launch_bounds__(256) rhat_reduce_kernel(const double* mean_j, const double* s2_j, int64_t N, int d,
-                                                          int stage, const double* grand, double grand_div, double* out)
-{
-    __shared__ double ra[256], rb[256];
-    const int p = blockIdx.x;
-    const int64_t stride = N * d;
-    double a = 0.0, b = 0.0;
-    const double gm = stage ? grand[p] / grand_div : 0.0;
-    int64_t h = 0, c = threadIdx.x;
-    while (c >= N) { c -= N; ++h; }
-    for (int64_t k = threadIdx.x; k < 2 * N; k += 256) {
-        const int64_t at = c + N * p + stride * h;
-        const double mj = mean_j[at];
-        if (stage == 0) {
-            a += mj;
-        } else {
-            const double dv = mj - gm;
-            a = fma(dv, dv, a);
-            b += s2_j[at];
-        }
-        c += 256;
-        while (c >= N) { c -= N; ++h; }
-    }
-    ra[threadIdx.x] = a;
-    rb[threadIdx.x] = b;
-    __syncthreads();
-    for (int s = 128; s > 0; s >>= 1) {
-        if ((int)threadIdx.x < s) {
-            ra[threadIdx.x] += ra[threadIdx.x + s];
-            rb[threadIdx.x] += rb[threadIdx.x + s];
-        }
-        __syncthreads();
-    }
-    if (threadIdx.x == 0) {
-        out[p] = ra[0];
-        if (stage) out[d + p] = rb[0];
-    }
-}
-
-__global__ void __launch_bounds__(256) rhat_tail_kernel(const double* mean_j, const double* s2_j, int64_t N, int d,
-                                                        double n, double m, double* rhat, int64_t slice)
-{
-    __shared__ double ra[256], rb[256];
-    const int p = blockIdx.x;
-    mean_j += (int64_t)blockIdx.y * slice;
-    s2_j += (int64_t)blockIdx.y * slice;
-    rhat += (int64_t)blockIdx.y * d;
-    const int64_t stride = N * d;
-    double a = 0.0, b = 0.0;
-    int64_t h0 = 0, c0 = threadIdx.x;
-    while (c0 >= N) { c0 -= N; ++h0; }
-    {
-        int64_t h = h0, c = c0;
-        for (int64_t k = threadIdx.x; k < 2 * N; k += 256) {
-            a += mean_j[c + N * p + stride * h];
-            c += 256;
-            while (c >= N) { c -= N; ++h; }
-        }
-    }
-    ra[threadIdx.x] = a;
-    __syncthreads();
-    for (int s = 128; s > 0; s >>= 1) {
-        if ((int)threadIdx.x < s) ra[threadIdx.x] += ra[threadIdx.x + s];
-        __syncthreads();
-    }
-    const double gm = ra[0] / m;
-    __syncthreads();
-    a = 0.0;
-    {
-        int64_t h = h0, c = c0;
-        for (int64_t k = threadIdx.x; k < 2 * N; k += 256) {
-            const int64_t at = c + N * p + stride * h;
-            const double dv = mean_j[at] - gm;
-            a = fma(dv, dv, a);
-            b += s2_j[at];
-            c += 256;
-            while (c >= N) { c -= N; ++h; }
-        }
-    }
-    ra[threadIdx.x] = a;
-    rb[threadIdx.x] = b;
-    __syncthreads();
-    for (int s = 128; s > 0; s >>= 1) {
-        if ((int)threadIdx.x < s) {
-            ra[threadIdx.x] += ra[threadIdx.x + s];
-            rb[threadIdx.x] += rb[threadIdx.x + s];
-        }
-        __syncthreads();
-    }
-    if (threadIdx.x == 0) {
-        const double B = n / (m - 1.0) * ra[0];
-        const double W = rb[0] / m;
-        const double varhat = (n - 1.0) / n * W + B / n;
-        rhat[p] = sqrt(varhat / W);
-    }
-}
-
-__global__ void rhat_final_kernel(const double* in, int d, double n, double m, double* rhat)
-{
-    const int p = blockIdx.x * blockDim.x + threadIdx.x;
-    if (p >= d) return;
-    const double B = n / (m - 1.0) * in[p];
-    const double W = in[d + p] / m;
-    const double varhat = (n - 1.0) / n * W + B / n;
-    rhat[p] = sqrt(varhat / W);
-}
 
 __global__ void __launch_bounds__(256) changed_from_history_kernel(const double* logobj, const double* lp_origin, int64_t N,
                                                                    int64_t s_from, long long* out)
diff --git a/demc.jl_amd/csrc/demcz_kernels_rhat.h b/demc.jl_amd/csrc/demcz_kernels_rhat.h
--- /dev/null
+++ b/demc.jl_amd/csrc/demcz_kernels_rhat.h
@@ -0,0 +1,187 @@
+#pragma once
+
+#include "demcz_device.h"
+#include "demcz_rhat_stats.h"
+
+#pragma clang fp contract(off)
+
+namespace demcz {
+
+__global__ void rhat_moments_kernel(const double* chain, int64_t N, int d, int64_t s0, int64_t n, int nchunk,
+                                    double* S1, double* S2, int64_t w, int64_t slice)
+{
+    const int64_t i = (int64_t)blockIdx.x * blockDim.x + threadIdx.x;
+    if (i >= N * d) return;
+    s0 += (int64_t)blockIdx.z * w;
+    S1 += (int64_t)blockIdx.z * slice;
+    S2 += (int64_t)blockIdx.z * slice;
+    const int h = blockIdx.y / nchunk, ck = blockIdx.y % nchunk;
+    const int64_t per = (n + nchunk - 1) / nchunk;
+    const int64_t t0 = ck * per, t1 = (t0 + per < n) ? t0 + per : n;
+    const int64_t stride = N * d;
+    const double* base = chain + i + stride * (s0 + h * n);
+    const double x0 = base[0];
+    double a = 0.0, b = 0.0;
+    int64_t t = t0;
+    for (; t + 8 <= t1; t += 8) {
+        double v[8];
+#pragma unroll
+        for (int u = 0; u < 8; ++u) v[u] = base[stride * (t + u)];
+#pragma unroll
+        for (int u = 0; u < 8; ++u) {
+            const double w = v[u] - x0;
+            a += w;
+            b = fma(w, w, b);
+        }
+    }
+    for (; t < t1; ++t) {
+        double v = base[stride * t] - x0;
+        a += v;
+        b = fma(v, v, b);
+    }
+    const int64_t o = i + stride * blockIdx.y;
+    S1[o] = a;
+    S2[o] = b;
+}
+
+__global__ void rhat_chainstats_kernel(const double* chain, int64_t N, int d, int64_t s0, int64_t n, int nchunk,
+                                       const double* S1, const double* S2, double* mean_j, double* s2_j, int64_t w, int64_t slice)
+{
+    const int64_t i = (int64_t)blockIdx.x * blockDim.x + threadIdx.x;
+    if (i >= N * d) return;
+    s0 += (int64_t)blockIdx.z * w;
+    S1 += (int64_t)blockIdx.z * slice;
+    S2 += (int64_t)blockIdx.z * slice;
+    mean_j += (int64_t)blockIdx.z * slice;
+    s2_j += (int64_t)blockIdx.z * slice;
+    const int h = blockIdx.y;
+    const int64_t stride = N * d;
+    const double x0 = chain[i + stride * (s0 + h * n)];
+    const int64_t first = i + stride * (h * nchunk);
+    rhat_chain_stats(x0, S1 + first, S2 + first, stride, nchunk, (double)n, mean_j[i + stride * h], s2_j[i + stride * h]);
+}
+
+__device__ __forceinline__ void rhat_tree(double* ra)
+{
+    __syncthreads();
+    for (int s = RHAT_TREE / 2; s > 0; s >>= 1) {
+        if ((int)threadIdx.x < s) ra[threadIdx.x] += ra[threadIdx.x + s];
+        __syncthreads();
+    }
+}
+__device__ __forceinline__ void rhat_tree(double* ra, double* rb)
+{
+    __syncthreads();
+    for (int s = RHAT_TREE / 2; s > 0; s >>= 1) {
+        if ((int)threadIdx.x < s) {
+            ra[threadIdx.x] += ra[threadIdx.x + s];
+            rb[threadIdx.x] += rb[threadIdx.x + s];
+        }
+        __syncthreads();
+    }
+}
+
+__global__ void __launch_bounds__(RHAT_TREE) rhat_reduce_kernel(const double* mean_j, const double* s2_j, int64_t N, int d,
+                                                                int stage, const double* grand, double grand_div, double* out)
+{
+    __shared__ double ra[RHAT_TREE], rb[RHAT_TREE];
+    const int p = blockIdx.x;
+    const int64_t stride = N * d;
+    const auto mean = [=](int64_t h, int64_t c, int64_t) { return mean_j[c + N * p + stride * h]; };
+    const auto var = [=](int64_t h, int64_t c, int64_t) { return s2_j[c + N * p + stride * h]; };
+    int64_t h0, c0;
+    rhat_first_element((int)threadIdx.x, N, h0, c0);
+    double a = 0.0, b = 0.0;
+    if (stage == 0) a = rhat_sum_means((int)threadIdx.x, N, h0, c0, mean);
+    else rhat_sum_squares((int)threadIdx.x, N, h0, c0, grand[p] / grand_div, mean, var, a, b);
+    ra[threadIdx.x] = a;
+    rb[threadIdx.x] = b;
+    rhat_tree(ra, rb);
+    if (threadIdx.x == 0) {
+        out[p] = ra[0];
+        if (stage) out[d + p] = rb[0];
+    }
+}
+
+__global__ void __launch_bounds__(RHAT_TREE) rhat_tail_kernel(const double* mean_j, const double* s2_j, int64_t N, int d,
+                                                              double n, double m, double* rhat, int64_t slice)
+{
+    __shared__ double ra[RHAT_TREE], rb[RHAT_TREE];
+    const int p = blockIdx.x;
+    mean_j += (int64_t)blockIdx.y * slice;
+    s2_j += (int64_t)blockIdx.y * slice;
+    rhat += (int64_t)blockIdx.y * d;
+    const int64_t stride = N * d;
+    const auto mean = [=](int64_t h, int64_t c, int64_t) { return mean_j[c + N * p + stride * h]; };
+    const auto var = [=](int64_t h, int64_t c, int64_t) { return s2_j[c + N * p + stride * h]; };
+    int64_t h0, c0;
+    rhat_first_element((int)threadIdx.x, N, h0, c0);
+    ra[threadIdx.x] = rhat_sum_means((int)threadIdx.x, N, h0, c0, mean);
+    rhat_tree(ra);
+    const double gm = ra[0] / m;
+    __syncthreads();
+    double a, b;
+    rhat_sum_squares((int)threadIdx.x, N, h0, c0, gm, mean, var, a, b);
+    ra[threadIdx.x] = a;
+    rb[threadIdx.x] = b;
+    rhat_tree(ra, rb);
+    if (threadIdx.x == 0) rhat[p] = rhat_from_sums(ra[0], rb[0], n, m);
+}
+
+__global__ void __launch_bounds__(RHAT_FINISH_BS) rhat_finish_kernel(const double* chain, int64_t N, int d, int64_t s0, int64_t n,
+                                                                     int nchunk, const double* S1, const double* S2, double m,
+                                                                     double* rhat, int64_t w, int64_t slice)
+{
+    extern __shared__ double rhat_stats_lds[];
+    __shared__ double ra[RHAT_TREE], rb[RHAT_TREE];
+    double* const lmean = rhat_stats_lds;
+    double* const lvar = rhat_stats_lds + 2 * N;
+    const int p = blockIdx.x, t = (int)threadIdx.x;
+    s0 += (int64_t)blockIdx.y * w;
+    S1 += (int64_t)blockIdx.y * slice;
+    S2 += (int64_t)blockIdx.y * slice;
+    rhat += (int64_t)blockIdx.y * d;
+    const int64_t stride = N * d;
+    const double nn = (double)n;
+    {
+        int64_t h, c;
+        rhat_first_element(t, N, h, c);
+        for (int64_t k = t; k < 2 * N; k += RHAT_FINISH_BS) {
+            const int64_t i = c + N * p;
+            const double x0 = chain[i + stride * (s0 + h * n)];
+            const int64_t first = i + stride * (h * nchunk);
+            rhat_chain_stats(x0, S1 + first, S2 + first, stride, nchunk, nn, lmean[k], lvar[k]);
+            c += RHAT_FINISH_BS;
+            while (c >= N) { c -= N; ++h; }
+        }
+    }
+    __syncthreads();
+    const bool tail = t < RHAT_TREE;
+    const auto mean = [=](int64_t, int64_t, int64_t k) { return lmean[k]; };
+    const auto var = [=](int64_t, int64_t, int64_t k) { return lvar[k]; };
+    int64_t h0 = 0, c0 = 0;
+    if (tail) {
+        rhat_first_element(t, N, h0, c0);
+        ra[t] = rhat_sum_means(t, N, h0, c0, mean);
+    }
+    rhat_tree(ra);
+    const double gm = ra[0] / m;
+    __syncthreads();
+    if (tail) {
+        double a, b;
+        rhat_sum_squares(t, N, h0, c0, gm, mean, var, a, b);
+        ra[t] = a;
+        rb[t] = b;
+    }
+    rhat_tree(ra, rb);
+    if (t == 0) rhat[p] = rhat_from_sums(ra[0], rb[0], nn, m);
+}
+
+__global__ void rhat_final_kernel(const double* in, int d, double n, double m, double* rhat)
+{
+    const int p = blockIdx.x * blockDim.x + threadIdx.x;
+    if (p >= d) return;
+    rhat[p] = rhat_from_sums(in[p], in[d + p], n, m);
+}
+
+}
diff --git a/demc.jl_amd/csrc/demcz_rhat_stats.h b/demc.jl_amd/csrc/demcz_rhat_stats.h
--- /dev/null
+++ b/demc.jl_amd/csrc/demcz_rhat_stats.h
@@ -0,0 +1,94 @@
+#pragma once
+
+#include <cmath>
+#include <cstdint>
+
+#if defined(__HIPCC__)
+#define DEMCZ_RHAT_FN __host__ __device__ __forceinline__
+#else
+#define DEMCZ_RHAT_FN inline
+#endif
+#if defined(__clang__)
+#define DEMCZ_RHAT_UNROLL _Pragma("unroll")
+#else
+#define DEMCZ_RHAT_UNROLL
+#endif
+
+#if defined(__clang__)
+#pragma clang fp contract(off)
+#endif
+
+namespace demcz {
+
+constexpr int RHAT_TREE = 256;
+constexpr int RHAT_FINISH_BS = 1024;
+constexpr int64_t RHAT_FINISH_MAX_N = 2048;
+
+DEMCZ_RHAT_FN void rhat_chain_stats(double x0, const double* S1, const double* S2, int64_t cstride, int nchunk, double nn,
+                                    double& mean, double& s2)
+{
+    double a = 0.0, b = 0.0;
+    int ck = 0;
+    for (; ck + 8 <= nchunk; ck += 8) {
+        double u[8], v[8];
+        DEMCZ_RHAT_UNROLL
+        for (int i = 0; i < 8; ++i) {
+            u[i] = S1[cstride * (ck + i)];
+            v[i] = S2[cstride * (ck + i)];
+        }
+        DEMCZ_RHAT_UNROLL
+        for (int i = 0; i < 8; ++i) {
+            a += u[i];
+            b += v[i];
+        }
+    }
+    for (; ck < nchunk; ++ck) {
+        a += S1[cstride * ck];
+        b += S2[cstride * ck];
+    }
+    mean = x0 + a / nn;
+    s2 = (b - a * a / nn) / (nn - 1.0);
+}
+
+DEMCZ_RHAT_FN void rhat_first_element(int t, int64_t N, int64_t& h, int64_t& c)
+{
+    h = 0;
+    c = t;
+    while (c >= N) { c -= N; ++h; }
+}
+
+template <class Mean>
+DEMCZ_RHAT_FN double rhat_sum_means(int t, int64_t N, int64_t h, int64_t c, Mean mean)
+{
+    double a = 0.0;
+    for (int64_t k = t; k < 2 * N; k += RHAT_TREE) {
+        a += mean(h, c, k);
+        c += RHAT_TREE;
+        while (c >= N) { c -= N; ++h; }
+    }
+    return a;
+}
+
+template <class Mean, class Var>
+DEMCZ_RHAT_FN void rhat_sum_squares(int t, int64_t N, int64_t h, int64_t c, double gm, Mean mean, Var var, double& a, double& b)
+{
+    a = 0.0;
+    b = 0.0;
+    for (int64_t k = t; k < 2 * N; k += RHAT_TREE) {
+        const double dv = mean(h, c, k) - gm;
+        a = __builtin_fma(dv, dv, a);
+        b += var(h, c, k);
+        c += RHAT_TREE;
+        while (c >= N) { c -= N; ++h; }
+    }
+}
+
+DEMCZ_RHAT_FN double rhat_from_sums(double ssq, double svar, double n, double m)
+{
+    const double B = n / (m - 1.0) * ssq;
+    const double W = svar / m;
+    const double varhat = (n - 1.0) / n * W + B / n;
+    return sqrt(varhat / W);
+}
+
+}
diff --git a/demc.jl_amd/engine.py b/demc.jl_amd/engine.py
--- a/demc.jl_amd/engine.py
+++ b/demc.jl_amd/engine.py
@@ -738,6 +738,11 @@
         self._chk(self._L.demcz_debug_kernel_counts(self._h, c))
         return dict(zip(("ps2", "ps_general", "other"), (int(v) for v in c)))
 
+    def rhat_kernel_counts(self):
+        c = (C.c_int64 * 2)()
+        self._chk(self._L.demcz_debug_rhat_counts(self._h, c))
+        return dict(zip(("finish", "chainstats_tail"), (int(v) for v in c)))
+
     def kernel_name(self):
         buf = C.create_string_buffer(192)
         self._chk(self._L.demcz_debug_kernel_name(self._h, buf, 192))
diff --git a/include/demcz.h b/include/demcz.h
--- a/include/demcz.h
+++ b/include/demcz.h
@@ -261,6 +261,7 @@
 int32_t demcz_set_live_rearms(demcz_handle* h, int32_t n);
 int32_t demcz_get_live_rearms(const demcz_handle* h, int32_t* rearms, int32_t* left);
 int32_t demcz_debug_kernel_counts(const demcz_handle* h, int64_t* counts);
+int32_t demcz_debug_rhat_counts(const demcz_handle* h, int64_t* counts);
 int32_t demcz_debug_kernel_name(const demcz_handle* h, char* buf, int32_t cap);
 
 int32_t demcz_debug_set_live_fault(demcz_handle* h, int32_t polls, int64_t g_from);
```

Result: no change. 724.1 million (-0.1%).
